# aerius-labs/zksnap-circuits-halo2

Measured on AMD Instinct MI355X. Metric: BN254 G1 MSM Mpoints/sec, higher is better.
Workload: dtype u32x9 (254-bit modular integer, radix 2^29); 1 GPU; BN254 G1 MSM, 2^20 random points/scalars per GPU (BASELINE configs[1]), point-range sharded x1, inputs resident in HBM, bases registered once (prepared fixed-base table, as under ParamsKZG::commit); points_per_gpu=1048576, parallelism=point-range shard x1 + all_gather(96 B) + fold

## Files before the change

include/zkhip.h:

```cpp
#ifndef ZKHIP_H
#define ZKHIP_H
#include <stddef.h>
#include <stdint.h>
#ifdef __cplusplus
extern "C" {
#endif

#define ZKHIP_OK 0
#define ZKHIP_EINVAL (-1)
#define ZKHIP_ENODEV (-2)
#define ZKHIP_EHIP (-3)
#define ZKHIP_ENOMEM (-4)
#define ZKHIP_EBUSY (-5)

int zkhip_init(const int *devices, int ndev);
void zkhip_shutdown(void);
const char *zkhip_last_error(void);
int zkhip_device_name(char *buf, size_t len);
int zkhip_device_count(void);
int zkhip_set_msm_shards(int shards);
int zkhip_msm_shards(void);


int zkhip_msm_g1(const uint64_t *scalars, const uint64_t *bases, size_t n, uint64_t out_xyz[12]);
// ... 103 lines not shown
                                      const uint64_t omega[4], void *d_z, void *stream);

int zkhip_lookup_permute(const uint64_t *input, const uint64_t *table, size_t usable_rows, uint64_t *permuted_input, uint64_t *permuted_table);
int zkhip_lookup_permute_device(const void *d_input, const void *d_table, size_t usable_rows, void *d_permuted_input, void *d_permuted_table,
                                void *stream);
int zkhip_lookup_permute_many_device(const void *const *d_inputs, const void *const *d_tables, uint32_t n_lookups, uint32_t log_n, size_t usable_rows,
                                     void *d_permuted_inputs, void *d_permuted_tables, void *stream);
int zkhip_lookup_products_device(const void *const *d_inputs, const void *const *d_tables, const void *d_permuted_inputs, const void *d_permuted_tables,
                                 uint32_t n_lookups, uint32_t log_n, size_t usable_rows, const uint64_t beta[4], const uint64_t gamma[4], void *d_z,
                                 void *stream);

typedef struct zkhip_check_report { uint64_t failures; uint64_t first; } zkhip_check_report;
int zkhip_check_rows_device(const zkhip_vm_program *progs, uint32_t n_progs, const void *const *d_columns, uint32_t n_columns,
                            uint32_t log_rows, uint64_t row0, uint64_t count, void *d_reports, void *stream);
int zkhip_check_copies_device(const void *const *d_columns, uint32_t n_columns, uint32_t log_n, const void *d_map_col, const void *d_map_row,
                              void *d_report, void *stream);
int zkhip_check_lookups_device(const void *const *d_inputs, const void *const *d_tables, uint32_t n_lookups, uint32_t log_n,
                               size_t usable_rows, void *d_reports, void *stream);

int zkhip_fr_random_device(const uint8_t seed[32], uint64_t stream_id, uint64_t first, size_t n, void *d_out, void *stream);
int zkhip_fr_random(const uint8_t seed[32], uint64_t stream_id, uint64_t first, size_t n, uint64_t *out);
int zkhip_fr_random_rows_device(const uint8_t seed[32], uint64_t stream_id, uint64_t first, const void *const *d_cols,
                                uint32_t n_cols, size_t row0, size_t count, void *stream);

int zkhip_alloc(size_t bytes, void **d_ptr);
int zkhip_free(void *d_ptr);
int zkhip_upload(void *d_dst, const void *src, size_t bytes);
int zkhip_download(void *dst, const void *d_src, size_t bytes);
int zkhip_sync(void);
int zkhip_stream_sync(void *stream);

int zkhip_msm_g1_device(const void *d_scalars, const void *d_bases, size_t n, void *d_out_xyz, void *stream);
int zkhip_msm_g2_device(const void *d_scalars, const void *d_bases, size_t n, void *d_out_xyz, void *stream);
int zkhip_prepare_bases_device(const void *d_bases, size_t n, uint64_t *handle);
int zkhip_prepare_bases_device_c(const void *d_bases, size_t n, int window_bits, uint64_t *handle);
int zkhip_release_bases(uint64_t handle);
int zkhip_prepared_window_bits(uint64_t handle);
int zkhip_msm_g1_prepared_device(uint64_t handle, size_t offset, const void *d_scalars, size_t n, void *d_out_xyz, void *stream);
int zkhip_msm_g1_registered_device(const uint64_t *bases, const void *d_scalars, size_t n, void *d_out_xyz, void *stream);
int zkhip_msm_g1_registered_batch_device(const uint64_t *bases, const void *d_scalars, size_t n, size_t batch, size_t scalar_stride, void *d_out_xyz,
                                         void *stream);
int zkhip_msm_g1_prepared_batch_device(uint64_t handle, size_t offset, const void *d_scalars, size_t n, size_t batch, size_t scalar_stride,
                                       void *d_out_xyz, void *stream);
int zkhip_msm_g1_device_c(const void *d_scalars, const void *d_bases, size_t n, void *d_out_xyz, int window_bits, void *stream);
int zkhip_ntt_fr_device(void *d_a, const uint64_t omega[4], uint32_t log_n, void *stream);
int zkhip_ifft_scaled_device(void *d_a, const uint64_t omega_inv[4], uint32_t log_n, const uint64_t divisor[4], void *stream);
int zkhip_mul_periodic_device(void *d_a, size_t n, const void *d_table, uint32_t period, void *stream);
int zkhip_coeff_to_extended_device(const void *d_a, size_t a_stride, uint32_t k, void *d_out, size_t out_stride, uint32_t ext_k, uint32_t batch,
                                   const uint64_t ext_omega[4], const uint64_t zeta[4], void *stream);
int zkhip_extended_to_coeff_device(const void *d_a, size_t a_stride, uint32_t ext_k, const uint64_t ext_omega_inv[4], const uint64_t ext_divisor[4],
                                   const uint64_t zeta[4], void *d_out, size_t out_stride, size_t out_len, uint32_t batch, void *stream);
int zkhip_ntt_fr_batch_device(void *d_a, const uint64_t omega[4], uint32_t log_n, uint32_t batch, size_t stride, void *stream);
int zkhip_ifft_scaled_batch_device(void *d_a, const uint64_t omega_inv[4], uint32_t log_n, const uint64_t divisor[4], uint32_t batch,
                                   size_t stride, void *stream);
int zkhip_g1_sum_device(const void *d_points_xyz, int m, void *d_out_xyz, void *stream);
int zkhip_g1_sum(const uint64_t *points_xyz, int m, uint64_t out_xyz[12]);
int zkhip_msm_window_bits(size_t n);

int zkhip_g1_gen_walk_device(const uint64_t t0[4], const uint64_t d[4], size_t n, void *d_out, void *stream);
int zkhip_g1_fixed_base_mul_device(const void *d_scalars, size_t n, void *d_out, void *stream);
int zkhip_g1_fft_device(void *d_points_xyz, const uint64_t omega[4], uint32_t log_n, void *stream);
int zkhip_g_to_lagrange_device(const void *d_g, uint32_t k, void *d_g_lagrange, void *stream);
int zkhip_g_to_lagrange(const uint64_t *g_xyz, uint32_t k, uint64_t *g_lagrange);
int zkhip_g1_batch_normalize(const uint64_t *points_xyz, size_t n, uint64_t *out_affine);
int zkhip_g1_batch_normalize_device(const void *d_points_xyz, size_t n, void *d_out_affine, void *stream);
int zkhip_g1_check_points(const uint64_t *points, size_t n, uint64_t *first_bad);
int zkhip_g1_check_points_device(const void *d_points, size_t n, uint64_t *first_bad, void *stream);
int zkhip_g1_compress(const uint64_t *points, size_t n, uint8_t *out32, int flag_layout);
int zkhip_g1_compress_device(const void *d_points, size_t n, void *d_out32, int flag_layout, void *stream);
int zkhip_g1_decompress(const uint8_t *in32, size_t n, uint64_t *points, int flag_layout, uint64_t *first_bad);
int zkhip_g1_decompress_device(const void *d_in32, size_t n, void *d_points, int flag_layout, uint64_t *first_bad, void *stream);
typedef struct zkhip_transcript zkhip_transcript;
zkhip_transcript *zkhip_transcript_new(int flag_layout);
zkhip_transcript *zkhip_transcript_new_reader(const uint8_t *proof, size_t len, int flag_layout);
void zkhip_transcript_free(zkhip_transcript *t);
int zkhip_transcript_common_scalars(zkhip_transcript *t, const uint64_t *fr_mont, size_t n);
int zkhip_transcript_common_points(zkhip_transcript *t, const uint64_t *affine_mont, size_t n);
int zkhip_transcript_squeeze(zkhip_transcript *t, uint64_t out_fr_mont[4]);
int zkhip_transcript_write_scalars(zkhip_transcript *t, const uint64_t *fr_mont, size_t n);
int zkhip_transcript_write_points_device(zkhip_transcript *t, const void *d_points_xyz, size_t n, void *stream);
int zkhip_transcript_write_scalars_device(zkhip_transcript *t, const void *d_fr, size_t n, void *stream);
int zkhip_transcript_write_points(zkhip_transcript *t, const uint64_t *points_xyz, size_t n);
int zkhip_transcript_read_scalars(zkhip_transcript *t, size_t n, uint64_t *fr_mont);
int zkhip_transcript_read_points_device(zkhip_transcript *t, size_t n, void *d_affine, void *stream);
int zkhip_transcript_read_points(zkhip_transcript *t, size_t n, uint64_t *affine_mont);
int zkhip_transcript_proof(const zkhip_transcript *t, uint8_t *buf, size_t cap, size_t *len);
zkhip_transcript *zkhip_transcript_new_poseidon(int flag_layout);
zkhip_transcript *zkhip_transcript_new_poseidon_reader(const uint8_t *proof, size_t len, int flag_layout);
int zkhip_profile_enable(int on);
int zkhip_profile_read(double *ms, char (*names)[64], int max);
int zkhip_profile_read_calls(double *ms, char (*names)[64], int *call_of, int max);

#define ZKHIP_POSEIDON_MAX_WIDTH 16
#define ZKHIP_POSEIDON_SUBTREE 256
int zkhip_poseidon_permute(uint64_t *states, size_t n);
int zkhip_poseidon_hash(const uint64_t *fr, size_t n, uint64_t out[4]);
int zkhip_poseidon_constants(uint64_t out[204 * 4]);
int zkhip_poseidon_hash_many_device(const void *d_in, size_t n, uint32_t width, void *d_out, void *stream);
int zkhip_poseidon_hash_points_device(const void *d_points, size_t n, uint32_t layout, void *d_out, void *stream);
int zkhip_poseidon_merkle_device(const void *d_leaves, size_t n_leaves, void *d_nodes, void *stream);

#define ZKHIP_IMT_MAX_DEPTH 24
typedef struct zkhip_imt zkhip_imt;
typedef struct zkhip_imt_witness {
  void *d_roots;
  void *d_low_leaves;
  void *d_new_leaves;
  void *d_low_indices;
  void *d_low_proofs;
  void *d_new_proofs;
} zkhip_imt_witness;
int zkhip_imt_create(uint32_t depth, zkhip_imt **t);
int zkhip_imt_destroy(zkhip_imt *t);
int zkhip_imt_insert(zkhip_imt *t, const uint64_t *values, size_t n_new, const zkhip_imt_witness *out, size_t *first_bad, void *stream);
int zkhip_imt_root(zkhip_imt *t, uint64_t out[4]);
int zkhip_imt_leaf(zkhip_imt *t, uint32_t index, uint64_t out[12]);
int zkhip_imt_proof(zkhip_imt *t, uint32_t index, uint64_t *out );
int zkhip_imt_size(const zkhip_imt *t, uint32_t *depth, uint32_t *used);
int zkhip_imt_export_device(zkhip_imt *t, void *d_leaves, void *d_nodes, void *d_preimages, void *stream);
int zkhip_imt_link(const uint64_t *used_vals, size_t n_used, const uint64_t *new_vals, size_t n_new, uint32_t *low_index_out, size_t *first_bad);

#define ZKHIP_PAILLIER_WORDS 6
#define ZKHIP_PAILLIER_MAX_N_BITS 192
int zkhip_paillier_mul_device(const uint64_t n[3], const void *d_a, const void *d_b, size_t count, void *d_out, void *stream);
int zkhip_paillier_tally_device(const uint64_t n[3], const void *d_ballots, size_t n_ballots, uint32_t n_cols, const void *d_init, void *d_running, void *stream);
int zkhip_paillier_encrypt_device(const uint64_t n[3], const uint64_t g[6], const void *d_m, const void *d_r, size_t count, void *d_out, void *stream);

#define ZKHIP_PLUME_MAX_MSG 64
int zkhip_secp256k1_lincomb_device(const void *d_a, const void *d_p, const void *d_b, const void *d_q, size_t count, void *d_out, void *d_status, void *stream);
int zkhip_secp256k1_hash_to_curve_device(const uint8_t *msg, size_t msg_len, const void *d_pk, size_t count, void *d_out, void *d_status, void *stream);
int zkhip_plume_verify_device(const uint8_t *msg, size_t msg_len, const void *d_pk, const void *d_nullifier, const void *d_s, const void *d_c, size_t count, void *d_status, void *d_report, void *d_h_out, void *stream);
int zkhip_plume_sign_device(const uint8_t *msg, size_t msg_len, const void *d_sk, const void *d_r, size_t count, void *d_pk, void *d_nullifier, void *d_s, void *d_c, void *d_status, void *d_h_out, void *stream);
int zkhip_secp256k1_hash_to_curve(const uint8_t *msg, size_t msg_len, const uint64_t pk[8], uint64_t out[8], uint32_t *status);
int zkhip_plume_verify(const uint8_t *msg, size_t msg_len, const uint64_t pk[8], const uint64_t nullifier[8], const uint64_t s[4], const uint64_t c[4], uint32_t *verdict, uint64_t h_out[8]);
int zkhip_plume_sign(const uint8_t *msg, size_t msg_len, const uint64_t sk[4], const uint64_t r[4], uint64_t pk[8], uint64_t nullifier[8], uint64_t s[4], uint64_t c[4], uint32_t *status, uint64_t h_out[8]);

int zkhip_fr_domain_points_device(uint32_t k, uint32_t usable_rows, const uint64_t omega[4], const void *d_x, size_t n_points, void *d_out, void *stream);
int zkhip_verify_identity_device(const zkhip_vm_program *prog, const void *d_evals, uint32_t n_evals, const void *d_challenges, uint32_t k,
                                 uint32_t usable_rows, const uint64_t omega[4], size_t n_proofs, void *d_status, void *d_report, void *stream);
int zkhip_fr_instance_evals_device(uint32_t k, const uint64_t omega[4], const void *d_x, const void *d_instances, const uint32_t *column_lens, uint32_t n_columns,
                                   const uint32_t *query_columns, const uint32_t *query_rotations, uint32_t n_queries, size_t n_proofs, void *d_out, void *stream);
int zkhip_verify_identity_instances_device(const zkhip_vm_program *prog, const void *d_evals, uint32_t n_evals, const void *d_challenges, uint32_t k,
                                           uint32_t usable_rows, const uint64_t omega[4], const void *d_instances, const uint32_t *column_lens, uint32_t n_columns,
                                           const uint32_t *query_columns, const uint32_t *query_rotations, uint32_t n_queries, size_t n_proofs,
                                           void *d_status, void *d_report, void *stream);

int zkhip_test_field_op(int field, int op, const uint64_t *a, const uint64_t *b, uint64_t *out, size_t n);
int zkhip_test_g1_op(int op, const uint64_t *a, const uint64_t *b, uint64_t *out_xyz, size_t n);

int zkhip_test_g2_op(int op, const uint64_t *a, const uint64_t *b, uint64_t *out_xyz, size_t n);

int zkhip_test_reduce512(const uint8_t in64[64], uint64_t out_fr_mont[4]);
uint32_t zkhip_test_transcript_chunk(size_t n);

#define ZKHIP_MAX_PAIRS 64
int zkhip_pairing_check(const uint64_t *g1, const uint64_t *g2, size_t n, int *ok);
int zkhip_pairing_check_device(const void *d_g1, const void *d_g2, size_t n, void *d_ok , void *stream);
int zkhip_test_fq12_op(int op, const uint64_t *a, const uint64_t *b, uint64_t *out);

struct zkhip_gwc_plan {
  uint32_t n_evals, n_sets, n_slots, reserved;
  const uint32_t *set_rotation;
  const uint32_t *query_set;
  const uint32_t *query_pos;
  const uint32_t *query_slot;
};
typedef struct zkhip_gwc_plan zkhip_gwc_plan;
int zkhip_gwc_scalars_device(const zkhip_gwc_plan *plan, const void *d_evals, const void *d_points, uint32_t k, const uint64_t omega[4], size_t n_proofs,
                             void *d_rows_a, void *d_rows_c, void *stream);
int zkhip_fr_fold_rows_device(const void *d_rows, uint32_t n_cols, uint32_t n_own, const void *d_r, int negate, size_t n_rows, void *d_out_own,
                              void *d_out_shared, void *stream);
struct zkhip_shplonk_plan {
  uint32_t n_evals, n_sets, n_slots, n_points;
  const uint32_t *point_rotation;
  const uint32_t *set_start;
  const uint32_t *set_point;
  const uint32_t *slot_set;
  const uint32_t *slot_pos;
  const uint32_t *query_slot;
  const uint32_t *query_point;
};
typedef struct zkhip_shplonk_plan zkhip_shplonk_plan;
int zkhip_shplonk_scalars_device(const zkhip_shplonk_plan *plan, const void *d_evals, const void *d_points, uint32_t k, const uint64_t omega[4], size_t n_proofs,
                                 void *d_rows_a, void *d_rows_c, void *d_status, void *stream);

#ifdef __cplusplus
}
#endif
#endif
```

zksnap_circuits_halo2_amd/_lib.py:

```python
from __future__ import annotations

import ctypes as C
import os

_HERE = os.path.dirname(os.path.abspath(__file__))
LIB_PATH = os.path.join(_HERE, "libzkhip.so")
ZKHIP_MAX_ROOTS = 8
ZKHIP_MAX_PAIRS = 64
ZKHIP_POSEIDON_MAX_WIDTH = 16
ZKHIP_POSEIDON_SUBTREE = 256
ZKHIP_IMT_MAX_DEPTH = 24
ZKHIP_PAILLIER_WORDS = 6
ZKHIP_PAILLIER_MAX_N_BITS = 192
ZKHIP_PLUME_MAX_MSG = 64

_SIGS = {
    "zkhip_init": (C.c_int, [C.POINTER(C.c_int), C.c_int]),
    "zkhip_shutdown": (None, []),
    "zkhip_last_error": (C.c_char_p, []),
    "zkhip_device_name": (C.c_int, [C.c_char_p, C.c_size_t]),
    "zkhip_device_count": (C.c_int, []),
    "zkhip_set_msm_shards": (C.c_int, [C.c_int]),
    "zkhip_msm_shards": (C.c_int, []),
    "zkhip_msm_g1": (C.c_int, [C.c_void_p, C.c_void_p, C.c_size_t, C.c_void_p]),
# ... 10 lines not shown
    "zkhip_set_ntt_fanout": (C.c_int, [C.c_int]),
    "zkhip_ntt_fanout": (C.c_int, []),
    "zkhip_register_bases": (C.c_int, [C.c_void_p, C.c_size_t]),
    "zkhip_unregister_bases": (C.c_int, [C.c_void_p]),
    "zkhip_ntt_fr": (C.c_int, [C.c_void_p, C.c_void_p, C.c_uint32]),
    "zkhip_ifft_scaled": (C.c_int, [C.c_void_p, C.c_void_p, C.c_uint32, C.c_void_p]),
    "zkhip_coeff_to_extended": (C.c_int, [C.c_void_p, C.c_uint32, C.c_void_p, C.c_uint32, C.c_void_p, C.c_void_p]),
    "zkhip_extended_to_coeff": (C.c_int, [C.c_void_p, C.c_uint32, C.c_void_p, C.c_void_p, C.c_void_p, C.c_void_p, C.c_size_t]),
    "zkhip_mul_periodic": (C.c_int, [C.c_void_p, C.c_size_t, C.c_void_p, C.c_uint32]),
    "zkhip_fr_eval_polynomial": (C.c_int, [C.c_void_p, C.c_size_t, C.c_void_p, C.c_void_p]),
    "zkhip_fr_kate_division": (C.c_int, [C.c_void_p, C.c_size_t, C.c_void_p, C.c_void_p]),
    "zkhip_fr_batch_invert": (C.c_int, [C.c_void_p, C.c_size_t]),
    "zkhip_fr_prefix_product": (C.c_int, [C.c_void_p, C.c_size_t, C.c_void_p]),
    "zkhip_fr_eval_polynomial_device": (C.c_int, [C.c_void_p, C.c_size_t, C.c_void_p, C.c_void_p, C.c_void_p]),
    "zkhip_fr_eval_polynomial_batch_device": (C.c_int, [C.c_void_p, C.c_size_t, C.c_size_t, C.c_void_p, C.c_void_p, C.c_void_p]),
    "zkhip_fr_kate_division_device": (C.c_int, [C.c_void_p, C.c_size_t, C.c_void_p, C.c_void_p, C.c_void_p]),
    "zkhip_fr_divide_by_roots": (C.c_int, [C.c_void_p, C.c_size_t, C.c_void_p, C.c_uint32, C.c_void_p, C.c_void_p]),
    "zkhip_fr_divide_by_roots_device": (C.c_int, [C.c_void_p, C.c_size_t, C.c_void_p, C.c_uint32, C.c_void_p, C.c_void_p, C.c_void_p]),
    "zkhip_fr_batch_invert_device": (C.c_int, [C.c_void_p, C.c_size_t, C.c_void_p]),
    "zkhip_fr_prefix_product_device": (C.c_int, [C.c_void_p, C.c_size_t, C.c_void_p, C.c_void_p]),
    "zkhip_fr_eval_rows": (C.c_int, [C.c_void_p, C.c_void_p, C.c_uint32, C.c_uint32, C.c_int, C.c_void_p]),
    "zkhip_fr_eval_rows_device": (C.c_int, [C.c_void_p, C.c_void_p, C.c_uint32, C.c_uint32, C.c_int, C.c_void_p, C.c_void_p]),
    "zkhip_fr_grand_product": (C.c_int, [C.c_void_p, C.c_void_p, C.c_size_t, C.c_void_p]),
    "zkhip_fr_grand_product_device": (C.c_int, [C.c_void_p, C.c_void_p, C.c_size_t, C.c_void_p, C.c_void_p]),
    "zkhip_lookup_permute": (C.c_int, [C.c_void_p, C.c_void_p, C.c_size_t, C.c_void_p, C.c_void_p]),
    "zkhip_lookup_permute_device": (C.c_int, [C.c_void_p, C.c_void_p, C.c_size_t, C.c_void_p, C.c_void_p, C.c_void_p]),
    "zkhip_lookup_permute_many_device": (C.c_int, [C.c_void_p, C.c_void_p, C.c_uint32, C.c_uint32, C.c_size_t, C.c_void_p, C.c_void_p, C.c_void_p]),
    "zkhip_lookup_products_device": (C.c_int, [C.c_void_p, C.c_void_p, C.c_void_p, C.c_void_p, C.c_uint32, C.c_uint32, C.c_size_t, C.c_void_p, C.c_void_p, C.c_void_p,
                                               C.c_void_p]),
    "zkhip_check_rows_device": (C.c_int, [C.c_void_p, C.c_uint32, C.c_void_p, C.c_uint32, C.c_uint32, C.c_uint64, C.c_uint64, C.c_void_p, C.c_void_p]),
    "zkhip_check_copies_device": (C.c_int, [C.c_void_p, C.c_uint32, C.c_uint32, C.c_void_p, C.c_void_p, C.c_void_p, C.c_void_p]),
    "zkhip_check_lookups_device": (C.c_int, [C.c_void_p, C.c_void_p, C.c_uint32, C.c_uint32, C.c_size_t, C.c_void_p, C.c_void_p]),
    "zkhip_fr_random_device": (C.c_int, [C.c_void_p, C.c_uint64, C.c_uint64, C.c_size_t, C.c_void_p, C.c_void_p]),
    "zkhip_fr_random": (C.c_int, [C.c_void_p, C.c_uint64, C.c_uint64, C.c_size_t, C.c_void_p]),
    "zkhip_fr_random_rows_device": (C.c_int, [C.c_void_p, C.c_uint64, C.c_uint64, C.c_void_p, C.c_uint32, C.c_size_t, C.c_size_t, C.c_void_p]),
    "zkhip_alloc": (C.c_int, [C.c_size_t, C.POINTER(C.c_void_p)]),
    "zkhip_free": (C.c_int, [C.c_void_p]),
    "zkhip_upload": (C.c_int, [C.c_void_p, C.c_void_p, C.c_size_t]),
    "zkhip_download": (C.c_int, [C.c_void_p, C.c_void_p, C.c_size_t]),
    "zkhip_sync": (C.c_int, []),
    "zkhip_stream_sync": (C.c_int, [C.c_void_p]),
    "zkhip_msm_g1_device": (C.c_int, [C.c_void_p, C.c_void_p, C.c_size_t, C.c_void_p, C.c_void_p]),
    "zkhip_prepare_bases_device": (C.c_int, [C.c_void_p, C.c_size_t, C.POINTER(C.c_uint64)]),
    "zkhip_g1_fft_device": (C.c_int, [C.c_void_p, C.c_void_p, C.c_uint32, C.c_void_p]),
    "zkhip_g_to_lagrange_device": (C.c_int, [C.c_void_p, C.c_uint32, C.c_void_p, C.c_void_p]),
    "zkhip_g_to_lagrange": (C.c_int, [C.c_void_p, C.c_uint32, C.c_void_p]),
    "zkhip_prepare_bases_device_c": (C.c_int, [C.c_void_p, C.c_size_t, C.c_int, C.POINTER(C.c_uint64)]),
    "zkhip_release_bases": (C.c_int, [C.c_uint64]),
    "zkhip_prepared_window_bits": (C.c_int, [C.c_uint64]),
    "zkhip_msm_g1_prepared_device": (C.c_int, [C.c_uint64, C.c_size_t, C.c_void_p, C.c_size_t, C.c_void_p, C.c_void_p]),
    "zkhip_msm_g1_prepared_batch_device": (C.c_int, [C.c_uint64, C.c_size_t, C.c_void_p, C.c_size_t, C.c_size_t, C.c_size_t, C.c_void_p, C.c_void_p]),
    "zkhip_msm_g1_device_c": (C.c_int, [C.c_void_p, C.c_void_p, C.c_size_t, C.c_void_p, C.c_int, C.c_void_p]),
    "zkhip_ntt_fr_device": (C.c_int, [C.c_void_p, C.c_void_p, C.c_uint32, C.c_void_p]),
    "zkhip_ntt_fr_batch_device": (C.c_int, [C.c_void_p, C.c_void_p, C.c_uint32, C.c_uint32, C.c_size_t, C.c_void_p]),
    "zkhip_ifft_scaled_batch_device": (C.c_int, [C.c_void_p, C.c_void_p, C.c_uint32, C.c_void_p, C.c_uint32, C.c_size_t, C.c_void_p]),
    "zkhip_ifft_scaled_device": (C.c_int, [C.c_void_p, C.c_void_p, C.c_uint32, C.c_void_p, C.c_void_p]),
    "zkhip_mul_periodic_device": (C.c_int, [C.c_void_p, C.c_size_t, C.c_void_p, C.c_uint32, C.c_void_p]),
    "zkhip_coeff_to_extended_device": (C.c_int, [C.c_void_p, C.c_size_t, C.c_uint32, C.c_void_p, C.c_size_t, C.c_uint32, C.c_uint32, C.c_void_p, C.c_void_p, C.c_void_p]),
    "zkhip_extended_to_coeff_device": (C.c_int, [C.c_void_p, C.c_size_t, C.c_uint32, C.c_void_p, C.c_void_p, C.c_void_p, C.c_void_p, C.c_size_t, C.c_size_t, C.c_uint32, C.c_void_p]),
    "zkhip_g1_sum_device": (C.c_int, [C.c_void_p, C.c_int, C.c_void_p, C.c_void_p]),
    "zkhip_g1_sum": (C.c_int, [C.c_void_p, C.c_int, C.c_void_p]),
    "zkhip_msm_window_bits": (C.c_int, [C.c_size_t]),
    "zkhip_g1_fixed_base_mul_device": (C.c_int, [C.c_void_p, C.c_size_t, C.c_void_p, C.c_void_p]),
    "zkhip_g1_gen_walk_device": (C.c_int, [C.c_void_p, C.c_void_p, C.c_size_t, C.c_void_p, C.c_void_p]),
    "zkhip_g1_batch_normalize": (C.c_int, [C.c_void_p, C.c_size_t, C.c_void_p]),
    "zkhip_g1_batch_normalize_device": (C.c_int, [C.c_void_p, C.c_size_t, C.c_void_p, C.c_void_p]),
    "zkhip_g1_check_points": (C.c_int, [C.c_void_p, C.c_size_t, C.POINTER(C.c_uint64)]),
    "zkhip_g1_check_points_device": (C.c_int, [C.c_void_p, C.c_size_t, C.POINTER(C.c_uint64), C.c_void_p]),
    "zkhip_msm_g1_registered_device": (C.c_int, [C.c_void_p, C.c_void_p, C.c_size_t, C.c_void_p, C.c_void_p]),
    "zkhip_msm_g1_registered_batch_device": (C.c_int, [C.c_void_p, C.c_void_p, C.c_size_t, C.c_size_t, C.c_size_t, C.c_void_p, C.c_void_p]),
    "zkhip_fr_gather_mul_device": (C.c_int, [C.c_void_p, C.c_size_t, C.c_void_p, C.c_void_p, C.c_size_t, C.c_void_p, C.c_size_t, C.c_void_p, C.c_void_p]),
    "zkhip_g1_compress": (C.c_int, [C.c_void_p, C.c_size_t, C.c_void_p, C.c_int]),
    "zkhip_g1_compress_device": (C.c_int, [C.c_void_p, C.c_size_t, C.c_void_p, C.c_int, C.c_void_p]),
    "zkhip_g1_decompress": (C.c_int, [C.c_void_p, C.c_size_t, C.c_void_p, C.c_int, C.POINTER(C.c_uint64)]),
    "zkhip_g1_decompress_device": (C.c_int, [C.c_void_p, C.c_size_t, C.c_void_p, C.c_int, C.POINTER(C.c_uint64), C.c_void_p]),
    "zkhip_permutation_products": (C.c_int, [C.c_void_p, C.c_void_p, C.c_uint32, C.c_uint32, C.c_uint32, C.c_size_t, C.c_void_p, C.c_void_p, C.c_void_p, C.c_void_p, C.c_void_p]),
    "zkhip_permutation_products_device": (C.c_int, [C.c_void_p, C.c_void_p, C.c_uint32, C.c_uint32, C.c_uint32, C.c_size_t, C.c_void_p, C.c_void_p, C.c_void_p, C.c_void_p,
                                                    C.c_void_p, C.c_void_p]),
    "zkhip_fr_eval_rows_sum_device": (C.c_int, [C.c_void_p, C.c_void_p, C.c_uint32, C.c_void_p, C.c_uint32, C.c_uint32, C.c_void_p, C.c_void_p]),
    "zkhip_fr_eval_rows_window_device": (C.c_int, [C.c_void_p, C.c_void_p, C.c_uint32, C.c_uint32, C.c_uint64, C.c_uint64, C.c_int, C.c_void_p, C.c_void_p]),
    "zkhip_fr_eval_rows_sharded_device": (C.c_int, [C.c_void_p, C.c_void_p, C.c_void_p, C.c_uint32, C.c_uint32, C.c_uint32, C.c_void_p, C.c_void_p, C.c_void_p,
                                                    C.c_void_p]),
    "zkhip_row_shards_create": (C.c_int, [C.c_uint32, C.c_uint32, C.c_uint32, C.c_uint32, C.POINTER(C.c_void_p)]),
    "zkhip_row_shards_destroy": (C.c_int, [C.c_void_p]),
    "zkhip_row_shards_window": (C.c_int, [C.c_void_p, C.c_uint32, C.c_uint32, C.POINTER(C.c_void_p), C.POINTER(C.c_int), C.POINTER(C.c_uint64),
                                          C.POINTER(C.c_uint64)]),
    "zkhip_row_shards_scatter_device": (C.c_int, [C.c_void_p, C.c_uint32, C.c_void_p, C.c_void_p]),
    "zkhip_row_shards_gather_device": (C.c_int, [C.c_void_p, C.c_uint32, C.c_void_p, C.c_void_p]),
    "zkhip_row_shards_upload": (C.c_int, [C.c_void_p, C.c_uint32, C.c_void_p]),
    "zkhip_coeff_to_extended_row_shards_device": (C.c_int, [C.c_void_p, C.c_uint32, C.c_uint32, C.c_size_t, C.c_void_p, C.c_void_p, C.c_void_p, C.c_uint32,
                                                            C.c_void_p]),
    "zkhip_lagrange_cosets_row_shards_device": (C.c_int, [C.c_uint32, C.c_uint64, C.c_void_p, C.c_void_p, C.c_void_p, C.c_void_p, C.c_uint32, C.c_void_p]),
    "zkhip_fr_linear_combination_device": (C.c_int, [C.c_void_p, C.c_void_p, C.c_size_t, C.c_size_t, C.c_void_p, C.c_void_p]),
    "zkhip_multiopen_gwc_device": (C.c_int, [C.c_void_p, C.c_uint32, C.c_void_p, C.c_size_t, C.c_void_p, C.c_void_p, C.c_size_t, C.POINTER(C.c_size_t)]),
    "zkhip_multiopen_shplonk_begin_device": (C.c_int, [C.c_void_p, C.c_uint32, C.c_void_p, C.c_size_t, C.c_void_p, C.c_void_p, C.c_void_p, C.POINTER(C.c_void_p)]),
    "zkhip_multiopen_shplonk_finish_device": (C.c_int, [C.c_void_p, C.c_void_p, C.c_void_p]),
    "zkhip_multiopen_shplonk_abort": (C.c_int, [C.c_void_p]),
    "zkhip_transcript_new": (C.c_void_p, [C.c_int]),
    "zkhip_transcript_new_reader": (C.c_void_p, [C.c_char_p, C.c_size_t, C.c_int]),
    "zkhip_transcript_free": (None, [C.c_void_p]),
    "zkhip_transcript_common_scalars": (C.c_int, [C.c_void_p, C.c_void_p, C.c_size_t]),
    "zkhip_transcript_common_points": (C.c_int, [C.c_void_p, C.c_void_p, C.c_size_t]),
    "zkhip_transcript_squeeze": (C.c_int, [C.c_void_p, C.c_void_p]),
    "zkhip_transcript_write_scalars": (C.c_int, [C.c_void_p, C.c_void_p, C.c_size_t]),
    "zkhip_transcript_write_points_device": (C.c_int, [C.c_void_p, C.c_void_p, C.c_size_t, C.c_void_p]),
    "zkhip_transcript_write_scalars_device": (C.c_int, [C.c_void_p, C.c_void_p, C.c_size_t, C.c_void_p]),
    "zkhip_transcript_write_points": (C.c_int, [C.c_void_p, C.c_void_p, C.c_size_t]),
    "zkhip_transcript_read_scalars": (C.c_int, [C.c_void_p, C.c_size_t, C.c_void_p]),
    "zkhip_transcript_read_points_device": (C.c_int, [C.c_void_p, C.c_size_t, C.c_void_p, C.c_void_p]),
    "zkhip_transcript_read_points": (C.c_int, [C.c_void_p, C.c_size_t, C.c_void_p]),
    "zkhip_transcript_proof": (C.c_int, [C.c_void_p, C.c_void_p, C.c_size_t, C.POINTER(C.c_size_t)]),
    "zkhip_transcript_new_poseidon": (C.c_void_p, [C.c_int]),
    "zkhip_transcript_new_poseidon_reader": (C.c_void_p, [C.c_char_p, C.c_size_t, C.c_int]),
    "zkhip_poseidon_permute": (C.c_int, [C.c_void_p, C.c_size_t]),
    "zkhip_poseidon_hash": (C.c_int, [C.c_void_p, C.c_size_t, C.c_void_p]),
    "zkhip_poseidon_constants": (C.c_int, [C.c_void_p]),
    "zkhip_poseidon_hash_many_device": (C.c_int, [C.c_void_p, C.c_size_t, C.c_uint32, C.c_void_p, C.c_void_p]),
    "zkhip_poseidon_hash_points_device": (C.c_int, [C.c_void_p, C.c_size_t, C.c_uint32, C.c_void_p, C.c_void_p]),
    "zkhip_poseidon_merkle_device": (C.c_int, [C.c_void_p, C.c_size_t, C.c_void_p, C.c_void_p]),
    "zkhip_imt_create": (C.c_int, [C.c_uint32, C.POINTER(C.c_void_p)]),
    "zkhip_imt_destroy": (C.c_int, [C.c_void_p]),
    "zkhip_imt_insert": (C.c_int, [C.c_void_p, C.c_void_p, C.c_size_t, C.c_void_p, C.POINTER(C.c_size_t), C.c_void_p]),
    "zkhip_imt_root": (C.c_int, [C.c_void_p, C.c_void_p]),
    "zkhip_imt_leaf": (C.c_int, [C.c_void_p, C.c_uint32, C.c_void_p]),
    "zkhip_imt_proof": (C.c_int, [C.c_void_p, C.c_uint32, C.c_void_p]),
    "zkhip_imt_size": (C.c_int, [C.c_void_p, C.POINTER(C.c_uint32), C.POINTER(C.c_uint32)]),
    "zkhip_imt_export_device": (C.c_int, [C.c_void_p, C.c_void_p, C.c_void_p, C.c_void_p, C.c_void_p]),
    "zkhip_imt_link": (C.c_int, [C.c_void_p, C.c_size_t, C.c_void_p, C.c_size_t, C.c_void_p, C.POINTER(C.c_size_t)]),
    "zkhip_paillier_mul_device": (C.c_int, [C.c_void_p, C.c_void_p, C.c_void_p, C.c_size_t, C.c_void_p, C.c_void_p]),
    "zkhip_paillier_tally_device": (C.c_int, [C.c_void_p, C.c_void_p, C.c_size_t, C.c_uint32, C.c_void_p, C.c_void_p, C.c_void_p]),
    "zkhip_paillier_encrypt_device": (C.c_int, [C.c_void_p, C.c_void_p, C.c_void_p, C.c_void_p, C.c_size_t, C.c_void_p, C.c_void_p]),
    "zkhip_secp256k1_lincomb_device": (C.c_int, [C.c_void_p, C.c_void_p, C.c_void_p, C.c_void_p, C.c_size_t, C.c_void_p, C.c_void_p, C.c_void_p]),
    "zkhip_secp256k1_hash_to_curve_device": (C.c_int, [C.c_char_p, C.c_size_t, C.c_void_p, C.c_size_t, C.c_void_p, C.c_void_p, C.c_void_p]),
    "zkhip_plume_verify_device": (C.c_int, [C.c_char_p, C.c_size_t, C.c_void_p, C.c_void_p, C.c_void_p, C.c_void_p, C.c_size_t, C.c_void_p, C.c_void_p, C.c_void_p,
                                            C.c_void_p]),
    "zkhip_secp256k1_hash_to_curve": (C.c_int, [C.c_char_p, C.c_size_t, C.c_void_p, C.c_void_p, C.c_void_p]),
    "zkhip_plume_verify": (C.c_int, [C.c_char_p, C.c_size_t, C.c_void_p, C.c_void_p, C.c_void_p, C.c_void_p, C.c_void_p, C.c_void_p]),
    "zkhip_plume_sign_device": (C.c_int, [C.c_char_p, C.c_size_t, C.c_void_p, C.c_void_p, C.c_size_t, C.c_void_p, C.c_void_p, C.c_void_p, C.c_void_p, C.c_void_p,
                                          C.c_void_p, C.c_void_p]),
    "zkhip_plume_sign": (C.c_int, [C.c_char_p, C.c_size_t, C.c_void_p, C.c_void_p, C.c_void_p, C.c_void_p, C.c_void_p, C.c_void_p, C.c_void_p, C.c_void_p]),
    "zkhip_fr_domain_points_device": (C.c_int, [C.c_uint32, C.c_uint32, C.c_void_p, C.c_void_p, C.c_size_t, C.c_void_p, C.c_void_p]),
    "zkhip_verify_identity_device": (C.c_int, [C.c_void_p, C.c_void_p, C.c_uint32, C.c_void_p, C.c_uint32, C.c_uint32, C.c_void_p, C.c_size_t, C.c_void_p, C.c_void_p,
                                               C.c_void_p]),
    "zkhip_fr_instance_evals_device": (C.c_int, [C.c_uint32, C.c_void_p, C.c_void_p, C.c_void_p, C.POINTER(C.c_uint32), C.c_uint32, C.POINTER(C.c_uint32),
                                                 C.POINTER(C.c_uint32), C.c_uint32, C.c_size_t, C.c_void_p, C.c_void_p]),
    "zkhip_verify_identity_instances_device": (C.c_int, [C.c_void_p, C.c_void_p, C.c_uint32, C.c_void_p, C.c_uint32, C.c_uint32, C.c_void_p, C.c_void_p,
                                                         C.POINTER(C.c_uint32), C.c_uint32, C.POINTER(C.c_uint32), C.POINTER(C.c_uint32), C.c_uint32, C.c_size_t,
                                                         C.c_void_p, C.c_void_p, C.c_void_p]),
    "zkhip_gwc_scalars_device": (C.c_int, [C.c_void_p, C.c_void_p, C.c_void_p, C.c_uint32, C.c_void_p, C.c_size_t, C.c_void_p, C.c_void_p, C.c_void_p]),
    "zkhip_fr_fold_rows_device": (C.c_int, [C.c_void_p, C.c_uint32, C.c_uint32, C.c_void_p, C.c_int, C.c_size_t, C.c_void_p, C.c_void_p, C.c_void_p]),
    "zkhip_shplonk_scalars_device": (C.c_int, [C.c_void_p, C.c_void_p, C.c_void_p, C.c_uint32, C.c_void_p, C.c_size_t, C.c_void_p, C.c_void_p, C.c_void_p, C.c_void_p]),
    "zkhip_test_reduce512": (C.c_int, [C.c_void_p, C.c_void_p]),
    "zkhip_test_transcript_chunk": (C.c_uint32, [C.c_size_t]),
    "zkhip_profile_enable": (C.c_int, [C.c_int]),
    "zkhip_profile_read": (C.c_int, [C.c_void_p, C.c_void_p, C.c_int]),
    "zkhip_profile_read_calls": (C.c_int, [C.c_void_p, C.c_void_p, C.c_void_p, C.c_int]),
    "zkhip_test_field_op": (C.c_int, [C.c_int, C.c_int, C.c_void_p, C.c_void_p, C.c_void_p, C.c_size_t]),
    "zkhip_test_g1_op": (C.c_int, [C.c_int, C.c_void_p, C.c_void_p, C.c_void_p, C.c_size_t]),
    "zkhip_pairing_check": (C.c_int, [C.c_void_p, C.c_void_p, C.c_size_t, C.POINTER(C.c_int)]),
    "zkhip_pairing_check_device": (C.c_int, [C.c_void_p, C.c_void_p, C.c_size_t, C.c_void_p, C.c_void_p]),
    "zkhip_test_fq12_op": (C.c_int, [C.c_int, C.c_void_p, C.c_void_p, C.c_void_p]),
}



class ProverQueryC(C.Structure):
    _fields_ = [("point", C.c_uint64 * 4), ("d_poly", C.c_void_p), ("eval", C.c_uint64 * 4), ("has_eval", C.c_uint32), ("reserved", C.c_uint32)]


class ImtWitness(C.Structure):
    _fields_ = [("d_roots", C.c_void_p), ("d_low_leaves", C.c_void_p), ("d_new_leaves", C.c_void_p), ("d_low_indices", C.c_void_p),
                ("d_low_proofs", C.c_void_p), ("d_new_proofs", C.c_void_p)]


class GwcPlan(C.Structure):
    _fields_ = [("n_evals", C.c_uint32), ("n_sets", C.c_uint32), ("n_slots", C.c_uint32), ("reserved", C.c_uint32),
                ("set_rotation", C.POINTER(C.c_uint32)), ("query_set", C.POINTER(C.c_uint32)), ("query_pos", C.POINTER(C.c_uint32)),
                ("query_slot", C.POINTER(C.c_uint32))]


class ShplonkPlan(C.Structure):
    _fields_ = [("n_evals", C.c_uint32), ("n_sets", C.c_uint32), ("n_slots", C.c_uint32), ("n_points", C.c_uint32),
                ("point_rotation", C.POINTER(C.c_uint32)), ("set_start", C.POINTER(C.c_uint32)), ("set_point", C.POINTER(C.c_uint32)),
                ("slot_set", C.POINTER(C.c_uint32)), ("slot_pos", C.POINTER(C.c_uint32)), ("query_slot", C.POINTER(C.c_uint32)),
                ("query_point", C.POINTER(C.c_uint32))]


class CheckReport(C.Structure):
    _fields_ = [("failures", C.c_uint64), ("first", C.c_uint64)]


class VmOperand(C.Structure):
    _fields_ = [("kind", C.c_uint8), ("rot", C.c_uint8), ("index", C.c_uint16)]


class VmInsn(C.Structure):
    _fields_ = [("op", C.c_uint8), ("dst", C.c_uint8), ("reserved", C.c_uint16), ("a", VmOperand), ("b", VmOperand), ("c", VmOperand)]


class VmProgram(C.Structure):
    _fields_ = [("insns", C.POINTER(VmInsn)), ("n_insns", C.c_uint32),
                ("constants", C.c_void_p), ("n_constants", C.c_uint32),
                ("rotations", C.POINTER(C.c_int32)), ("n_rotations", C.c_uint32),
                ("rot_scale", C.c_int32), ("result_reg", C.c_uint32), ("omega", C.c_void_p)]


VM_REGS = 16
_lib = None


class ZkhipError(RuntimeError):
    index = None

    def __init__(self, code: int, msg: str):
        super().__init__(f"libzkhip error {code}: {msg}")
        self.code = code


def load() -> C.CDLL:
    global _lib
    if _lib is not None:
        return _lib
    path = os.environ.get("ZKHIP_LIB_PATH", LIB_PATH)
    if not os.path.exists(path):
        raise ImportError(f"{path} not found: build it with `python -c 'import __graft_entry__ as g; g.build()'` "
                          "(hipcc, gfx950).  There is no CPU fallback.")
    try:
        import torch
    except ImportError:
        pass
    lib = C.CDLL(path)
    for name, (res, args) in _SIGS.items():
        fn = getattr(lib, name)
        fn.restype = res
        fn.argtypes = args
    _lib = lib
    return lib


def exported_symbols():
    return sorted(_SIGS)


def check(rc: int) -> None:
    if rc != 0:
        raise ZkhipError(rc, load().zkhip_last_error().decode(errors="replace"))
```

zksnap_circuits_halo2_amd/csrc/capi.hip:

```cpp
#include <hip/hip_runtime.h>
#include <algorithm>
#include <atomic>
#include <condition_variable>
#include <cstdarg>
#include <cstdio>
#include <cstdlib>
#include <cstring>
#include <dlfcn.h>
#include <functional>
#include <map>
#include <memory>
#include <mutex>
#include <thread>
#include <vector>
#include "zkhip_internal.hpp"
#include "blake2b.hpp"
#include "poseidon.hpp"
#include "imt.hpp"
#include "modn.hpp"
#include "secp256k1_h2c.hpp"
#include "../../include/zkhip.hpp"

namespace zkhip {

// ... 3824 lines not shown
  if (!t) return;
  delete t->sponge;
  if (t->pinned) { (void)hipHostFree(t->pinned); (void)hipGetLastError(); }
  delete t;
}

int zkhip_transcript_common_scalars(zkhip_transcript* t, const uint64_t* fr_mont, size_t n) {
  if (!t || (n && !fr_mont)) { set_error("transcript_common_scalars: null pointer"); return ZKHIP_EINVAL; }
  for (size_t i = 0; i < n; i++) {
    uint8_t repr[32];
    fr_mont_to_repr(fr_mont + i * 4, repr);
    tr_absorb_scalar(t, repr);
  }
  return ZKHIP_OK;
}

int zkhip_transcript_common_points(zkhip_transcript* t, const uint64_t* affine_mont, size_t n) {
  if (!t || (n && !affine_mont)) { set_error("transcript_common_points: null pointer"); return ZKHIP_EINVAL; }
  for (size_t i = 0; i < n; i++)
    if (bytes_zero((const uint8_t*)(affine_mont + i * 8), 64)) { set_error("transcript: cannot write points at infinity to the transcript (point %zu of %zu)", i, n); return ZKHIP_EINVAL; }
  for (size_t i = 0; i < n; i++) {
    uint8_t xy[64];
    fq_mont_to_repr(affine_mont + i * 8, xy);
    fq_mont_to_repr(affine_mont + i * 8 + 4, xy + 32);
    tr_absorb_point(t, xy);
  }
  return ZKHIP_OK;
}

int zkhip_transcript_squeeze(zkhip_transcript* t, uint64_t out_fr_mont[4]) {
  if (!t || !out_fr_mont) { set_error("transcript_squeeze: null pointer"); return ZKHIP_EINVAL; }
  if (t->poseidon) {
    const halo2::Fr c = t->sponge->squeeze();
    memcpy(out_fr_mont, c.l, 32);
    return ZKHIP_OK;
  }
  const uint8_t prefix = 0x00;
  t->st.update(&prefix, 1);
  uint8_t digest[64];
  t->st.digest(digest, 64);
  fr_reduce512(digest, out_fr_mont);
  return ZKHIP_OK;
}

int zkhip_transcript_write_scalars(zkhip_transcript* t, const uint64_t* fr_mont, size_t n) {
  int rc = tr_check_write(t, fr_mont, n, "transcript_write_scalars");
  if (rc != ZKHIP_OK) return rc;
  for (size_t i = 0; i < n; i++) {
    uint8_t repr[32];
    fr_mont_to_repr(fr_mont + i * 4, repr);
    tr_absorb_scalar(t, repr);
    t->proof.insert(t->proof.end(), repr, repr + 32);
  }
  return ZKHIP_OK;
}

int zkhip_transcript_write_points_device(zkhip_transcript* t, const void* d_points_xyz, size_t n, void* stream) {
  ZK_API_RANGE();
  int rc = tr_check_write(t, d_points_xyz, n, "transcript_write_points_device");
  if (rc != ZKHIP_OK) return rc;
  if ((uintptr_t)d_points_xyz & 15) { set_error("transcript_write_points_device: d_points_xyz must be 16-byte aligned"); return ZKHIP_EINVAL; }
  if (n == 0) return ZKHIP_OK;
  hipStream_t s = caller_stream(stream);
  scratch_pin P(s);
  if (P.rc != ZKHIP_OK) return P.rc;
  stream_drain drain(s);
  if ((rc = tr_write_points_core(t, P.sc, s, d_points_xyz, n)) != ZKHIP_OK) return rc;
  drain.done();
  return ZKHIP_OK;
}

int zkhip_transcript_write_scalars_device(zkhip_transcript* t, const void* d_fr, size_t n, void* stream) {
  ZK_API_RANGE();
  int rc = tr_check_write(t, d_fr, n, "transcript_write_scalars_device");
  if (rc != ZKHIP_OK) return rc;
  if ((uintptr_t)d_fr & 15) { set_error("transcript_write_scalars_device: d_fr must be 16-byte aligned"); return ZKHIP_EINVAL; }
  if (n == 0) return ZKHIP_OK;
  hipStream_t s = caller_stream(stream);
  scratch_pin P(s);
  if (P.rc != ZKHIP_OK) return P.rc;
  stream_drain drain(s);
  if ((rc = tr_write_scalars_core(t, P.sc, s, d_fr, n)) != ZKHIP_OK) return rc;
  drain.done();
  return ZKHIP_OK;
}

int zkhip_transcript_write_points(zkhip_transcript* t, const uint64_t* points_xyz, size_t n) {
  ZK_API_RANGE();
  int rc = tr_check_write(t, points_xyz, n, "transcript_write_points");
  if (rc != ZKHIP_OK) return rc;
  if (n == 0) return ZKHIP_OK;
  lane_hold H;
  if (H.rc != ZKHIP_OK) return H.rc;
  if ((rc = H.sc->poly.reserve(n * 96)) != ZKHIP_OK) return rc;
  HIPCHK(hipMemcpyAsync(H.sc->poly.p, points_xyz, n * 96, hipMemcpyHostToDevice, H.s));
  if ((rc = tr_write_points_core(t, H.sc, H.s, H.sc->poly.p, n)) != ZKHIP_OK) return rc;
  return H.finish();
}

int zkhip_transcript_read_scalars(zkhip_transcript* t, size_t n, uint64_t* fr_mont) {
  int rc = tr_check_read(t, fr_mont, n, "transcript_read_scalars");
  if (rc != ZKHIP_OK) return rc;
  const uint8_t* src = t->proof.data() + t->cursor;
  for (size_t i = 0; i < n; i++)
    if (!fr_repr_to_mont(src + i * 32, fr_mont + i * 4)) { set_error("transcript: read_scalars: scalar %zu of %zu (proof byte %zu) is not below r", i, n, t->cursor + i * 32); return ZKHIP_EINVAL; }
  for (size_t i = 0; i < n; i++) tr_absorb_scalar(t, src + i * 32);
  t->cursor += n * 32;
  return ZKHIP_OK;
}

int zkhip_transcript_read_points_device(zkhip_transcript* t, size_t n, void* d_affine, void* stream) {
  ZK_API_RANGE();
  int rc = tr_check_read(t, d_affine, n, "transcript_read_points_device");
  if (rc != ZKHIP_OK) return rc;
  if ((uintptr_t)d_affine & 15) { set_error("transcript_read_points_device: d_affine must be 16-byte aligned"); return ZKHIP_EINVAL; }
  if (n == 0) return ZKHIP_OK;
  hipStream_t s = caller_stream(stream);
  scratch_pin P(s);
  if (P.rc != ZKHIP_OK) return P.rc;
  stream_drain drain(s);
  if ((rc = tr_read_points_core(t, P.sc, s, n, d_affine, nullptr)) != ZKHIP_OK) return rc;
  drain.done();
  return ZKHIP_OK;
}

int zkhip_transcript_read_points(zkhip_transcript* t, size_t n, uint64_t* affine_mont) {
  ZK_API_RANGE();
  int rc = tr_check_read(t, affine_mont, n, "transcript_read_points");
  if (rc != ZKHIP_OK) return rc;
  if (n == 0) return ZKHIP_OK;
  lane_hold H;
  if (H.rc != ZKHIP_OK) return H.rc;
  if ((rc = H.sc->bases.reserve(n * 64)) != ZKHIP_OK) return rc;
  if ((rc = tr_read_points_core(t, H.sc, H.s, n, H.sc->bases.p, affine_mont)) != ZKHIP_OK) return rc;
  return H.finish();
}

int zkhip_transcript_proof(const zkhip_transcript* t, uint8_t* buf, size_t cap, size_t* len) {
  if (!t || !len) { set_error("transcript_proof: null pointer"); return ZKHIP_EINVAL; }
  *len = t->proof.size();
  if (!buf) return ZKHIP_OK;
  if (cap < t->proof.size()) { set_error("transcript_proof: %zu bytes of room, %zu needed", cap, t->proof.size()); return ZKHIP_EINVAL; }
  if (!t->proof.empty()) memcpy(buf, t->proof.data(), t->proof.size());
  return ZKHIP_OK;
}

int zkhip_test_reduce512(const uint8_t in64[64], uint64_t out_fr_mont[4]) {
  if (!in64 || !out_fr_mont) { set_error("test_reduce512: null pointer"); return ZKHIP_EINVAL; }
  fr_reduce512(in64, out_fr_mont);
  return ZKHIP_OK;
}

uint32_t zkhip_test_transcript_chunk(size_t n) { return transcript_chunk(n); }

}
```

zksnap_circuits_halo2_amd/csrc/msm.hip:

```cpp
#include <hip/hip_runtime.h>
#include <atomic>
#include <cstdint>
#include <cstdio>
#include <cstring>
#include <cstdlib>
#include <mutex>
#include "ec_quad.hpp"
#include "fe_inverse.hpp"
#include "reduce_plan.hpp"
#include "zkhip_internal.hpp"

namespace zkhip {

static inline size_t align_up(size_t v, size_t a) { return (v + a - 1) / a * a; }

constexpr int FINE_BITS = 12;
constexpr int MAX_GROUPS = 128;
constexpr int MAX_WIDE_W = 16;
struct win_layout { int c, W, narrow; };
__host__ __device__ __forceinline__ int win_bits(const win_layout& L, int w) { return w < L.W - L.narrow ? L.c : L.c - 1; }
__host__ __device__ __forceinline__ int win_off(const win_layout& L, int w) { const int full = L.W - L.narrow; return w <= full ? w * L.c : full * L.c + (w - full) * (L.c - 1); }
static int msm_narrow_windows(int c, int W) {
  if (c <= 16) return 0;
  const int narrow = W * c - 256;
  return narrow > 0 && narrow <= W ? narrow : 0;
}
constexpr int MAX_TASK_LEN = 128;
constexpr int TASK_SHIFT = 6;

__device__ __forceinline__ xyzz load_xyzz(const uint32_t* base, size_t idx) {
  const uint4* q = reinterpret_cast<const uint4*>(base + idx * 36);
  uint32_t w[36];
#pragma unroll
  for (int i = 0; i < 9; i++) {
    uint4 v = q[i];
    w[4 * i] = v.x; w[4 * i + 1] = v.y; w[4 * i + 2] = v.z; w[4 * i + 3] = v.w;
  }
  xyzz r;
#pragma unroll
  for (int i = 0; i < 9; i++) { r.X.l[i] = w[i]; r.Y.l[i] = w[9 + i]; r.ZZ.l[i] = w[18 + i]; r.ZZZ.l[i] = w[27 + i]; }
  return r;
}

__device__ __forceinline__ void store_xyzz(uint32_t* base, size_t idx, const xyzz& a) {
  uint32_t w[36];
#pragma unroll
  for (int i = 0; i < 9; i++) { w[i] = a.X.l[i]; w[9 + i] = a.Y.l[i]; w[18 + i] = a.ZZ.l[i]; w[27 + i] = a.ZZZ.l[i]; }
  uint4* q = reinterpret_cast<uint4*>(base + idx * 36);
#pragma unroll
  for (int i = 0; i < 9; i++) q[i] = make_uint4(w[4 * i], w[4 * i + 1], w[4 * i + 2], w[4 * i + 3]);
}

__device__ __forceinline__ xyzz xyzz_shfl_xor(const xyzz& a, int mask) {
  xyzz r;
#pragma unroll
  for (int i = 0; i < NL; i++) {
    r.X.l[i] = (uint32_t)__shfl_xor((int)a.X.l[i], mask, 64);
    r.Y.l[i] = (uint32_t)__shfl_xor((int)a.Y.l[i], mask, 64);
    r.ZZ.l[i] = (uint32_t)__shfl_xor((int)a.ZZ.l[i], mask, 64);
    r.ZZZ.l[i] = (uint32_t)__shfl_xor((int)a.ZZZ.l[i], mask, 64);
  }
  return r;
}

__device__ __forceinline__ fe load_fe9_generic(const uint32_t* p, size_t idx) {
  fe r;
#pragma unroll
  for (int i = 0; i < 9; i++) r.l[i] = p[idx * 9 + i];
  return r;
}
__device__ __forceinline__ void store_fe9_generic(uint32_t* p, size_t idx, const fe& a) {
#pragma unroll
  for (int i = 0; i < 9; i++) p[idx * 9 + i] = a.l[i];
}

__global__ void __launch_bounds__(256) k_digits(const uint32_t* __restrict__ scalars, int16_t* __restrict__ digits,
                                                uint32_t n, uint32_t n_pad, int c, int W, uint32_t K, size_t scalar_stride, int narrow) {
  const size_t idx = (size_t)blockIdx.x * blockDim.x + threadIdx.x;
  if (idx >= (size_t)K * n_pad) return;
  const uint32_t kb = (uint32_t)(idx / n_pad), i = (uint32_t)(idx % n_pad);
  digits += (size_t)kb * n_pad;
  const size_t row = (size_t)K * n_pad;
  if (i >= n) {
    for (int win = 0; win < W; win++) digits[(size_t)win * row + i] = 0;
    return;
  }
  uint32_t w[8];
  load_words(scalars + ((size_t)kb * scalar_stride + i) * 8, w);
  fe c32;
#pragma unroll
  for (int k = 0; k < NL; k++) c32.l[k] = FrParams::FROM_EXT_CANON[k];
  fe s = fe_canon_lt2p<FrParams>(fe_mul<FrParams>(c32, fe_unpack<0>(w)));
  fe_pack(s, w);
  const win_layout lay{c, W, narrow};
  uint32_t carry = 0;
  for (int win = 0; win < W; win++) {
    const int bit = win_off(lay, win), cw = win_bits(lay, win);
    const uint32_t half = 1u << (cw - 1), mask = (1u << cw) - 1;
    uint32_t v = 0;
    if (bit < 256) {
      int wi = bit >> 5, sh = bit & 31;
      uint64_t two = w[wi];
      if (wi + 1 < 8) two |= (uint64_t)w[wi + 1] << 32;
      v = (uint32_t)(two >> sh) & mask;
    }
    v += carry;
    int32_t d;
    if (v >= half) { d = (int32_t)v - (int32_t)(1u << cw); carry = 1; } else { d = (int32_t)v; carry = 0; }
    digits[(size_t)win * row + i] = (int16_t)d;
  }
}

__global__ void __launch_bounds__(1024) k_digits_wide(const uint32_t* __restrict__ scalars, int32_t* __restrict__ digits, uint32_t n, uint32_t n_pad,
                                                       int c, int W, uint32_t* __restrict__ gcount, int narrow) {
  __shared__ uint32_t cnt[MAX_WIDE_W * MAX_GROUPS];
  for (uint32_t t = threadIdx.x; t < (uint32_t)W * MAX_GROUPS; t += blockDim.x) cnt[t] = 0;
  __syncthreads();
  const win_layout lay{c, W, narrow};
  for (uint32_t i = blockIdx.x * blockDim.x + threadIdx.x; i < n_pad; i += gridDim.x * blockDim.x) {
    if (i >= n) {
      for (int win = 0; win < W; win++) digits[(size_t)win * n_pad + i] = 0;
      continue;
    }
    uint32_t w[8];
    load_words(scalars + (size_t)i * 8, w);
    fe c32;
#pragma unroll
    for (int k = 0; k < NL; k++) c32.l[k] = FrParams::FROM_EXT_CANON[k];
    fe sv = fe_canon_lt2p<FrParams>(fe_mul<FrParams>(c32, fe_unpack<0>(w)));
    fe_pack(sv, w);
    uint32_t carry = 0;
    for (int win = 0; win < W; win++) {
      const int bit = win_off(lay, win), cw = win_bits(lay, win);
      const uint32_t half = 1u << (cw - 1), mask = (1u << cw) - 1;
      uint32_t v = 0;
      if (bit < 256) {
        const int wi = bit >> 5, sh = bit & 31;
        uint64_t two = w[wi];
        if (wi + 1 < 8) two |= (uint64_t)w[wi + 1] << 32;
        v = (uint32_t)(two >> sh) & mask;
      }
      v += carry;
      int32_t d;
      if (v >= half) { d = (int32_t)v - (int32_t)(1u << cw); carry = 1; } else { d = (int32_t)v; carry = 0; }
      digits[(size_t)win * n_pad + i] = d;
      if (d != 0) atomicAdd(&cnt[win * MAX_GROUPS + (((uint32_t)(d < 0 ? -d : d) - 1) >> FINE_BITS)], 1u);
    }
  }
  __syncthreads();
  for (uint32_t t = threadIdx.x; t < (uint32_t)W * MAX_GROUPS; t += blockDim.x)
    if (cnt[t]) atomicAdd(&gcount[t], cnt[t]);
}

namespace glv {
__device__ constexpr uint32_t G1[3] = {0xc7e0b3d7u, 0xd91d232eu, 0x2u};
__device__ constexpr uint32_t G2[5] = {0x391eb18eu, 0x7a7bd9d4u, 0xa773d2cfu, 0x4ccef014u, 0x2u};
__device__ constexpr uint32_t A1[2] = {0x94d213e3u, 0x89d32568u};
__device__ constexpr uint32_t A2[4] = {0x1221250bu, 0x0be4e154u, 0xeeb859fdu, 0x6f4d8248u};
__device__ constexpr uint32_t NB1[4] = {0x7d4f1128u, 0x8211bbebu, 0xeeb859fcu, 0x6f4d8248u};
__device__ constexpr uint32_t BETA_EXT[8] = {0xd782e155u, 0x71930c11u, 0xffbe3323u, 0xa6bb947cu, 0xd4741444u, 0xaa303344u, 0x26594943u, 0x2c3b3f0du};

template <int NA, int NB, int NO>
__device__ __forceinline__ void mul_low(const uint32_t (&a)[NA], const uint32_t* __restrict__ b, uint32_t (&out)[NO]) {
#pragma unroll
  for (int i = 0; i < NO; i++) out[i] = 0;
#pragma unroll
  for (int i = 0; i < NA; i++) {
    uint32_t carry = 0;
#pragma unroll
    for (int j = 0; j < NB; j++) {
      if (i + j < NO) {
        const uint64_t t = (uint64_t)a[i] * b[j] + out[i + j] + carry;
        out[i + j] = (uint32_t)t;
        carry = (uint32_t)(t >> 32);
      }
    }
    if (i + NB < NO) out[i + NB] = carry;
  }
}

__device__ __forceinline__ bool abs160(uint32_t (&v)[5], uint32_t (&mag)[4]) {
// ... 270 lines not shown

constexpr uint32_t SORT_CHUNK = 28672;

__global__ void __launch_bounds__(64) k_group_offsets(const uint32_t* __restrict__ wcount, int W, int G, uint32_t* __restrict__ goff, uint32_t* __restrict__ wcursor,
                                                       uint32_t* __restrict__ cstart, uint32_t chunk) {
  if (blockIdx.x != 0 || threadIdx.x >= 64) return;
  const int lane = threadIdx.x;
  uint32_t c0 = 0, c1 = 0;
  for (int w = 0; w < W; w++) {
    if (2 * lane < G) c0 += wcount[w * MAX_GROUPS + 2 * lane];
    if (2 * lane + 1 < G) c1 += wcount[w * MAX_GROUPS + 2 * lane + 1];
  }
  const uint32_t k0 = (c0 + chunk - 1) / chunk, k1 = (c1 + chunk - 1) / chunk;
  uint32_t x = c0 + c1, y = k0 + k1;
#pragma unroll
  for (int off = 1; off < 64; off <<= 1) {
    const uint32_t xs = __shfl_up(x, off, 64), ys = __shfl_up(y, off, 64);
    if (lane >= off) { x += xs; y += ys; }
  }
  const uint32_t ex = x - (c0 + c1), ey = y - (k0 + k1);
  if (2 * lane < G) { goff[2 * lane] = ex; cstart[2 * lane] = ey; }
  if (2 * lane + 1 < G) { goff[2 * lane + 1] = ex + c0; cstart[2 * lane + 1] = ey + k0; }
  uint32_t r0 = ex, r1 = ex + c0;
  for (int w = 0; w < W; w++) {
    if (2 * lane < G) { wcursor[w * MAX_GROUPS + 2 * lane] = r0; r0 += wcount[w * MAX_GROUPS + 2 * lane]; }
    if (2 * lane + 1 < G) { wcursor[w * MAX_GROUPS + 2 * lane + 1] = r1; r1 += wcount[w * MAX_GROUPS + 2 * lane + 1]; }
  }
  if (lane == 63) { goff[G] = x; cstart[G] = y; }
}

constexpr int FINE_BATCH = 7;
__device__ __forceinline__ void fine_histogram(const uint16_t* __restrict__ stage_fine, uint32_t start, uint32_t end, uint32_t* __restrict__ cur) {
  for (uint32_t p = start + threadIdx.x; p < end; p += FINE_BATCH * blockDim.x) {
    uint32_t f[FINE_BATCH];
#pragma unroll
    for (int k = 0; k < FINE_BATCH; k++) { const uint32_t q = p + k * blockDim.x; f[k] = q < end ? stage_fine[q] : 0xffffffffu; }
#pragma unroll
    for (int k = 0; k < FINE_BATCH; k++) if (f[k] != 0xffffffffu) atomicAdd(&cur[f[k]], 1u);
  }
}

__global__ void __launch_bounds__(1024) k_fine_sorted(const uint16_t* __restrict__ stage_fine, const uint32_t* __restrict__ stage_ref,
                                                      const uint32_t* __restrict__ goff, const uint32_t* __restrict__ cstart, int G,
                                                      uint32_t* __restrict__ cursor, uint32_t* __restrict__ sorted) {
  extern __shared__ uint32_t hist[];
  constexpr uint32_t FB = 1u << FINE_BITS;
  constexpr uint32_t CHUNK = SORT_CHUNK;
  constexpr int PER_LANE = CHUNK / 1024;
  static_assert(FB == 4096, "one thread owns four buckets in the scan");
  static_assert(CHUNK % 1024 == 0 && CHUNK / 32 <= 1024, "a lane owns CHUNK / 1024 entries; one mask word per thread");
  __shared__ uint32_t wsum[3][16];
  uint32_t* cur = hist;
  uint32_t* delta = hist + FB;
  uint32_t* refs = hist + 2 * FB;
  uint32_t* mask = refs + CHUNK;
  uint32_t* wpre = mask + CHUNK / 32;
  const uint32_t w = blockIdx.x;
  if (w >= cstart[G]) return;
  uint32_t glo = 0, ghi = (uint32_t)G;
  while (ghi - glo > 1) { const uint32_t mid = (glo + ghi) >> 1; if (cstart[mid] <= w) glo = mid; else ghi = mid; }
  const uint32_t g = glo;
  const uint32_t start = goff[g] + (w - cstart[g]) * CHUNK, end = min(goff[g + 1], start + CHUNK), cnt_n = end - start;
  uint32_t f[PER_LANE], r[PER_LANE];
#pragma unroll
  for (int k = 0; k < PER_LANE; k++) { const uint32_t q = start + threadIdx.x + k * 1024u; f[k] = q < end ? stage_fine[q] : 0xffffffffu; }
#pragma unroll
  for (int k = 0; k < PER_LANE; k++) { const uint32_t q = start + threadIdx.x + k * 1024u; r[k] = q < end ? stage_ref[q] : 0u; }
  for (uint32_t b = threadIdx.x; b < FB; b += blockDim.x) cur[b] = 0;
  if (threadIdx.x < CHUNK / 32) mask[threadIdx.x] = 0;
  __syncthreads();
  static_assert(CHUNK <= (1u << 15) && FINE_BITS + 15 < 32, "fine id and rank share a register, and 0xffffffff stays the mark of no entry");
#pragma unroll
  for (int k = 0; k < PER_LANE; k++) if (f[k] != 0xffffffffu) f[k] |= atomicAdd(&cur[f[k]], 1u) << FINE_BITS;
  __syncthreads();
  uint32_t c[4], l[4], s = 0;
#pragma unroll
  for (int k = 0; k < 4; k++) { c[k] = cur[4 * threadIdx.x + k]; s += c[k]; }
  uint32_t* gl = cursor + (size_t)g * FB;
  uint32_t gb[4];
#pragma unroll
  for (int k = 0; k < 4; k++) gb[k] = c[k] ? atomicAdd(&gl[4 * threadIdx.x + k], c[k]) : 0u;
  const int lane = threadIdx.x & 63, wave = threadIdx.x >> 6;
  const uint32_t nz = (c[0] != 0) + (c[1] != 0) + (c[2] != 0) + (c[3] != 0);
  uint32_t x = s, y = nz;
#pragma unroll
  for (int off = 1; off < 64; off <<= 1) {
    const uint32_t xs = __shfl_up(x, off, 64), ys = __shfl_up(y, off, 64);
    if (lane >= off) { x += xs; y += ys; }
  }
  if (lane == 63) { wsum[0][wave] = x; wsum[1][wave] = y; }
  __syncthreads();
  uint32_t run = x - s, rank = y - nz;
#pragma unroll
  for (int i = 0; i < 16; i++) if (i < wave) { run += wsum[0][i]; rank += wsum[1][i]; }
#pragma unroll
  for (int k = 0; k < 4; k++) { l[k] = run; run += c[k]; }
#pragma unroll
  for (int k = 0; k < 4; k++) {
    cur[4 * threadIdx.x + k] = l[k];
    if (c[k]) {
      delta[rank++] = gb[k] - l[k];
      atomicOr(&mask[l[k] >> 5], 1u << (l[k] & 31));
    }
  }
  __syncthreads();
#pragma unroll
  for (int k = 0; k < PER_LANE; k++) if (f[k] != 0xffffffffu) refs[cur[f[k] & (FB - 1)] + (f[k] >> FINE_BITS)] = r[k];
  const uint32_t pc = threadIdx.x < CHUNK / 32 ? (uint32_t)__popc(mask[threadIdx.x]) : 0u;
  uint32_t z = pc;
#pragma unroll
  for (int off = 1; off < 64; off <<= 1) {
    const uint32_t t = __shfl_up(z, off, 64);
    if (lane >= off) z += t;
  }
  if (lane == 63) wsum[2][wave] = z;
  __syncthreads();
  uint32_t zb = z - pc;
#pragma unroll
  for (int i = 0; i < 16; i++) if (i < wave) zb += wsum[2][i];
  if (threadIdx.x < CHUNK / 32) wpre[threadIdx.x] = zb;
  __syncthreads();
  for (uint32_t i = threadIdx.x; i < cnt_n; i += blockDim.x) {
    const uint32_t rk = wpre[i >> 5] + (uint32_t)__popc(mask[i >> 5] & ((2u << (i & 31)) - 1u)) - 1u;
    sorted[delta[rk] + i] = refs[i];
  }
}

__global__ void __launch_bounds__(1024) k_fine_count(const uint16_t* __restrict__ stage_fine, const uint32_t* __restrict__ goff,
                                                     const uint32_t* __restrict__ cstart, int G, uint32_t* __restrict__ count, uint32_t chunk) {
  constexpr uint32_t FB = 1u << FINE_BITS;
  __shared__ uint32_t cur[FB];
  const uint32_t w = blockIdx.x;
  if (w >= cstart[G]) return;
  uint32_t glo = 0, ghi = (uint32_t)G;
  while (ghi - glo > 1) { const uint32_t mid = (glo + ghi) >> 1; if (cstart[mid] <= w) glo = mid; else ghi = mid; }
  const uint32_t g = glo;
  const uint32_t start = goff[g] + (w - cstart[g]) * chunk, end = min(goff[g + 1], start + chunk);
  for (uint32_t b = threadIdx.x; b < FB; b += blockDim.x) cur[b] = 0;
  __syncthreads();
  fine_histogram(stage_fine, start, end, cur);
  __syncthreads();
  uint32_t* gl = count + (size_t)g * FB;
  for (uint32_t b = threadIdx.x; b < FB; b += blockDim.x) {
    const uint32_t v = cur[b];
    if (v) atomicAdd(&gl[b], v);
  }
}

constexpr int SCAN_BLOCK = 256, SCAN_PER_THREAD = 4,
          SCAN_TILE = SCAN_BLOCK * SCAN_PER_THREAD;
constexpr uint32_t SCAN_APPLY_WGS = 256;

template <int MODE>
__device__ __forceinline__ uint32_t scan_xform(uint32_t v, uint32_t task_shift) {
  return MODE == 0 ? v : (v + (1u << task_shift) - 1) >> task_shift;
}

__device__ __forceinline__ uint32_t block_exclusive_scan(uint32_t v, uint32_t* lds, uint32_t& total) {
  const int lane = threadIdx.x & 63, wave = threadIdx.x >> 6;
  uint32_t x = v;
#pragma unroll
  for (int off = 1; off < 64; off <<= 1) {
    uint32_t y = __shfl_up(x, off, 64);
    if (lane >= off) x += y;
  }
  if (lane == 63) lds[wave] = x;
  __syncthreads();
  uint32_t base = 0, tot = 0;
#pragma unroll
  for (int i = 0; i < SCAN_BLOCK / 64; i++) {
    uint32_t t = lds[i];
    if (i < wave) base += t;
    tot += t;
  }
  __syncthreads();
  total = tot;
  return base + x - v;
}

__global__ void __launch_bounds__(SCAN_BLOCK) k_scan_sums2(const uint32_t* __restrict__ in, uint32_t n, uint32_t* __restrict__ sums0,
                                                           uint32_t* __restrict__ sums1, uint32_t task_shift) {
  __shared__ uint32_t lds[4];
  const uint32_t base = blockIdx.x * SCAN_TILE + threadIdx.x * SCAN_PER_THREAD;
  uint32_t s0 = 0, s1 = 0;
#pragma unroll
  for (int i = 0; i < SCAN_PER_THREAD; i++) if (base + i < n) { const uint32_t v = in[base + i]; s0 += v; s1 += scan_xform<1>(v, task_shift); }
  uint32_t t0, t1;
  block_exclusive_scan(s0, lds, t0);
  block_exclusive_scan(s1, lds, t1);
  if (threadIdx.x == 0) { sums0[blockIdx.x] = t0; sums1[blockIdx.x] = t1; }
}

__global__ void __launch_bounds__(SCAN_BLOCK) k_scan_top2(uint32_t* __restrict__ sums0, uint32_t* __restrict__ sums1, uint32_t nb,
                                                          uint32_t* __restrict__ total0, uint32_t* __restrict__ total1) {
  __shared__ uint32_t lds[4];
  uint32_t run0 = 0, run1 = 0;
  for (uint32_t base = 0; base < nb; base += SCAN_BLOCK) {
    const uint32_t i = base + threadIdx.x;
    const uint32_t v0 = i < nb ? sums0[i] : 0, v1 = i < nb ? sums1[i] : 0;
    uint32_t t0, t1;
    const uint32_t e0 = block_exclusive_scan(v0, lds, t0), e1 = block_exclusive_scan(v1, lds, t1);
    if (i < nb) { sums0[i] = run0 + e0; sums1[i] = run1 + e1; }
    run0 += t0; run1 += t1;
  }
  if (threadIdx.x == 0) { *total0 = run0; *total1 = run1; }
}

__global__ void __launch_bounds__(SCAN_BLOCK) k_scan_apply2(const uint32_t* __restrict__ in, uint32_t n, const uint32_t* __restrict__ sums0,
                                                            const uint32_t* __restrict__ sums1, const uint32_t* __restrict__ total0,
                                                            const uint32_t* __restrict__ total1, uint32_t* __restrict__ offset,
                                                            uint32_t* __restrict__ cursor, uint32_t* __restrict__ task_off, uint32_t task_shift,
                                                            uint32_t nblk, uint32_t* __restrict__ len_count) {
  __shared__ uint32_t lds[4];
  __shared__ uint32_t lh[MAX_TASK_LEN + 1];
  static_assert(SCAN_BLOCK > MAX_TASK_LEN, "one thread per length");
  if (threadIdx.x <= MAX_TASK_LEN) lh[threadIdx.x] = 0;
  __syncthreads();
  uint32_t n_full = 0;
  auto load_tile = [&](uint32_t blk, uint32_t (&v)[SCAN_PER_THREAD]) {
    const uint32_t base = blk * SCAN_TILE + threadIdx.x * SCAN_PER_THREAD;
#pragma unroll
    for (int i = 0; i < SCAN_PER_THREAD; i++) v[i] = (blk < nblk && base + i < n) ? in[base + i] : 0;
  };
  uint32_t v[SCAN_PER_THREAD], vn[SCAN_PER_THREAD];
  load_tile(blockIdx.x, v);
  for (uint32_t blk = blockIdx.x; blk < nblk; blk += gridDim.x) {
    const uint32_t base = blk * SCAN_TILE + threadIdx.x * SCAN_PER_THREAD;
    load_tile(blk + gridDim.x, vn);
    uint32_t s0 = 0, s1 = 0;
#pragma unroll
    for (int i = 0; i < SCAN_PER_THREAD; i++) { s0 += v[i]; s1 += scan_xform<1>(v[i], task_shift); }
    uint32_t t0, t1;
    uint32_t e0 = block_exclusive_scan(s0, lds, t0) + sums0[blk];
    uint32_t e1 = block_exclusive_scan(s1, lds, t1) + sums1[blk];
#pragma unroll
    for (int i = 0; i < SCAN_PER_THREAD; i++) {
      if (base + i < n) { offset[base + i] = e0; cursor[base + i] = e0; task_off[base + i] = e1; }
      const uint32_t m = scan_xform<1>(v[i], task_shift);
      if (m) {
        n_full += m - 1;
        atomicAdd(&lh[v[i] - ((m - 1) << task_shift)], 1u);
      }
      e0 += v[i];
      e1 += m;
    }
#pragma unroll
    for (int i = 0; i < SCAN_PER_THREAD; i++) v[i] = vn[i];
  }
#pragma unroll
  for (int off = 32; off >= 1; off >>= 1) n_full += (uint32_t)__shfl_xor((int)n_full, off, 64);
  if ((threadIdx.x & 63) == 0 && n_full) atomicAdd(&lh[1u << task_shift], n_full);
  __syncthreads();
  if (threadIdx.x <= MAX_TASK_LEN && lh[threadIdx.x]) atomicAdd(&len_count[threadIdx.x], lh[threadIdx.x]);
  if (blockIdx.x == 0 && threadIdx.x == 0) { offset[n] = *total0; task_off[n] = *total1; }
}

constexpr uint32_t SCAN_SINGLE_MAX = 8192;
template <int MODE>
__global__ void __launch_bounds__(1024) k_scan_single(const uint32_t* __restrict__ in, uint32_t n, uint32_t* __restrict__ total_out,
                                                      uint32_t* __restrict__ out, uint32_t* __restrict__ out2, uint32_t task_shift,
                                                      uint32_t* __restrict__ len_cursor) {
  __shared__ uint32_t wsum[16];
  __shared__ uint32_t lh[MAX_TASK_LEN + 1];
  if (MODE == 1 && threadIdx.x <= MAX_TASK_LEN) lh[threadIdx.x] = 0;
  __syncthreads();
  const int lane = threadIdx.x & 63, wave = threadIdx.x >> 6;
  const uint32_t full = 1u << task_shift;
  uint32_t running = 0, n_full = 0;
  for (uint32_t tile = 0; tile < n; tile += 8192) {
    const uint32_t base = tile + threadIdx.x * 8;
    uint32_t v[8], s = 0;
#pragma unroll
    for (int i = 0; i < 8; i++) {
      const uint32_t raw = base + i < n ? in[base + i] : 0u;
      v[i] = scan_xform<MODE>(raw, task_shift);
      s += v[i];
      if (MODE == 1 && raw) {
        n_full += v[i] - 1;
        atomicAdd(&lh[raw - ((v[i] - 1) << task_shift)], 1u);
      }
    }
    uint32_t x = s;
#pragma unroll
    for (int off = 1; off < 64; off <<= 1) {
      const uint32_t y = __shfl_up(x, off, 64);
      if (lane >= off) x += y;
    }
    if (lane == 63) wsum[wave] = x;
    __syncthreads();
    uint32_t before = 0, tot = 0;
#pragma unroll
    for (int i = 0; i < 16; i++) {
      const uint32_t t = wsum[i];
      if (i < wave) before += t;
      tot += t;
    }
    __syncthreads();
    uint32_t ex = running + before + x - s;
#pragma unroll
    for (int i = 0; i < 8; i++) {
      if (base + i < n) { out[base + i] = ex; if (out2) out2[base + i] = ex; }
      ex += v[i];
    }
    running += tot;
  }
  if (threadIdx.x == 0) { out[n] = running; *total_out = running; }
  if (MODE == 1) {
    if (n_full) atomicAdd(&lh[full], n_full);
    __syncthreads();
    if (threadIdx.x == 0) {
      uint32_t run = 0;
      for (int L = MAX_TASK_LEN; L >= 1; L--) { len_cursor[L] = run; run += lh[L]; }
    }
  }
}

constexpr uint32_t HEAVY_SLICE = 2048;
constexpr uint32_t COOP_TASKS = 32;
__global__ void __launch_bounds__(256) k_make_tasks(const uint32_t* __restrict__ offset, const uint32_t* __restrict__ task_off,
                                                    uint32_t nbuckets, task_t* __restrict__ tasks, uint32_t task_shift,
                                                    uint32_t* __restrict__ max_parts, uint32_t seq_parts,
                                                    uint32_t* __restrict__ heavy_count, uint2* __restrict__ heavy, uint32_t heavy_cap) {
  uint32_t nt = 0;
  const uint32_t lane = threadIdx.x & 63u;
  for (uint32_t base = blockIdx.x * blockDim.x + (threadIdx.x & ~63u); base < nbuckets; base += gridDim.x * blockDim.x) {
    const uint32_t k = base + lane;
    uint32_t s = 0, e = 0, t = 0, m = 0;
    if (k < nbuckets) { s = offset[k]; e = offset[k + 1]; t = task_off[k]; m = task_off[k + 1] - t; }
    const bool coop = m > COOP_TASKS;
    if (!coop) {
      for (uint32_t j = 0; j < m; j++) {
        task_t tk;
        tk.bucket = k;
        tk.start = s + (j << task_shift);
        tk.len = min(1u << task_shift, e - tk.start);
        tasks[t + j] = tk;
      }
    }
    if (m > seq_parts) {
      const uint32_t P = (m + HEAVY_SLICE - 1) / HEAVY_SLICE;
      const uint32_t idx = atomicAdd(heavy_count, P);
      for (uint32_t i = 0; i < P; i++)
        if (idx + i < heavy_cap) heavy[idx + i] = make_uint2(k, i);
    }
    nt = max(nt, m);
    unsigned long long big = __ballot(coop);
    while (big) {
      const int src = __ffsll((long long)big) - 1;
      big &= big - 1;
      const uint32_t bk = (uint32_t)__shfl((int)k, src, 64), bs = (uint32_t)__shfl((int)s, src, 64), be = (uint32_t)__shfl((int)e, src, 64),
                     bt = (uint32_t)__shfl((int)t, src, 64), bm = (uint32_t)__shfl((int)m, src, 64);
      for (uint32_t j = lane; j < bm; j += 64) {
        task_t tk;
        tk.bucket = bk;
        tk.start = bs + (j << task_shift);
        tk.len = min(1u << task_shift, be - tk.start);
        tasks[bt + j] = tk;
      }
    }
  }
#pragma unroll
  for (int off = 32; off >= 1; off >>= 1) nt = max(nt, (uint32_t)__shfl_xor((int)nt, off, 64));
  if ((threadIdx.x & 63) == 0 && nt > 1) atomicMax(max_parts, nt);
}

constexpr int ORDER_JMAX = 64;
__global__ void __launch_bounds__(256) k_make_order(const uint32_t* __restrict__ offset, const uint32_t* __restrict__ task_off,
                                                    uint32_t nbuckets, uint32_t task_shift, uint32_t* __restrict__ len_cursor,
                                                    const uint32_t* __restrict__ sorted, uint4* __restrict__ order,
                                                    const uint32_t* __restrict__ len_count, task_t* __restrict__ tasks,
                                                    uint32_t* __restrict__ max_parts, uint32_t seq_parts, uint32_t* __restrict__ heavy_count,
                                                    uint2* __restrict__ heavy, uint32_t heavy_cap) {
  __shared__ uint32_t lh[MAX_TASK_LEN + 1], lbase[MAX_TASK_LEN + 1];
  __shared__ uint32_t jcnt[ORDER_JMAX + 1], joff[ORDER_JMAX + 1];
  static_assert(MAX_TASK_LEN == 128, "two lengths per lane of one wavefront");
  if (threadIdx.x <= MAX_TASK_LEN) lh[threadIdx.x] = 0;
  if (threadIdx.x <= ORDER_JMAX) jcnt[threadIdx.x] = 0;
  if (threadIdx.x >= 192) {
    const int lane = threadIdx.x - 192, L0 = MAX_TASK_LEN - 2 * lane, L1 = L0 - 1;
    const uint32_t c0 = len_count ? len_count[L0] : 0u, c1 = len_count ? len_count[L1] : 0u;
    uint32_t x = c0 + c1;
#pragma unroll
    for (int off = 1; off < 64; off <<= 1) {
      const uint32_t y = __shfl_up(x, off, 64);
      if (lane >= off) x += y;
    }
    const uint32_t ex = x - (c0 + c1);
    lbase[L0] = ex;
    lbase[L1] = ex + c0;
    if (lane == 0) lbase[0] = 0;
  }
  __syncthreads();
  const uint32_t full = 1u << task_shift, step = gridDim.x * blockDim.x;
  for (uint32_t k = blockIdx.x * blockDim.x + threadIdx.x; k < nbuckets; k += step) {
    const uint32_t nt = task_off[k + 1] - task_off[k];
    if (nt) {
      const uint32_t rem = (offset[k + 1] - offset[k]) - ((nt - 1) << task_shift);
      atomicAdd(&lh[rem], 1u);
      const uint32_t nfull = nt - 1, head = min(nfull, (uint32_t)ORDER_JMAX);
      for (uint32_t j = 0; j < head; j++) atomicAdd(&jcnt[j], 1u);
      if (nfull > head) atomicAdd(&jcnt[ORDER_JMAX], nfull - head);
    }
  }
  __syncthreads();
  if (threadIdx.x == 0) {
    uint32_t run = 0;
    for (int j = 0; j <= ORDER_JMAX; j++) { joff[j] = run; run += jcnt[j]; }
    const uint32_t base = run ? lbase[full] + atomicAdd(&len_cursor[full], run) : 0u;
    for (int j = 0; j <= ORDER_JMAX; j++) joff[j] += base;
  }
  if (threadIdx.x <= MAX_TASK_LEN && threadIdx.x != full) { const uint32_t v = lh[threadIdx.x]; lh[threadIdx.x] = v ? lbase[threadIdx.x] + atomicAdd(&len_cursor[threadIdx.x], v) : 0u; }
  __syncthreads();
  if (threadIdx.x == 0 && lh[full]) lh[full] = lbase[full] + atomicAdd(&len_cursor[full], lh[full]);
  __syncthreads();
  const uint32_t lane = threadIdx.x & 63u;
  uint32_t mx = 0;
  for (uint32_t base = blockIdx.x * blockDim.x + (threadIdx.x & ~63u); base < nbuckets; base += step) {
    const uint32_t k = base + lane;
    uint32_t t = 0, nt = 0, s0 = 0, pos = 0, nfull = 0, head = 0;
    if (k < nbuckets) { t = task_off[k]; nt = task_off[k + 1] - t; }
    if (nt) {
      s0 = offset[k];
      const uint32_t rem = (offset[k + 1] - s0) - ((nt - 1) << task_shift);
      nfull = nt - 1;
      head = min(nfull, (uint32_t)ORDER_JMAX);
      for (uint32_t j = 0; j < head; j++) {
        const uint32_t st = s0 + (j << task_shift);
        order[atomicAdd(&joff[j], 1u)] = make_uint4(t + j, st, full, sorted[st]);
        if (tasks) tasks[t + j] = task_t{k, st, full};
      }
      if (nfull > head) pos = atomicAdd(&joff[ORDER_JMAX], nfull - head);
      const uint32_t st = s0 + ((nt - 1) << task_shift);
      order[atomicAdd(&lh[rem], 1u)] = make_uint4(nt == 1 ? (0x80000000u | k) : t + nt - 1, st, rem, sorted[st]);
      if (tasks) tasks[t + nt - 1] = task_t{k, st, rem};
      if (tasks && nt > seq_parts) {
        const uint32_t P = (nt + HEAVY_SLICE - 1) / HEAVY_SLICE;
        const uint32_t idx = atomicAdd(heavy_count, P);
        for (uint32_t i = 0; i < P; i++)
          if (idx + i < heavy_cap) heavy[idx + i] = make_uint2(k, i);
      }
      mx = max(mx, nt);
    }
    const bool coop = nfull - head > COOP_TASKS;
    if (!coop) {
      for (uint32_t j = head; j < nfull; j++) {
        const uint32_t st = s0 + (j << task_shift);
        order[pos + j - head] = make_uint4(t + j, st, full, sorted[st]);
        if (tasks) tasks[t + j] = task_t{k, st, full};
      }
    }
    unsigned long long big = __ballot(coop);
    while (big) {
      const int src = __ffsll((long long)big) - 1;
      big &= big - 1;
      const uint32_t bt = (uint32_t)__shfl((int)t, src, 64), bs0 = (uint32_t)__shfl((int)s0, src, 64), bpos = (uint32_t)__shfl((int)pos, src, 64),
                     bnfull = (uint32_t)__shfl((int)nfull, src, 64), bhead = (uint32_t)__shfl((int)head, src, 64);
      for (uint32_t j = bhead + lane; j < bnfull; j += 64) {
        const uint32_t st = bs0 + (j << task_shift);
        order[bpos + j - bhead] = make_uint4(bt + j, st, full, sorted[st]);
        if (tasks) tasks[bt + j] = task_t{base + (uint32_t)src, st, full};
      }
    }
  }
  if (tasks) {
#pragma unroll
    for (int off = 32; off >= 1; off >>= 1) mx = max(mx, (uint32_t)__shfl_xor((int)mx, off, 64));
    if (lane == 0 && mx > 1) atomicMax(max_parts, mx);
  }
}

template <bool TABLE>
__global__ void __launch_bounds__(128) __attribute__((amdgpu_waves_per_eu(4, 4))) k_accumulate(const task_t* __restrict__ tasks, const uint32_t* __restrict__ ntasks_p,
                                                    const uint4* __restrict__ order, const uint32_t* __restrict__ sorted,
                                                    const uint32_t* __restrict__ bases, uint32_t* __restrict__ partials,
                                                    uint32_t* __restrict__ buckets, const uint32_t* __restrict__ bases2, uint32_t split) {
  auto point = [&](uint32_t idx) -> affine_words {
    if constexpr (!TABLE) { if (idx >= split) return load_affine(bases2, idx - split); }
    return load_affine(bases, idx);
  };
  const uint32_t ntasks = *ntasks_p;
  for (uint32_t i = blockIdx.x * blockDim.x + threadIdx.x; i < ntasks; i += gridDim.x * blockDim.x) {
    const uint4 rec = order[i];
    const uint32_t t = rec.x;
    struct { uint32_t start, len; } tk = {rec.y, rec.z};
    xyzz acc = xyzz_identity();
    const uint32_t* refs = sorted + tk.start;
    uint32_t ref = rec.w;
    affine_words pt = point(ref & 0x7fffffffu);
    uint32_t j = 0;
    if constexpr (TABLE) {
      if (!affine_is_identity(pt)) {
        acc.X = fe_unpack<0>(pt.x);
        acc.Y = fe_unpack<0>(pt.y);
        if (ref >> 31) acc.Y = fe_norm(fe_neg_red(acc.Y, Fq::P2_S1));
        acc.ZZ = acc.ZZZ = fe_one<Fq>();
      }
      if (tk.len > 1) {
        ref = refs[1];
        pt = point(ref & 0x7fffffffu);
      }
      j = 1;
    }
    uint32_t nref = j + 1 < tk.len ? refs[j + 1] : 0u;
    for (; j < tk.len; j++) {
      affine_words cur = pt;
      uint32_t cref = ref;
      if (j + 1 < tk.len) {
        ref = nref;
        pt = point(ref & 0x7fffffffu);
      }
      if (j + 2 < tk.len) nref = refs[j + 2];
      if (affine_is_identity(cur)) continue;
      fe x2, y2;
      if constexpr (TABLE) {
        x2 = fe_unpack<0>(cur.x);
        y2 = fe_unpack<0>(cur.y);
        if (cref >> 31) y2 = fe_neg_red(y2, Fq::P2_S1);
      } else {
        x2 = fe_from_ext_lazy(cur.x);
        y2 = fe_from_ext_lazy(cur.y);
        if (cref >> 31) y2 = fe_neg_red(y2, Fq::P64_S1);
      }
      xyzz_madd<true>(acc, x2, y2);
    }
    if (t >> 31) store_xyzz(buckets, t & 0x7fffffffu, acc);
    else store_xyzz(partials, t, acc);
  }
}

constexpr uint32_t HEAVY_WGS = 256;
constexpr uint32_t HEAVY_QUAD_MAX = 256;

__device__ __forceinline__ xyzz workgroup_sum_128(xyzz acc, uint32_t* __restrict__ xch) {
#pragma unroll 1
  for (uint32_t half = 64; half >= 1; half >>= 1) {
    __syncthreads();
    if (threadIdx.x >= half && threadIdx.x < 2 * half) store_xyzz(xch, threadIdx.x - half, acc);
    __syncthreads();
    if (threadIdx.x < half) acc = xyzz_add(acc, load_xyzz(xch, threadIdx.x));
  }
  return acc;
}

__device__ __forceinline__ void combine_heavy_buckets(uint32_t wg, const uint32_t* __restrict__ task_off, uint32_t* __restrict__ partials,
                                                      uint32_t* __restrict__ buckets, const uint32_t* __restrict__ heavy_count,
                                                      const uint2* __restrict__ heavy, uint32_t heavy_cap, uint32_t* __restrict__ heavy_done,
                                                      uint32_t* __restrict__ xch , uint32_t quad_max) {
  __shared__ uint32_t is_last;
  const uint32_t nh = min(*heavy_count, heavy_cap);
  for (uint32_t i = wg; i < nh; i += HEAVY_WGS) {
    const uint2 e = heavy[i];
    const uint32_t k = e.x, sl = e.y, t = task_off[k], m = task_off[k + 1] - t;
    const uint32_t P = (m + HEAVY_SLICE - 1) / HEAVY_SLICE, lo = sl * HEAVY_SLICE, hi = min(m, lo + HEAVY_SLICE);
    if (m <= quad_max) {
      const uint32_t q = threadIdx.x & 3, quad = threadIdx.x >> 2;
      xyzz acc = xyzz_identity();
#pragma unroll 1
      for (uint32_t j = quad; j < m; j += 32) acc = xyzz_add_quad(acc, load_xyzz(partials, t + j), q);
#pragma unroll 1
      for (int mask = 4; mask < 64; mask <<= 1) acc = xyzz_add_quad(acc, xyzz_shfl_xor(acc, mask), q);
      __syncthreads();
      if (threadIdx.x == 64) store_xyzz(xch, 0, acc);
      __syncthreads();
      if (threadIdx.x < 4) {
        acc = xyzz_add_quad(acc, load_xyzz(xch, 0), q);
        if (q == 0) store_xyzz(buckets, k, acc);
      }
      continue;
    }
    xyzz acc = xyzz_identity();
#pragma unroll 1
    for (uint32_t j = lo + threadIdx.x; j < hi; j += 128) acc = xyzz_add(acc, load_xyzz(partials, t + j));
    acc = workgroup_sum_128(acc, xch);
    if (P == 1) {
      if (threadIdx.x == 0) store_xyzz(buckets, k, acc);
      continue;
    }
    if (threadIdx.x == 0) {
      store_xyzz(partials, t + lo, acc);
      __threadfence();
      is_last = atomicAdd(&heavy_done[i - sl], 1u) == P - 1;
    }
    __syncthreads();
    if (!is_last) continue;
    __threadfence();
    acc = xyzz_identity();
#pragma unroll 1
    for (uint32_t j = threadIdx.x; j < P; j += 128) acc = xyzz_add(acc, load_xyzz(partials, t + j * HEAVY_SLICE));
    acc = workgroup_sum_128(acc, xch);
    if (threadIdx.x == 0) store_xyzz(buckets, k, acc);
  }
}

template <int COMBINE_LANES>
__global__ void __launch_bounds__(128) k_combine_seq(const uint32_t* __restrict__ task_off, uint32_t nbuckets,
                                                     uint32_t* __restrict__ partials, uint32_t* __restrict__ buckets,
                                                     uint32_t seq_parts, uint32_t blocks, const uint32_t* __restrict__ heavy_count,
                                                     const uint2* __restrict__ heavy, uint32_t heavy_cap, uint32_t* __restrict__ heavy_done, uint32_t quad_max) {
  __shared__ __attribute__((aligned(16))) uint32_t xch[64 * 36];
  if (blockIdx.x >= blocks) { combine_heavy_buckets(blockIdx.x - blocks, task_off, partials, buckets, heavy_count, heavy, heavy_cap, heavy_done, xch, quad_max); return; }
  const uint32_t gid = blockIdx.x * blockDim.x + threadIdx.x;
  const uint32_t k = gid / COMBINE_LANES, q = gid % COMBINE_LANES;
  const bool live = k < nbuckets;
  xyzz acc = xyzz_identity();
  uint32_t m = 0;
  if (live) {
    const uint32_t t = task_off[k];
    m = task_off[k + 1] - t;
    const uint32_t left = (m == 1 || m > seq_parts) ? 0u : m;
#pragma unroll 1
    for (uint32_t j = q; j < left; j += COMBINE_LANES) acc = xyzz_add(acc, load_xyzz(partials, t + j));
// ... 134 lines not shown
    if (q == 0) {
      if (jac_out) store_jacobian(acc, jac_out + (size_t)win * 24);
      else store_xyzz(winsum, win, acc);
    }
  }
}

constexpr int FINISH_CHAIN0 = 11, FINISH_CHAIN1 = 15, FINISH_CHAIN2 = 17;

__global__ void __launch_bounds__(FINISH_THREADS) k_reduce_finish(const uint32_t* __restrict__ in, uint32_t in_stride, uint32_t N, int s,
                                                                  uint32_t* __restrict__ winsum, uint32_t* __restrict__ jac_out) {
  __shared__ __attribute__((aligned(16))) uint32_t lds[(REDUCE_FINISH_ADDS + REDUCE_FINISH_ADDS2) * 36];
  __shared__ __attribute__((aligned(16))) uint32_t xch[3 * 36];
  constexpr uint32_t BUF1 = REDUCE_FINISH_ADDS * 36;
  const int win = blockIdx.x;
  const uint32_t q = threadIdx.x & 3, quad = threadIdx.x >> 2;
  const uint32_t* wi = in + (size_t)win * in_stride * 36;
  const bool levels = N > 2;
  uint32_t cur = 0;
  bool first = true;
#pragma unroll 1
  while (N > 2) {
    const uint32_t per_win = N / 2 + (uint32_t)s * (N / 4);
    const uint32_t nxt = first ? 0u : (cur == 0 ? BUF1 : 0u);
    static_assert(FINISH_THREADS / 4 >= (int)REDUCE_FINISH_ADDS, "one quad per addition of the widest level");
    if (quad < per_win) {
      uint32_t ia, ib;
      reduce_step_operands(N, s, quad, ia, ib);
      xyzz a, b;
      if (first) { a = load_xyzz(wi, ia); b = load_xyzz(wi, ib); }
      else { a = load_xyzz(lds + cur, ia); b = load_xyzz(lds + cur, ib); }
      const xyzz r = xyzz_add_quad(a, b, q);
      if (q == 0) store_xyzz(lds + nxt, quad, r);
    }
    __syncthreads();
    cur = nxt; first = false;
    N >>= 1;
    s++;
  }
  const int nz = s - 1;
  const int wave = threadIdx.x >> 6, j = (threadIdx.x & 63) >> 2;
  const int n0 = min(nz, FINISH_CHAIN0) + 1;
  int dbl = 0;
  int idx = -1;
  int count = 0;
  auto chains = [&](int lo, int hi) {
    count = max(0, min(nz, hi) - lo + 1);
    if (j < count) { dbl = lo + j; idx = dbl < nz ? 2 + dbl : 1; }
  };
  if (wave == 0) { chains(0, FINISH_CHAIN0); count = n0 + 2; if (j == n0) idx = 0; else if (j == n0 + 1) idx = 1; }
  else if (wave == 1) chains(FINISH_CHAIN0 + 1, FINISH_CHAIN1);
  else if (wave == 2) chains(FINISH_CHAIN1 + 1, FINISH_CHAIN2);
  else if (wave == 3) chains(FINISH_CHAIN2 + 1, 63);
  xyzz acc = xyzz_identity();
  if (idx >= 0) { if (levels) acc = load_xyzz(lds + cur, idx); else acc = load_xyzz(wi, idx); }
#pragma unroll 1
  for (int i = 0; i < dbl; i++) acc = xyzz_dbl_quad(acc, q);
#pragma unroll 1
  for (int phase = 0; phase < 2; phase++) {
    if (phase == 1) {
      __syncthreads();
      count = wave == 0 ? 4 : 0;
      if (wave == 0 && j >= 1) acc = j < 4 ? load_xyzz(xch, j - 1) : xyzz_identity();
    }
#pragma unroll 1
    for (int mask = 4; (mask >> 2) < count; mask <<= 1) acc = xyzz_add_quad(acc, xyzz_shfl_xor(acc, mask), q);
    if (phase == 0 && wave >= 1 && wave <= 3 && (threadIdx.x & 63) == 0) store_xyzz(xch, wave - 1, acc);
  }
  if (threadIdx.x == 0) {
    if (jac_out) store_jacobian(acc, jac_out + (size_t)win * 24);
    else store_xyzz(winsum, win, acc);
  }
}

__global__ void __launch_bounds__(64) k_fold(const uint32_t* __restrict__ winsum, int W, int c, uint32_t* __restrict__ out) {
  if (threadIdx.x >= 4 || blockIdx.x != 0) return;
  const uint32_t q = threadIdx.x;
  xyzz acc = load_xyzz(winsum, W - 1);
  for (int w = W - 2; w >= 0; w--) {
#pragma unroll 1
    for (int i = 0; i < c; i++) acc = xyzz_dbl_quad(acc, q);
    acc = xyzz_add_quad(acc, load_xyzz(winsum, w), q);
  }
  if (q == 0) store_jacobian(acc, out);
}

__global__ void __launch_bounds__(STORE_THREADS) k_store_results(const uint32_t* __restrict__ winsum, uint32_t K, uint32_t* __restrict__ out) {
  const uint32_t k = blockIdx.x * blockDim.x + threadIdx.x;
  if (k < K) store_jacobian(load_xyzz(winsum, k), out + (size_t)k * 24);
}

__global__ void __launch_bounds__(64) k_sum_jacobian(const uint32_t* __restrict__ in, int m, uint32_t* __restrict__ out, uint32_t stride) {
  const uint32_t q = threadIdx.x & 3;
  const int grp = threadIdx.x >> 2;
  in += (size_t)blockIdx.x * 24;
  out += (size_t)blockIdx.x * 24;
  xyzz acc = xyzz_identity();
  for (int i = grp; i < m; i += 16) acc = xyzz_add_quad(acc, load_jacobian(in + (size_t)i * stride * 24), q);
#pragma unroll 1
  for (int mask = 4; mask < 64; mask <<= 1) {
    if ((mask >> 2) >= m && mask > 4) break;
    acc = xyzz_add_quad(acc, xyzz_shfl_xor(acc, mask), q);
  }
  if (threadIdx.x == 0) store_jacobian(acc, out);
}

static bool msm_top_window_is_degenerate(int c) {
  const int W = (256 + c - 1) / c, top_bits = 254 - (W - 1) * c;
  return top_bits > 0 && top_bits < 6;
}

static inline int msm_windows(int c, bool glv) {
  if (!glv) return (256 + c - 1) / c;
  return (128 + c - 1) / c + ((c == 2 || c == 4) ? 1 : 0);
}

int msm_pick_window(size_t n) {
  int best = 16;
  double best_cost = 1e300;
  for (int c = 2; c <= 16; c++) {
    const int Wi = msm_windows(c, true), top_bits = 127 - (Wi - 1) * c;
    if (top_bits > 0 && top_bits < 6) continue;
    const double cost = (double)Wi * (10.0 * (double)(2 * n) + 28.0 * (double)(1u << (c - 1)));
    if (cost < best_cost) { best_cost = cost; best = c; }
  }
  return best;
}


constexpr int MAX_WINDOW_PREPARED = 20;

int msm_pick_window_prepared(size_t n) {
  const bool large = n >= ((size_t)1 << 20);
  int best = 2;
  double best_cost = 1e300;
  for (int c = 2; c <= MAX_WINDOW_PREPARED; c++) {
    const double W = (256 + c - 1) / c, buckets = (double)(1u << (c - 1));
    if (msm_top_window_is_degenerate(c) && c <= 16) continue;
    if (c > 16 && !large) continue;
    if (c == 17) continue;
    double cost;
    if (!large) cost = W * 10.0 * (double)n + 28.0 * buckets;
    else {
      const double eff = c == 20 ? 1.0 : (c == 19 ? 1.13 : (c == 18 ? 1.06 : 1.07));
      cost = W * (10.0 * eff + 1.0) * (double)n + 39.0 * buckets + 1.1e6 * (double)(c - 2) + 13.0e6;
    }
    if (cost < best_cost) { best_cost = cost; best = c; }
  }
  if (n >= ((size_t)1 << 14) && n < ((size_t)3 << 14)) best = 15;
  return best;
}

struct msm_layout {
  uint32_t task_shift;
  size_t max_tasks;
  void* digits;
  uint32_t* stage_ref; uint16_t* stage_fine;
  char* zero_lo; size_t zero_bytes;
  uint32_t *gcounters, *counters, *count, *sorted, *offset, *cursor, *task_off, *bsum1, *bsum2;
  task_t* tasks; uint4* order;
  uint32_t *partials, *pyrA, *pyrB, *winsum;
  uint32_t* endo;
  int combine_lanes;
  uint32_t seq_parts;
  uint2* heavy; uint32_t heavy_cap;
  uint32_t* heavy_done;
  size_t total;
};

static uint32_t msm_task_shift(size_t entries , size_t NB, size_t xyzz_bytes = 144) {
  uint32_t task_shift = TASK_SHIFT;
  if ((entries >> 7) >= ((size_t)3 << 16)) task_shift = 7;
  const bool g2 = xyzz_bytes == 288;
  if ((entries >> TASK_SHIFT) < ((size_t)1 << (g2 ? 14 : 17))) {
    const double occ = (double)entries / (double)NB;
    double best = 1e300;
    for (uint32_t sh = 2; sh <= (uint32_t)TASK_SHIFT; sh++) {
      const double L = (double)(1u << sh), parts = occ / L;
      const double est = 5.0 * L + (g2 ? 15.0 : 10.0) * (parts > 1.0 ? parts - 1.0 : 0.0);
      if (est < best) { best = est; task_shift = sh; }
    }
  }
  return task_shift;
}

constexpr size_t GLV_TWO_LEVEL_MIN = (size_t)1 << 18;
constexpr size_t PREP_TWO_LEVEL_MIN = (size_t)1 << 16;
static bool msm_two_level(int c, bool glv, size_t n_in, bool shared_buckets, size_t K) {
  if (c > 16) return true;
  if (c != 16 || K != 1) return false;
  if (glv) return n_in >= GLV_TWO_LEVEL_MIN;
  return shared_buckets && n_in >= PREP_TWO_LEVEL_MIN;
}

static msm_layout msm_lay_out(char* base, size_t n_in, size_t K, int c, bool prepared, size_t xyzz_bytes = 144, bool glv = false) {
  msm_layout L;
  const size_t n = glv ? 2 * n_in : n_in;
  const size_t W = (size_t)msm_windows(c, glv), B = (size_t)1 << (c - 1), WB = prepared ? K : W, NB = WB * B;
  const bool wide = msm_two_level(c, glv, n_in, prepared, K);
  const size_t nk = n * K, entries = W * nk;
  const size_t n_pad = (n + 7) & ~(size_t)7;
  L.task_shift = msm_task_shift(entries, NB, xyzz_bytes);
  L.max_tasks = (entries >> L.task_shift) + NB + 1;
  const double parts_avg = (double)entries / (double)NB / (double)(1u << L.task_shift);
  L.combine_lanes = parts_avg <= 2.0 ? 1 : (parts_avg <= 4.0 ? 2 : (parts_avg <= 12.0 ? 4 : 8));
  L.seq_parts = 16u * (uint32_t)L.combine_lanes;
  L.heavy_cap = (uint32_t)(std::min<size_t>(L.max_tasks / (L.seq_parts + 1) + 1, NB) + L.max_tasks / HEAVY_SLICE + 1);
  char* p = base;
  auto carve = [&](size_t bytes) { void* r = p; p += align_up(bytes, 256); return r; };
  L.digits = carve(W * K * n_pad * (wide ? sizeof(int32_t) : sizeof(int16_t)));
  L.stage_ref = wide ? (uint32_t*)carve(entries * sizeof(uint32_t)) : nullptr;
  L.stage_fine = wide ? (uint16_t*)carve(entries * sizeof(uint16_t)) : nullptr;
  L.zero_lo = p;
  L.gcounters = wide ? (uint32_t*)carve(32768) : nullptr;
  L.counters = (uint32_t*)carve(2048);
  L.count = (uint32_t*)carve((NB + 1) * sizeof(uint32_t));
  L.heavy_done = (uint32_t*)carve((size_t)L.heavy_cap * sizeof(uint32_t));
  L.zero_bytes = (size_t)(p - L.zero_lo);
  L.sorted = (uint32_t*)carve(entries * sizeof(uint32_t));
  L.offset = (uint32_t*)carve((NB + 1) * sizeof(uint32_t));
  L.cursor = (uint32_t*)carve((NB + 1) * sizeof(uint32_t));
  L.task_off = (uint32_t*)carve((NB + 1) * sizeof(uint32_t));
  L.heavy = (uint2*)carve((size_t)L.heavy_cap * sizeof(uint2));
  L.bsum1 = (uint32_t*)carve((NB / SCAN_TILE + 2) * sizeof(uint32_t));
  L.bsum2 = (uint32_t*)carve((NB / SCAN_TILE + 2) * sizeof(uint32_t));
  L.tasks = (task_t*)carve(L.max_tasks * sizeof(task_t));
  L.order = (uint4*)carve(L.max_tasks * sizeof(uint4));
  L.partials = (uint32_t*)carve(L.max_tasks * xyzz_bytes);
  L.pyrA = (uint32_t*)carve(WB * B * xyzz_bytes);
  L.pyrB = (uint32_t*)carve(WB * B * xyzz_bytes);
  L.winsum = (uint32_t*)carve((W + K) * xyzz_bytes);
  L.endo = glv ? (uint32_t*)carve(n_in * (xyzz_bytes == 288 ? 128 : 64)) : nullptr;
  L.total = (size_t)(p - base);
  return L;
}

static bool msm_uses_glv(bool prepared, size_t batch) { return !prepared && batch == 1; }
int msm_glv_windows(int c) { return msm_windows(c, true); }

int msm_direct_max_log() {
  static const int v = [] { const char* e = getenv("ZKHIP_DIRECT_MAX_LOG"); const int x = e ? atoi(e) : 15; return (x >= 0 && x <= 18) ? x : 15; }();
  return v;
}
static inline bool msm_direct_wanted(size_t n) { const int L = msm_direct_max_log(); return L > 0 && n >= 2 && n <= ((size_t)1 << L); }

size_t msm_workspace_bytes(size_t n_one, int c, bool prepared, size_t batch, size_t xyzz_bytes) {
  if (n_one == 0 || batch == 0) return 0;
  size_t b = msm_lay_out(nullptr, n_one, batch, c, prepared, xyzz_bytes, msm_uses_glv(prepared, batch)).total;
  if (prepared && batch == 1 && xyzz_bytes == 144 && msm_direct_wanted(n_one)) b = std::max(b, msm_direct_workspace_bytes(n_one));
  return b;
}

int msm_build_tasks(const uint32_t* d_scalars, size_t n_in, size_t batch, size_t scalar_stride, int c, bool shared_buckets, uint32_t ref_base, uint32_t ref_stride,
                    size_t xyzz_bytes, void* ws, size_t ws_bytes, hipStream_t stream, msm_tasks_view* out, bool glv) {
  const uint32_t K = (uint32_t)batch;
  const bool wide = msm_two_level(c, glv, n_in, shared_buckets, batch);
  const int W = msm_windows(c, glv);
  if (glv && (K != 1 || c > 16 || shared_buckets)) { set_error("msm: GLV digits are for one vector of the general path"); return ZKHIP_EINVAL; }
  const size_t n = glv ? 2 * n_in : n_in;
  const uint32_t B = 1u << (c - 1);
  const int WB = shared_buckets ? (int)K : W;
  const uint32_t NB = (uint32_t)WB * B;
  if ((size_t)W * n * K >= (1ull << 32) || (size_t)WB * B >= (1ull << 31)) { set_error("msm: W*n*batch overflows 32-bit slot index"); return ZKHIP_EINVAL; }
  if (c > 16 && (!shared_buckets || K != 1)) { set_error("msm: windows above 16 bits need one shared bucket set"); return ZKHIP_EINVAL; }
  if (wide && !shared_buckets && (size_t)W * (B >> FINE_BITS) > (size_t)MAX_GROUPS) { set_error("msm: two-level sort: %d windows x %u groups exceed %d", W, B >> FINE_BITS, MAX_GROUPS); return ZKHIP_EINVAL; }
  if (wide && W > MAX_WIDE_W) { set_error("msm: %d windows of %d bits exceed the wide path's %d", W, c, MAX_WIDE_W); return ZKHIP_EINVAL; }
  const msm_layout lay = msm_lay_out((char*)ws, n_in, K, c, shared_buckets, xyzz_bytes, glv);
  if (ws_bytes < lay.total) { set_error("msm: workspace too small (%zu < %zu bytes)", ws_bytes, lay.total); return ZKHIP_EINVAL; }
  const uint32_t task_shift = lay.task_shift;
  const uint32_t n_pad = (uint32_t)((n + 7) & ~(size_t)7);
  void* const digits = lay.digits;
  uint32_t* const stage_ref = lay.stage_ref;
  uint16_t* const stage_fine = lay.stage_fine;
  uint32_t *const gcounters = lay.gcounters, *const counters = lay.counters, *const count = lay.count, *const sorted = lay.sorted,
           *const offset = lay.offset, *const cursor = lay.cursor, *const task_off = lay.task_off, *const bsum1 = lay.bsum1, *const bsum2 = lay.bsum2;
  task_t* const tasks = lay.tasks;
  uint4* const order = lay.order;

  prof_begin(stream);
  HIPCHK(hipMemsetAsync(lay.zero_lo, 0, lay.zero_bytes, stream));
  const size_t sstride = K > 1 ? scalar_stride : n;
  const unsigned dblocks = (unsigned)(((size_t)K * n_pad + 255) / 256);
  const int narrow = (shared_buckets && !glv) ? msm_narrow_windows(c, W) : 0;
  if (glv && wide) hipLaunchKernelGGL(k_digits_glv<int32_t>, dim3((unsigned)((std::max<size_t>(n_in, 8) + 255) / 256)), dim3(256), 0, stream, d_scalars, (int32_t*)digits, (uint32_t)n_in, n_pad, c, W);
  else if (glv) hipLaunchKernelGGL(k_digits_glv<int16_t>, dim3((unsigned)((std::max<size_t>(n_in, 8) + 255) / 256)), dim3(256), 0, stream, d_scalars, (int16_t*)digits, (uint32_t)n_in, n_pad, c, W);
  else if (wide) {
    const unsigned wg_cap = n_pad > (1u << 21) ? 1024u : 512u;
    const unsigned wblocks = (unsigned)std::min<size_t>(((size_t)n_pad + 1023) / 1024, wg_cap);
    hipLaunchKernelGGL(k_digits_wide, dim3(wblocks), dim3(1024), 0, stream, d_scalars, (int32_t*)digits, (uint32_t)n, n_pad, c, W, gcounters + 1024, narrow);
  }
  else hipLaunchKernelGGL(k_digits, dim3(dblocks), dim3(256), 0, stream, d_scalars, (int16_t*)digits, (uint32_t)n, n_pad, c, W, K, sstride, 0);
  prof_mark(stream, "digits");
  uint32_t chunks = (uint32_t)((n + 65535) / 65536);
  while (chunks * (uint32_t)W * K < 256 && chunks < (n + 4095) / 4096) chunks *= 2;
  if (chunks == 0) chunks = 1;
  const uint32_t chunk = (uint32_t)((((n + chunks - 1) / chunks) + 7) & ~(size_t)7);
  const size_t lds = wide ? ((size_t)4 << FINE_BITS) : (size_t)B * sizeof(uint32_t);
  static std::once_flag attr_once[64];
  static hipError_t attr_err[64];
  int cur_dev = 0;
  HIPCHK(hipGetDevice(&cur_dev));
  std::call_once(attr_once[cur_dev & 63], [&] {
    hipError_t e = hipFuncSetAttribute((const void*)k_sort_pass<false>, hipFuncAttributeMaxDynamicSharedMemorySize, 128 * 1024);
    if (e == hipSuccess) e = hipFuncSetAttribute((const void*)k_sort_pass<true>, hipFuncAttributeMaxDynamicSharedMemorySize, 128 * 1024);
    if (e == hipSuccess) e = hipFuncSetAttribute((const void*)k_fine_sorted, hipFuncAttributeMaxDynamicSharedMemorySize, (2 * (1 << FINE_BITS) + SORT_CHUNK + SORT_CHUNK / 16) * 4);
    attr_err[cur_dev & 63] = e;
  });
  HIPCHK(attr_err[cur_dev & 63]);
  const uint32_t gstride = (wide && !shared_buckets) ? (B >> FINE_BITS) : 0u;
  const int G = wide ? (int)(gstride ? (uint32_t)W * gstride : (B >> FINE_BITS)) : 1;
  const uint32_t sort_chunk = SORT_CHUNK;
  const uint32_t sort_chunks = (uint32_t)(((size_t)W * n + sort_chunk - 1) / sort_chunk) + (uint32_t)G;
  const uint32_t wb_stride = shared_buckets ? 0u : B;
  if (wide) {
    if (glv)
      hipLaunchKernelGGL(k_coarse_count, dim3(chunks, W), dim3(1024), 0, stream, (const int32_t*)digits, n_pad, chunk, gcounters + 1024, gstride);
    hipLaunchKernelGGL(k_group_offsets, dim3(1), dim3(64), 0, stream, gcounters + 1024, W, G, gcounters + 128, gcounters + 3072, gcounters + 512, sort_chunk);
    static_assert(MAX_GROUPS == 128, "k_coarse_sorted scans two groups per lane of one wavefront");
    hipLaunchKernelGGL(k_coarse_sorted, dim3((n_pad + COARSE_CHUNK - 1) / COARSE_CHUNK, W), dim3(1024), 0, stream, (const int32_t*)digits, n_pad, gcounters + 3072,
                       stage_ref, stage_fine, ref_base, ref_stride, gstride);
    prof_mark(stream, "coarse");
    hipLaunchKernelGGL(k_fine_count, dim3(sort_chunks), dim3(1024), 0, stream, stage_fine, gcounters + 128, gcounters + 512, G, count, sort_chunk);
  } else {
    hipLaunchKernelGGL(k_sort_pass<false>, dim3(chunks, W, K), dim3(1024), lds, stream, (const int16_t*)digits, n_pad, chunk, c, count, (uint32_t*)nullptr, wb_stride, ref_base, ref_stride);
  }
  prof_mark(stream, "count");
  const uint32_t nblk = (NB + SCAN_TILE - 1) / SCAN_TILE;
  const bool scan_single = NB <= SCAN_SINGLE_MAX;
  if (scan_single) {
    hipLaunchKernelGGL(k_scan_single<0>, dim3(1), dim3(1024), 0, stream, count, (uint32_t)NB, counters + 0, offset, cursor, 0u, (uint32_t*)nullptr);
  } else {
    hipLaunchKernelGGL(k_scan_sums2, dim3(nblk), dim3(SCAN_BLOCK), 0, stream, count, NB, bsum1, bsum2, task_shift);
    hipLaunchKernelGGL(k_scan_top2, dim3(1), dim3(SCAN_BLOCK), 0, stream, bsum1, bsum2, nblk, counters + 0, counters + 1);
    hipLaunchKernelGGL(k_scan_apply2, dim3(std::min(nblk, SCAN_APPLY_WGS)), dim3(SCAN_BLOCK), 0, stream, count, NB, bsum1, bsum2, counters + 0, counters + 1, offset, cursor, task_off,
                       task_shift, nblk, counters + 32);
  }
  prof_mark(stream, "scan");
  if (wide) {
    hipLaunchKernelGGL(k_fine_sorted, dim3(sort_chunks), dim3(1024), (size_t)(2u * (1u << FINE_BITS) + SORT_CHUNK + SORT_CHUNK / 16) * 4, stream, stage_fine, stage_ref,
                       gcounters + 128, gcounters + 512, G, cursor, sorted);
  }
  else hipLaunchKernelGGL(k_sort_pass<true>, dim3(chunks, W, K), dim3(1024), lds, stream, (const int16_t*)digits, n_pad, chunk, c, cursor, sorted, wb_stride, ref_base, ref_stride);
  prof_mark(stream, "scatter");
  const unsigned task_blocks = (unsigned)std::min<size_t>((NB + 255) / 256, 256);
  if (scan_single) {
    hipLaunchKernelGGL(k_scan_single<1>, dim3(1), dim3(1024), 0, stream, count, (uint32_t)NB, counters + 1, task_off, (uint32_t*)nullptr, task_shift, counters + 192);
    hipLaunchKernelGGL(k_make_tasks, dim3(task_blocks), dim3(256), 0, stream, offset, task_off, NB, tasks, task_shift, counters + 2, lay.seq_parts,
                       counters + 3, lay.heavy, lay.heavy_cap);
    hipLaunchKernelGGL(k_make_order, dim3(task_blocks), dim3(256), 0, stream, offset, task_off, NB, task_shift, counters + 192, sorted, order,
                       (const uint32_t*)nullptr, (task_t*)nullptr, counters + 2, lay.seq_parts, counters + 3, lay.heavy, lay.heavy_cap);
  } else {
    hipLaunchKernelGGL(k_make_order, dim3(task_blocks), dim3(256), 0, stream, offset, task_off, NB, task_shift, counters + 192, sorted, order,
                       (const uint32_t*)(counters + 32), tasks, counters + 2, lay.seq_parts, counters + 3, lay.heavy, lay.heavy_cap);
  }
  prof_mark(stream, "tasks");
  out->c = c; out->W = W; out->WB = WB; out->B = B; out->NB = NB; out->task_shift = task_shift; out->max_tasks = lay.max_tasks; out->nk = n * K;
  out->tasks = tasks; out->ntasks = counters + 1; out->max_parts = counters + 2; out->order = order; out->sorted = sorted; out->task_off = task_off;
  out->partials = lay.partials; out->pyrA = lay.pyrA; out->pyrB = lay.pyrB; out->winsum = lay.winsum;
  out->combine_lanes = lay.combine_lanes; out->seq_parts = lay.seq_parts; out->heavy_count = counters + 3; out->heavy = lay.heavy; out->heavy_cap = lay.heavy_cap; out->heavy_done = lay.heavy_done;
  out->endo = lay.endo;
  HIPCHK(hipGetLastError());
  return ZKHIP_OK;
}

static int msm_accumulate_combine(const msm_tasks_view& tv, const uint32_t* d_bases, bool prepared, bool glv, size_t n, uint32_t* buckets, hipStream_t stream) {
  const uint32_t NB = tv.NB;
  const size_t max_tasks = tv.max_tasks;
  const task_t* const tasks = tv.tasks;
  uint32_t* const counters = tv.ntasks - 1;
  const uint4* const order = tv.order;
  const uint32_t *const sorted = tv.sorted, *const task_off = tv.task_off;
  uint32_t* const partials = tv.partials;
  {
    uint32_t blocks = (uint32_t)((max_tasks + 127) / 128);
    if (blocks > 256 * 64) blocks = 256 * 64;
    if (prepared) hipLaunchKernelGGL(k_accumulate<true>, dim3(blocks), dim3(128), 0, stream, tasks, counters + 1, order, sorted, d_bases, partials, buckets, (const uint32_t*)nullptr, 0xffffffffu);
    else hipLaunchKernelGGL(k_accumulate<false>, dim3(blocks), dim3(128), 0, stream, tasks, counters + 1, order, sorted, d_bases, partials, buckets, (const uint32_t*)tv.endo,
                            glv ? (uint32_t)n : 0xffffffffu);
  }
  prof_mark(stream, "accumulate");
  {
    const int combine_lanes = tv.combine_lanes;
    const uint32_t seq_parts = tv.seq_parts;
    const size_t lanes_total = (size_t)NB * combine_lanes;
    const bool quad = lanes_total * 4 <= 131072;
    const unsigned blocks = (unsigned)((lanes_total * (quad ? 4 : 1) + 127) / 128);
#define ZK_LAUNCH_COMBINE(L)                                                                                                                        \
    do {                                                                                                                                              \
      if (quad) hipLaunchKernelGGL(k_combine_seq_quad<L>, dim3(blocks + HEAVY_WGS), dim3(128), 0, stream, task_off, NB, partials, buckets, seq_parts, blocks,   \
                                   tv.heavy_count, (const uint2*)tv.heavy, tv.heavy_cap, tv.heavy_done, HEAVY_QUAD_MAX);                              \
      else hipLaunchKernelGGL(k_combine_seq<L>, dim3(blocks + HEAVY_WGS), dim3(128), 0, stream, task_off, NB, partials, buckets, seq_parts, blocks,             \
                              tv.heavy_count, (const uint2*)tv.heavy, tv.heavy_cap, tv.heavy_done, HEAVY_QUAD_MAX);                                   \
    } while (0)
    if (combine_lanes == 1) ZK_LAUNCH_COMBINE(1);
    else if (combine_lanes == 2) ZK_LAUNCH_COMBINE(2);
    else if (combine_lanes == 4) ZK_LAUNCH_COMBINE(4);
    else ZK_LAUNCH_COMBINE(8);
#undef ZK_LAUNCH_COMBINE
  }
  prof_mark(stream, "combine");
  return ZKHIP_OK;
}

static int msm_reduce_buckets(int WB, uint32_t B, int c, uint32_t K, bool prepared, uint32_t* cur, uint32_t* nxt, uint32_t* winsum, uint32_t* d_out, hipStream_t stream) {
  if (B == 1) { set_error("msm: internal: B == 1"); return ZKHIP_EINVAL; }
  reduce_plan plan;
  if (!reduce_make_plan(B, WB, prepared, &plan)) { set_error("msm: internal: no reduction plan for %u buckets x %d sets", B, WB); return ZKHIP_EINVAL; }
  uint32_t* const jac_out = plan.direct ? d_out : nullptr;
  for (int i = 0; i < plan.n; i++) {
    const reduce_launch& L = plan.l[i];
    const dim3 rows(L.grid, WB), threads(PYRAMID_THREADS);
    const bool sum = L.kind == REDUCE_FINISH || L.kind == REDUCE_HORNER_QUAD || L.kind == REDUCE_HORNER;
    if (sum) prof_mark(stream, "pyramid");
    switch (L.kind) {
      case REDUCE_STEP: hipLaunchKernelGGL(k_pyramid_step, rows, threads, 0, stream, cur, nxt, L.N, L.s, L.in_stride, L.out_stride); break;
      case REDUCE_STEP_QUAD: hipLaunchKernelGGL(k_pyramid_step_quad, rows, threads, 0, stream, cur, nxt, L.N, L.s, L.in_stride, L.out_stride); break;
      case REDUCE_PAIR_QUAD: hipLaunchKernelGGL(k_pyramid_pair_quad, rows, threads, 0, stream, cur, nxt, L.N, L.s, L.in_stride, L.out_stride); break;
      case REDUCE_PAIR: hipLaunchKernelGGL(k_pyramid_pair, rows, threads, 0, stream, cur, nxt, L.N, L.in_stride, L.out_stride); break;
      case REDUCE_FINISH: hipLaunchKernelGGL(k_reduce_finish, dim3(L.grid), dim3(FINISH_THREADS), 0, stream, cur, L.in_stride, L.N, L.s, winsum, jac_out); break;
      case REDUCE_HORNER_QUAD: hipLaunchKernelGGL(k_window_horner_quad, dim3(L.grid), dim3(128), 0, stream, cur, L.in_stride, plan.nz, winsum, jac_out); break;
      case REDUCE_HORNER: hipLaunchKernelGGL(k_window_horner, dim3(L.grid), dim3(HORNER_THREADS), 0, stream, cur, L.in_stride, plan.nz, winsum, WB); break;
      case REDUCE_STORE: hipLaunchKernelGGL(k_store_results, dim3(L.grid), dim3(STORE_THREADS), 0, stream, winsum, K, d_out); break;
      case REDUCE_FOLD: hipLaunchKernelGGL(k_fold, dim3(L.grid), dim3(64), 0, stream, winsum, WB, c, d_out); break;
    }
    if (sum) prof_mark(stream, "horner");
    if (L.out_stride) { uint32_t* t = cur; cur = nxt; nxt = t; }
  }
  prof_mark(stream, "fold");
  HIPCHK(hipGetLastError());
  return ZKHIP_OK;
}

int msm_g1_device(const uint32_t* d_scalars, const uint32_t* d_bases, size_t n, uint32_t* d_out, void* ws, size_t ws_bytes,
                  int c_override, hipStream_t stream, const prepared_bases* prepared, size_t prepared_off, size_t batch,
                  size_t scalar_stride) {
  if (batch == 0) return ZKHIP_OK;
  if (n == 0) {
    for (size_t k = 0; k < batch; k++) hipLaunchKernelGGL(k_sum_jacobian, dim3(1), dim3(64), 0, stream, (const uint32_t*)nullptr, 0, d_out + k * 24, 1u);
    HIPCHK(hipGetLastError());
    return ZKHIP_OK;
  }
  if (batch > 1 && (!prepared || prepared->c > 16 || batch > 65535)) { set_error("msm: batch needs prepared bases with a window <= 16 bits"); return ZKHIP_EINVAL; }
  const uint32_t K = (uint32_t)batch;
  if (n >= (1ull << 31)) { set_error("msm: n = %zu too large", n); return ZKHIP_EINVAL; }
  const int c = prepared ? prepared->c : (c_override > 0 ? c_override : msm_pick_window(n));
  if (c < 2 || c > (prepared ? MAX_WINDOW_PREPARED : 16)) { set_error("msm: window bits %d out of range", c); return ZKHIP_EINVAL; }
  if (prepared) {
    if (prepared_off + n > prepared->n) { set_error("msm: range exceeds the prepared bases"); return ZKHIP_EINVAL; }
    if ((size_t)((256 + c - 1) / c) * prepared->n >= (1ull << 31)) { set_error("msm: prepared table too large for 31-bit point references"); return ZKHIP_EINVAL; }
    d_bases = prepared->table;
    if (prepared->direct && batch == 1) return msm_g1_direct(d_scalars, n, prepared, prepared_off, d_out, ws, ws_bytes, stream);
  }
  msm_tasks_view tv;
  const bool glv = msm_uses_glv(prepared != nullptr, batch);
  int rc = msm_build_tasks(d_scalars, n, batch, scalar_stride, c, prepared != nullptr, prepared ? (uint32_t)prepared_off : 0u, prepared ? (uint32_t)prepared->n : 0u,
                           144, ws, ws_bytes, stream, &tv, glv);
  if (rc != ZKHIP_OK) return rc;
  if (glv) hipLaunchKernelGGL(k_endo_bases, dim3((unsigned)((n + 255) / 256)), dim3(256), 0, stream, d_bases, (uint32_t)n, tv.endo);
  if ((rc = msm_accumulate_combine(tv, d_bases, prepared != nullptr, glv, n, tv.pyrA, stream)) != ZKHIP_OK) return rc;
  return msm_reduce_buckets(tv.WB, tv.B, c, K, prepared != nullptr, tv.pyrA, tv.pyrB, tv.winsum, d_out, stream);
}

__global__ void __launch_bounds__(128) k_bucket_sets_add(uint32_t* __restrict__ acc, const uint32_t* __restrict__ add, uint32_t nb) {
  const uint32_t k = blockIdx.x * blockDim.x + threadIdx.x;
  if (k >= nb) return;
  store_xyzz(acc, k, xyzz_add(load_xyzz(acc, k), load_xyzz(add, k)));
}

static size_t msm_chunk_lay_bytes(size_t chunk_cap, int c) {
  size_t b = msm_lay_out(nullptr, chunk_cap, 1, c, true).total;
  if (chunk_cap > 1) b = std::max(b, msm_lay_out(nullptr, chunk_cap - 1, 1, c, true).total);
  return align_up(b, 256);
}

size_t msm_chunk_workspace_bytes(size_t chunk_cap, int c) {
  if (chunk_cap == 0) return 0;
  return msm_chunk_lay_bytes(chunk_cap, c) + align_up(((size_t)1 << (c - 1)) * 144, 256);
}

int msm_chunk_add(const uint32_t* d_scalars, size_t n, const prepared_bases* pb, size_t pb_off, size_t chunk_cap, bool first, void* ws, size_t ws_bytes, hipStream_t stream) {
  if (!pb || n == 0 || n > chunk_cap || pb_off + n > pb->n) { set_error("msm_chunk_add: bad piece (n = %zu, capacity %zu)", n, chunk_cap); return ZKHIP_EINVAL; }
  const size_t lay_bytes = msm_chunk_lay_bytes(chunk_cap, pb->c);
  if (ws_bytes < msm_chunk_workspace_bytes(chunk_cap, pb->c)) { set_error("msm_chunk_add: workspace too small"); return ZKHIP_EINVAL; }
  uint32_t* const acc = (uint32_t*)((char*)ws + lay_bytes);
  msm_tasks_view tv;
  int rc = msm_build_tasks(d_scalars, n, 1, 0, pb->c, true, (uint32_t)pb_off, (uint32_t)pb->n, 144, ws, lay_bytes, stream, &tv, false);
  if (rc != ZKHIP_OK) return rc;
  if ((rc = msm_accumulate_combine(tv, pb->table, true, false, n, first ? acc : tv.pyrA, stream)) != ZKHIP_OK) return rc;
  if (!first) hipLaunchKernelGGL(k_bucket_sets_add, dim3((tv.NB + 127) / 128), dim3(128), 0, stream, acc, (const uint32_t*)tv.pyrA, tv.NB);
  HIPCHK(hipGetLastError());
  return ZKHIP_OK;
}

int msm_chunk_finish(const prepared_bases* pb, size_t chunk_cap, uint32_t* d_out, void* ws, size_t ws_bytes, hipStream_t stream) {
  if (!pb || ws_bytes < msm_chunk_workspace_bytes(chunk_cap, pb->c)) { set_error("msm_chunk_finish: workspace too small"); return ZKHIP_EINVAL; }
  const msm_layout lay = msm_lay_out((char*)ws, chunk_cap, 1, pb->c, true);
  uint32_t* const acc = (uint32_t*)((char*)ws + msm_chunk_lay_bytes(chunk_cap, pb->c));
  return msm_reduce_buckets(1, 1u << (pb->c - 1), pb->c, 1, true, acc, lay.pyrA, lay.winsum, d_out, stream);
}


constexpr int GEN_CHUNK = 32;

__device__ __forceinline__ xyzz scalar_mul_affine(const uint32_t (&kw)[8], const fe& gx, const fe& gy) {
  xyzz acc = xyzz_identity();
  for (int bit = 255; bit >= 0; bit--) {
    acc = xyzz_dbl(acc);
    if ((kw[bit >> 5] >> (bit & 31)) & 1) xyzz_madd(acc, gx, gy);
  }
// ... 661 lines not shown
```

zksnap_circuits_halo2_amd/csrc/msm_g2.hip:

```cpp
#include <hip/hip_runtime.h>
#include <cstdint>
#include "ec2.hpp"
#include "ec2_quad.hpp"
#include "reduce_plan.hpp"
#include "zkhip_internal.hpp"

namespace zkhip {

__device__ constexpr uint32_t BETA2_EXT[8] = {0x13e80b9cu, 0x3350c88eu, 0xdb5e56b9u, 0x7dce557cu, 0xb615564au, 0x6001b4b8u, 0x020217e0u, 0x2682e617u};

__global__ void __launch_bounds__(256) k2_endo_bases(const uint32_t* __restrict__ bases, uint32_t n, uint32_t* __restrict__ endo) {
  const uint32_t i = blockIdx.x * blockDim.x + threadIdx.x;
  if (i >= n) return;
  const affine2_words pt = load_affine2(bases, i);
  const fe beta = fq_from_ext(BETA2_EXT);
  uint32_t out[32];
  fq_to_ext(fe_mul<Fq>(beta, fq_from_ext(pt.w)), out);
  fq_to_ext(fe_mul<Fq>(beta, fq_from_ext(pt.w + 8)), out + 8);
#pragma unroll
  for (int k = 16; k < 32; k++) out[k] = pt.w[k];
  uint4* o = reinterpret_cast<uint4*>(endo + (size_t)i * 32);
#pragma unroll
  for (int k = 0; k < 8; k++) o[k] = make_uint4(out[4 * k], out[4 * k + 1], out[4 * k + 2], out[4 * k + 3]);
}
// ... 59 lines not shown
  const bool live = k < nbuckets;
  xyzz2 acc = xyzz2_identity();
  uint32_t m = 0;
  if (live) {
    const uint32_t t = task_off[k];
    m = task_off[k + 1] - t;
    if (m > seq_parts) m = 1;
    if (m != 1) {
#pragma unroll 1
      for (uint32_t j = q; j < m; j += LANES) acc = xyzz2_add_lazy_regmem<true>(acc, partials, t + j);
    }
  }
#pragma unroll 1
  for (int mask = 1; mask < LANES; mask <<= 1) acc = xyzz2_add_lazy<true>(acc, xyzz2_shfl_xor(acc, mask));
  if (live && q == 0 && m != 1) store_xyzz2(buckets, k, acc);
}

__global__ void __launch_bounds__(64) k2_combine_heavy(const uint32_t* __restrict__ task_off, const uint32_t* __restrict__ partials, uint32_t* __restrict__ buckets,
                                                       const uint32_t* __restrict__ heavy_count, const uint2* __restrict__ heavy, uint32_t heavy_cap) {
  __shared__ __attribute__((aligned(16))) uint32_t xch[32 * 72];
  const uint32_t nh = min(*heavy_count, heavy_cap);
  for (uint32_t i = blockIdx.x; i < nh; i += gridDim.x) {
    const uint2 e = heavy[i];
    if (e.y != 0) continue;
    const uint32_t k = e.x, t = task_off[k], m = task_off[k + 1] - t;
    xyzz2 acc = xyzz2_identity();
#pragma unroll 1
    for (uint32_t j = threadIdx.x; j < m; j += 64) acc = xyzz2_add_lazy_regmem<true>(acc, partials, t + j);
#pragma unroll 1
    for (uint32_t half = 32; half >= 1; half >>= 1) {
      __syncthreads();
      if (threadIdx.x >= half && threadIdx.x < 2 * half) store_xyzz2(xch, threadIdx.x - half, acc);
      __syncthreads();
      if (threadIdx.x < half) acc = xyzz2_add_lazy_regmem<true>(acc, xch, threadIdx.x);
    }
    if (threadIdx.x == 0) store_xyzz2(buckets, k, acc);
  }
}

__global__ void __launch_bounds__(64) k2_pyramid_step(const uint32_t* __restrict__ in, uint32_t* __restrict__ out, uint32_t N, int s, uint32_t in_stride,
                                                      uint32_t out_stride) {
  const uint32_t per_win = N / 2 + (uint32_t)s * (N / 4);
  const uint32_t tid = blockIdx.x * blockDim.x + threadIdx.x;
  if (tid >= per_win) return;
  const int win = blockIdx.y;
  const uint32_t* wi = in + (size_t)win * in_stride * 72;
  uint32_t* wo = out + (size_t)win * out_stride * 72;
  uint32_t ia, ib;
  reduce_step_operands(N, s, tid, ia, ib);
  store_xyzz2(wo, tid, xyzz2_add_lazy_mem<true>(wi, ia, wi, ib));
}

__global__ void __launch_bounds__(64) k2_pyramid_step_quad(const uint32_t* __restrict__ in, uint32_t* __restrict__ out, uint32_t N, int s, uint32_t in_stride,
                                                           uint32_t out_stride) {
  const uint32_t per_win = N / 2 + (uint32_t)s * (N / 4);
  const uint32_t gid = blockIdx.x * blockDim.x + threadIdx.x;
  const uint32_t tid = gid >> 2, q = gid & 3;
  if (tid >= per_win) return;
  const int win = blockIdx.y;
  const uint32_t* wi = in + (size_t)win * in_stride * 72;
  uint32_t* wo = out + (size_t)win * out_stride * 72;
  uint32_t ia, ib;
  reduce_step_operands(N, s, tid, ia, ib);
  const xyzz2 r = xyzz2_quad_to_std(xyzz2_add_quad_lazy(load_xyzz2(wi, ia), load_xyzz2(wi, ib), q));
  if (q == 0) store_xyzz2(wo, tid, r);
}

__global__ void __launch_bounds__(128) k2_window_sum(const uint32_t* __restrict__ in, uint32_t in_stride, int nz, uint32_t* __restrict__ winsum, int W) {
  __shared__ __attribute__((aligned(16))) uint32_t xch[72];
  const int win = blockIdx.x, term = threadIdx.x >> 2;
  const uint32_t q = threadIdx.x & 3;
  const uint32_t* wi = in + (size_t)win * in_stride * 72;
  xyzz2 acc = xyzz2_identity();
  int dbl = 0;
  if (term < nz) { acc = load_xyzz2(wi, 2 + term); dbl = term; }
  else if (term == nz) { acc = load_xyzz2(wi, 1); dbl = nz; }
  else if (term == nz + 1) acc = xyzz2_add_quad_lazy(load_xyzz2(wi, 0), load_xyzz2(wi, 1), q);
#pragma unroll 1
  for (int i = 0; i < dbl; i++) acc = xyzz2_dbl_quad_lazy(acc, q);
#pragma unroll 1
  for (int mask = 4; mask < 64; mask <<= 1) acc = xyzz2_add_quad_lazy(acc, xyzz2_quad_to_std(xyzz2_shfl_xor(acc, mask)), q);
  acc = xyzz2_quad_to_std(acc);
  if (threadIdx.x == 64) store_xyzz2(xch, 0, acc);
  __syncthreads();
  if (threadIdx.x < 4) {
    acc = xyzz2_quad_to_std(xyzz2_add_quad_lazy(acc, load_xyzz2(xch, 0), q));
    if (q == 0) store_xyzz2(winsum, win, acc);
  }
}

__global__ void __launch_bounds__(64) k2_fold(const uint32_t* __restrict__ winsum, int W, int c, uint32_t* __restrict__ out) {
  if (threadIdx.x >= 4 || blockIdx.x != 0) return;
  const uint32_t q = threadIdx.x;
  xyzz2 acc = load_xyzz2(winsum, W - 1);
  for (int w = W - 2; w >= 0; w--) {
#pragma unroll 1
    for (int i = 0; i < c; i++) acc = xyzz2_dbl_quad_lazy(acc, q);
    acc = xyzz2_add_quad_lazy(acc, load_xyzz2(winsum, w), q);
  }
  if (q == 0) store_jacobian2(xyzz2_quad_to_std(acc), out);
}

__global__ void __launch_bounds__(64) k2_store_identity(uint32_t* __restrict__ out) {
  if (threadIdx.x == 0 && blockIdx.x == 0) store_jacobian2(xyzz2_identity(), out);
}

__global__ void __launch_bounds__(64) k2_test_op_quad(int op, const uint32_t* __restrict__ a, const uint32_t* __restrict__ b, uint32_t* __restrict__ out, size_t n) {
  const size_t gid = (size_t)blockIdx.x * blockDim.x + threadIdx.x;
  const size_t i = gid >> 2;
  const uint32_t q = (uint32_t)(gid & 3);
  if (i >= n) return;
  const affine2_words pa = load_affine2(a, i), pb = load_affine2(b, i);
  xyzz2 A = xyzz2_identity(), B = xyzz2_identity();
  fe2 x, y;
  if (!affine2_is_identity(pa)) { affine2_coords(pa, false, x, y); xyzz2_madd(A, x, y); A = xyzz2_dbl(A); }
  if (!affine2_is_identity(pb)) { affine2_coords(pb, false, x, y); xyzz2_madd(B, x, y); }
  xyzz2 r;
  if (op == 3) r = xyzz2_add_quad(A, B, q);
  else if (op == 4) r = xyzz2_dbl_quad(A, q);
  else if (op == 5) r = xyzz2_quad_to_std(xyzz2_add_quad_lazy(xyzz2_dbl_quad_lazy(A, q), B, q));
  else r = xyzz2_quad_to_std(xyzz2_dbl_quad_lazy(xyzz2_dbl_quad_lazy(xyzz2_dbl_quad_lazy(A, q), q), q));
  if (q == 0) store_jacobian2(r, out + i * 48);
}

__global__ void __launch_bounds__(64) k2_test_op(int op, const uint32_t* __restrict__ a, const uint32_t* __restrict__ b, uint32_t* __restrict__ out, size_t n) {
  const size_t i = (size_t)blockIdx.x * blockDim.x + threadIdx.x;
  if (i >= n) return;
  const affine2_words pa = load_affine2(a, i), pb = load_affine2(b, i);
  xyzz2 acc = xyzz2_identity();
  fe2 x, y;
  if (!affine2_is_identity(pa)) { affine2_coords(pa, false, x, y); xyzz2_madd(acc, x, y); }
  if (op == 1) acc = xyzz2_dbl(acc);
  else if (!affine2_is_identity(pb)) {
    affine2_coords(pb, op == 2, x, y);
    if (i & 1) xyzz2_madd(acc, x, y);
    else { xyzz2 t = xyzz2_identity(); xyzz2_madd(t, x, y); acc = xyzz2_add(acc, t); }
  }
  store_jacobian2(acc, out + i * 48);
}

static int pick_window_g2(size_t n) {
  int best = 2;
  double best_cost = 1e300;
  for (int c = 2; c <= 16; c++) {
    const int W = msm_glv_windows(c), top_bits = 127 - (W - 1) * c;
    if (top_bits > 0 && top_bits < 6) continue;
    const double cost = (double)W * (34.0 * (double)(2 * n) + 96.0 * (double)(1u << (c - 1))) + 1.3e6 * (double)c * (double)(W - 1) / 16.0;
    if (cost < best_cost) { best_cost = cost; best = c; }
  }
  return best;
}

size_t msm_g2_workspace_bytes(size_t n) { return n ? msm_workspace_bytes(n, pick_window_g2(n), false, 1, 288) : 0; }

int msm_g2_device(const uint32_t* d_scalars, const uint32_t* d_bases, size_t n, uint32_t* d_out, void* ws, size_t ws_bytes, hipStream_t stream) {
  if (n == 0) {
    hipLaunchKernelGGL(k2_store_identity, dim3(1), dim3(64), 0, stream, d_out);
    HIPCHK(hipGetLastError());
    return ZKHIP_OK;
  }
  if (n >= (1ull << 31)) { set_error("msm_g2: n = %zu too large", n); return ZKHIP_EINVAL; }
  const int c = pick_window_g2(n);
  msm_tasks_view tv;
  int rc = msm_build_tasks(d_scalars, n, 1, n, c, false, 0u, 0u, 288, ws, ws_bytes, stream, &tv, true);
  if (rc != ZKHIP_OK) return rc;
  hipLaunchKernelGGL(k2_endo_bases, dim3((unsigned)((n + 255) / 256)), dim3(256), 0, stream, d_bases, (uint32_t)n, tv.endo);
  {
    uint32_t blocks = (uint32_t)((tv.max_tasks + 63) / 64);
    if (blocks > 256 * 32) blocks = 256 * 32;
    hipLaunchKernelGGL(k2_accumulate, dim3(blocks), dim3(64), 0, stream, tv.ntasks, tv.order, tv.sorted, d_bases, tv.partials, tv.pyrA, (const uint32_t*)tv.endo, (uint32_t)n);
  }
  prof_mark(stream, "accumulate_g2");
  {
    const unsigned cblocks = (unsigned)(((size_t)tv.NB * (size_t)tv.combine_lanes + 63) / 64);
    if (tv.combine_lanes == 1) hipLaunchKernelGGL(k2_combine<1>, dim3(cblocks), dim3(64), 0, stream, tv.task_off, tv.NB, tv.partials, tv.pyrA, tv.seq_parts);
    else if (tv.combine_lanes == 2) hipLaunchKernelGGL(k2_combine<2>, dim3(cblocks), dim3(64), 0, stream, tv.task_off, tv.NB, tv.partials, tv.pyrA, tv.seq_parts);
    else if (tv.combine_lanes == 4) hipLaunchKernelGGL(k2_combine<4>, dim3(cblocks), dim3(64), 0, stream, tv.task_off, tv.NB, tv.partials, tv.pyrA, tv.seq_parts);
    else hipLaunchKernelGGL(k2_combine<8>, dim3(cblocks), dim3(64), 0, stream, tv.task_off, tv.NB, tv.partials, tv.pyrA, tv.seq_parts);
  }
  hipLaunchKernelGGL(k2_combine_heavy, dim3(256), dim3(64), 0, stream, tv.task_off, tv.partials, tv.pyrA, tv.heavy_count, (const uint2*)tv.heavy, tv.heavy_cap);
  prof_mark(stream, "combine_g2");
  uint32_t* cur = tv.pyrA;
  uint32_t* nxt = tv.pyrB;
  uint32_t in_stride = tv.B, N = tv.B;
  int s = 1;
  while (N > 2) {
    const uint32_t per_win = N / 2 + (uint32_t)s * (N / 4);
    if ((size_t)per_win * tv.WB <= 32768) hipLaunchKernelGGL(k2_pyramid_step_quad, dim3((4 * per_win + 63) / 64, tv.WB), dim3(64), 0, stream, cur, nxt, N, s, in_stride, per_win);
    else hipLaunchKernelGGL(k2_pyramid_step, dim3((per_win + 63) / 64, tv.WB), dim3(64), 0, stream, cur, nxt, N, s, in_stride, per_win);
    uint32_t* t = cur; cur = nxt; nxt = t;
    in_stride = per_win;
    N >>= 1;
    s++;
  }
  const int nz = s - 1;
  prof_mark(stream, "pyramid_g2");
  hipLaunchKernelGGL(k2_window_sum, dim3(tv.WB), dim3(128), 0, stream, cur, in_stride, nz, tv.winsum, tv.WB);
  hipLaunchKernelGGL(k2_fold, dim3(1), dim3(64), 0, stream, tv.winsum, tv.WB, c, d_out);
  prof_mark(stream, "fold_g2");
  HIPCHK(hipGetLastError());
  return ZKHIP_OK;
}

int test_g2_op(int op, const uint32_t* d_a, const uint32_t* d_b, uint32_t* d_out, size_t n, hipStream_t stream) {
  if (n == 0) return ZKHIP_OK;
  if (op >= 3) hipLaunchKernelGGL(k2_test_op_quad, dim3((unsigned)((4 * n + 63) / 64)), dim3(64), 0, stream, op, d_a, d_b, d_out, n);
  else hipLaunchKernelGGL(k2_test_op, dim3((unsigned)((n + 63) / 64)), dim3(64), 0, stream, op, d_a, d_b, d_out, n);
  return hipGetLastError() == hipSuccess ? ZKHIP_OK : ZKHIP_EHIP;
}

}
```

zksnap_circuits_halo2_amd/csrc/zkhip_internal.hpp:

```cpp
#pragma once
#include <string>
#include <hip/hip_runtime.h>
#include <cstddef>
#include <cstdint>
#include <cstring>
#include <vector>
#include "../../include/zkhip.h"
#include "scan_plan.hpp"
#include "rowvm_blob.hpp"

namespace zkhip {

void set_error(const char* fmt, ...) __attribute__((format(printf, 1, 2)));

static inline bool fr_words_canonical(const uint64_t w[4]) {
  constexpr uint64_t R[4] = {0x43e1f593f0000001ull, 0x2833e84879b97091ull, 0xb85045b68181585dull, 0x30644e72e131a029ull};
  for (int i = 3; i >= 0; i--)
    if (w[i] != R[i]) return w[i] < R[i];
  return false;
}

#define HIPCHK(x) do { hipError_t e_ = (x); if (e_ != hipSuccess) { ::zkhip::set_error("%s failed: %s", #x, hipGetErrorString(e_)); return ZKHIP_EHIP; } } while (0)

void prof_begin(hipStream_t stream);
void prof_mark(hipStream_t stream, const char* name);

int g1_gen_walk_device(const uint32_t t0_ext[8], const uint32_t d_ext[8], size_t n, uint32_t* d_out, void* ws, size_t ws_bytes, hipStream_t stream);
size_t g1_gen_walk_workspace(size_t n);
size_t g1_fixed_base_table_bytes();
size_t g1_fixed_base_workspace(size_t n);
int g1_fixed_base_table_build(uint32_t* d_table, void* ws, size_t ws_bytes, hipStream_t stream);
int g1_fixed_base_mul_device(const uint32_t* d_scalars, size_t n, const uint32_t* d_table, uint32_t* d_out, void* ws, size_t ws_bytes, hipStream_t stream);
int msm_pick_window(size_t n);
size_t msm_workspace_bytes(size_t n, int c, bool prepared = false, size_t batch = 1, size_t xyzz_bytes = 144);
struct task_t {
  uint32_t bucket, start, len;
};
struct msm_tasks_view {
  int c, W, WB;
  uint32_t B, NB, task_shift;
  size_t max_tasks, nk;
  const task_t* tasks;
  uint32_t* ntasks;
  uint32_t* max_parts;
  const uint4* order;
  const uint32_t* sorted;
  const uint32_t* task_off;
  uint32_t *partials, *pyrA, *pyrB, *winsum;
  int combine_lanes;
  uint32_t seq_parts;
  const uint32_t* heavy_count;
  const void* heavy;
  uint32_t heavy_cap;
  uint32_t* heavy_done;
  uint32_t* endo;
};
int msm_glv_windows(int c);
int msm_build_tasks(const uint32_t* d_scalars, size_t n, size_t batch, size_t scalar_stride, int c, bool shared_buckets, uint32_t ref_base, uint32_t ref_stride,
                    size_t xyzz_bytes, void* ws, size_t ws_bytes, hipStream_t stream, msm_tasks_view* out, bool glv = false);
size_t msm_g2_workspace_bytes(size_t n);
int msm_g2_device(const uint32_t* d_scalars, const uint32_t* d_bases, size_t n, uint32_t* d_out, void* ws, size_t ws_bytes, hipStream_t stream);
int test_g2_op(int op, const uint32_t* d_a, const uint32_t* d_b, uint32_t* d_out, size_t n, hipStream_t stream);
int test_g2_formula_op(int op, const uint32_t* d_a, const uint32_t* d_b, uint32_t* d_out, uint32_t* d_work, size_t n, hipStream_t stream);
int pairing_check_device(const uint32_t* d_g1, const uint32_t* d_g2, size_t n, uint32_t* d_ok, hipStream_t stream);
int test_fq12_op(int op, int which, const uint32_t* d_a, const uint32_t* d_b, uint32_t* d_out, hipStream_t stream);
struct prepared_bases {
  uint32_t* table;
  size_t n;
  int c, W;
  uint32_t* direct = nullptr;
};
size_t direct_table_bytes(size_t n);
size_t msm_direct_workspace_bytes(size_t n);
int prepare_direct_table(prepared_bases* pb, const uint32_t* d_bases, hipStream_t stream);
int msm_g1_direct(const uint32_t* d_scalars, size_t n, const prepared_bases* pb, size_t off, uint32_t* d_out, void* ws, size_t ws_bytes, hipStream_t stream);
int msm_pick_window_prepared(size_t n);
int msm_g1_device(const uint32_t* d_scalars, const uint32_t* d_bases, size_t n, uint32_t* d_out, void* ws, size_t ws_bytes,
                  int c_override, hipStream_t stream, const prepared_bases* prepared = nullptr, size_t prepared_off = 0, size_t batch = 1,
                  size_t scalar_stride = 0);
size_t msm_chunk_workspace_bytes(size_t chunk_cap, int c);
int msm_chunk_add(const uint32_t* d_scalars, size_t n, const prepared_bases* pb, size_t pb_off, size_t chunk_cap, bool first, void* ws, size_t ws_bytes, hipStream_t stream);
int msm_chunk_finish(const prepared_bases* pb, size_t chunk_cap, uint32_t* d_out, void* ws, size_t ws_bytes, hipStream_t stream);
int prepare_bases_device(const uint32_t* d_bases, size_t n, hipStream_t stream, prepared_bases** out, int c_override = 0, size_t n_whole = 0);
void release_prepared(prepared_bases* pb);
int sum_jacobian_device(const uint32_t* d_in, int m, uint32_t* d_out, hipStream_t stream, size_t count = 1);
size_t g1_batch_normalize_workspace(size_t n);
int g1_batch_normalize_device(const uint32_t* d_in, size_t n, uint32_t* d_out, void* ws, size_t ws_bytes, hipStream_t stream);
size_t g1_fft_workspace(size_t n);
int g1_fft_device(const uint32_t* d_in, int in_format, uint32_t* d_out, int out_format, uint32_t log_n, const uint32_t omega_ext[8],
                  const uint32_t* scale_ext, void* ws, size_t ws_bytes, hipStream_t stream);

int ntt_passes(uint32_t L);
int ntt_transform(const uint32_t* d_in, uint32_t in_len, uint32_t in_stride, uint32_t* d_out, uint32_t out_len, uint32_t out_stride,
                  uint32_t batch, uint32_t L, const uint32_t omega_ext[8], const uint32_t* in_scale, uint32_t in_period,
                  const uint32_t* out_scale, uint32_t out_period, uint32_t* tmp0, uint32_t* tmp1, hipStream_t stream);
int fr_mul_periodic_device(uint32_t* d_a, size_t n, const uint32_t* d_table_ext, uint32_t period, hipStream_t stream);
int fr_scale_device(uint32_t* d_a, size_t n, const uint32_t scale_ext[8], hipStream_t stream);
void ntt_clear_cache();

struct arg_ring {
  static constexpr int SLOTS = 8;
  static constexpr size_t SLOT_BYTES = 32768;
  void* host = nullptr;
  hipEvent_t ev[SLOTS] = {};
  bool used[SLOTS] = {};
  int turn = 0;
  int upload(void* dst, const void* src, size_t bytes, hipStream_t stream) {
    if (bytes == 0) return ZKHIP_OK;
    if (bytes > SLOT_BYTES) return plain(dst, src, bytes, stream);
    if (!host && hipHostMalloc(&host, SLOTS * SLOT_BYTES, hipHostMallocDefault) != hipSuccess) { (void)hipGetLastError(); host = nullptr; return plain(dst, src, bytes, stream); }
    const int s = turn;
    turn = (turn + 1) % SLOTS;
    if (!ev[s] && hipEventCreateWithFlags(&ev[s], hipEventDisableTiming) != hipSuccess) { (void)hipGetLastError(); ev[s] = nullptr; return plain(dst, src, bytes, stream); }
    if (used[s] && hipEventSynchronize(ev[s]) != hipSuccess) { set_error("arg_ring: event wait failed"); return ZKHIP_EHIP; }
    void* slot = (char*)host + (size_t)s * SLOT_BYTES;
    std::memcpy(slot, src, bytes);
    if (hipMemcpyAsync(dst, slot, bytes, hipMemcpyHostToDevice, stream) != hipSuccess || hipEventRecord(ev[s], stream) != hipSuccess) { set_error("arg_ring: copy failed"); return ZKHIP_EHIP; }
    used[s] = true;
    return ZKHIP_OK;
  }
  static int plain(void* dst, const void* src, size_t bytes, hipStream_t stream) {
    if (hipMemcpyAsync(dst, src, bytes, hipMemcpyHostToDevice, stream) != hipSuccess || hipStreamSynchronize(stream) != hipSuccess) { set_error("upload of call arguments failed"); return ZKHIP_EHIP; }
    return ZKHIP_OK;
  }
  void release() {
    for (int i = 0; i < SLOTS; i++) if (ev[i]) { if (used[i]) (void)hipEventSynchronize(ev[i]); (void)hipEventDestroy(ev[i]); ev[i] = nullptr; used[i] = false; }
    if (host) { (void)hipHostFree(host); host = nullptr; }
  }
};
static inline int upload_args(arg_ring* ring, void* dst, const void* src, size_t bytes, hipStream_t stream) {
  return ring ? ring->upload(dst, src, bytes, stream) : arg_ring::plain(dst, src, bytes, stream);
}

size_t poly_workspace_bytes(size_t n);
int fr_eval_polynomial_device(const uint32_t* d_a, size_t n, const uint32_t x_host[8], uint32_t* d_result, void* ws, size_t ws_bytes, hipStream_t stream);
size_t poly_batch_workspace_bytes(size_t n, size_t count);
int fr_eval_polynomial_batch_device(const void* const* d_polys_host, size_t count, size_t n, const uint32_t x_host[8], uint32_t* d_results,
                                    void* ws, size_t ws_bytes, hipStream_t stream, arg_ring* ring = nullptr);
int fr_kate_division_device(const uint32_t* d_a, size_t n, const uint32_t b_host[8], uint32_t* d_q, void* ws, size_t ws_bytes, hipStream_t stream);
size_t poly_roots_workspace_bytes(size_t n, uint32_t m);
int fr_divide_by_roots_device(const uint32_t* d_a, size_t n, const uint32_t (*roots_host)[8], uint32_t m, uint32_t* d_q, uint32_t* d_evals, void* ws,
                              size_t ws_bytes, hipStream_t stream);
int fr_prefix_product_device(const uint32_t* d_v, size_t n, uint32_t* d_out, void* ws, size_t ws_bytes, hipStream_t stream);
int fr_batch_invert_device(uint32_t* d_a, size_t n, void* ws, size_t ws_bytes, hipStream_t stream);
int fr_lagrange_cosets_window_device(uint32_t* out_l0, uint32_t* out_last, uint32_t* out_active, size_t W, uint64_t start, uint32_t k, uint32_t ext_k,
                                     uint32_t n_terms, int active_is_sum, const uint32_t consts[10][8], hipStream_t stream);
size_t lincomb_workspace_bytes(size_t count, size_t n);
int fr_linear_combination_device(const void* const* d_cols_host, const uint32_t* coeffs_host, size_t count, size_t n, uint32_t* d_out, void* ws, size_t ws_bytes,
                                 hipStream_t stream, arg_ring* ring = nullptr);
size_t perm_workspace_bytes(uint32_t nperm, uint32_t chunk, uint32_t log_n);
int fr_permutation_products_device(const void* const* d_values_host, const void* const* d_sigmas_host, uint32_t nperm, uint32_t chunk, uint32_t log_n,
                                   size_t usable, const uint32_t beta[8], const uint32_t gamma[8], const uint32_t delta[8], const uint32_t omega[8],
                                   uint32_t* d_z, void* ws, size_t ws_bytes, hipStream_t stream, arg_ring* ring = nullptr);
size_t lookup_products_workspace_bytes(uint32_t n_lookups, uint32_t log_n);
int fr_lookup_products_device(const void* const* d_inputs_host, const void* const* d_tables_host, const uint32_t* d_permuted_inputs, const uint32_t* d_permuted_tables,
                              uint32_t n_lookups, uint32_t log_n, size_t usable, const uint32_t beta[8], const uint32_t gamma[8], uint32_t* d_z, void* ws,
                              size_t ws_bytes, hipStream_t stream, arg_ring* ring = nullptr);

int row_vm_validate(const zkhip_vm_program* p, uint32_t n_columns, uint32_t log_rows, int accumulate);
struct vm_staging {
  void* host[2] = {nullptr, nullptr};
  size_t cap[2] = {0, 0};
  hipEvent_t copied[2] = {nullptr, nullptr};
  int turn = 0;
  void release();
};
enum vm_form { VM_WHOLE, VM_WINDOW, VM_CHECK };
struct vm_call {
  const zkhip_vm_program* progs = nullptr;
  uint32_t n_progs = 1;
  const void* const* d_columns = nullptr;
  uint32_t n_columns = 0, log_rows = 0;
  vm_form form = VM_WHOLE;
  uint64_t row0 = 0, count = 0;
  int accumulate = 0;
  uint32_t* d_out = nullptr;
  uint32_t* const* d_outs = nullptr;
  void* ws = nullptr;
  size_t ws_bytes = 0;
  hipStream_t stream = nullptr;
  vm_staging* staging = nullptr;
  bool interpreter_only = false;
  int* compiled = nullptr;
};
int row_vm_launch(const vm_call& c);
bool row_vm_jit_wanted(const zkhip_vm_program* p, uint32_t n_columns, uint32_t log_rows);
bool row_vm_jit_wanted_window(const zkhip_vm_program* p, uint32_t n_columns, uint64_t count);
int row_vm_jit_launch(const zkhip_vm_program* p, const void* const* d_columns, uint32_t n_columns, uint32_t log_rows, bool window, uint64_t row0, uint64_t count,
                      int accumulate, const uint32_t* d_consts, const uint32_t* d_pow_lo, const uint32_t* d_pow_hi, uint32_t* d_out, hipStream_t stream);
void row_vm_jit_clear();
uint64_t row_vm_jit_launches();
int row_vm_jit_source(const zkhip_vm_program* p, uint32_t n_columns, uint32_t log_rows, std::string* out);
int row_vm_jit_compile_only(const zkhip_vm_program* p, uint32_t n_columns, uint32_t log_rows, size_t* code_bytes);
int fr_pointwise_mul_device(const uint32_t* d_a, const uint32_t* d_b, size_t n, uint32_t* d_out, hipStream_t stream);
int fr_gather_mul_device(const uint32_t* d_a, uint32_t a_len, const uint32_t* d_ia, const uint32_t* d_b, uint32_t b_len, const uint32_t* d_ib, size_t n,
                         uint32_t* d_out, hipStream_t stream);
int check_reports_init_device(void* d_reports, uint32_t n, hipStream_t stream);
int check_copies_device(const void* d_columns_dev, uint32_t n_columns, uint32_t log_n, const uint32_t* d_map_col, const uint32_t* d_map_row, void* d_report,
                        hipStream_t stream);

size_t lookup_permute_workspace_bytes(size_t usable_rows);
int lookup_permute_device(const uint32_t* d_input, const uint32_t* d_table, size_t usable_rows, uint32_t* d_out_input, uint32_t* d_out_table,
                          void* ws, size_t ws_bytes, hipStream_t stream);
size_t lookup_permute_many_workspace_bytes(uint32_t n_lookups, size_t usable_rows);
int lookup_permute_many_device(const void* const* d_inputs_host, const void* const* d_tables_host, uint32_t n_lookups, size_t n, size_t usable_rows,
                               uint32_t* d_out_input, uint32_t* d_out_table, void* ws, size_t ws_bytes, hipStream_t stream, arg_ring* ring = nullptr);
size_t lookup_check_workspace_bytes(uint32_t n_lookups, size_t usable_rows);
int lookup_check_device(const void* const* d_inputs_host, const void* const* d_tables_host, uint32_t n_lookups, size_t usable_rows, void* d_reports, void* ws,
                        size_t ws_bytes, hipStream_t stream, arg_ring* ring = nullptr);

int fr_random_device(const uint8_t seed[32], uint64_t stream_id, uint64_t first, size_t n, uint32_t* d_out, hipStream_t stream);
size_t fr_random_rows_workspace_bytes(uint32_t n_cols);
int fr_random_rows_device(const uint8_t seed[32], uint64_t stream_id, uint64_t first, const void* const* d_cols_host, uint32_t n_cols, size_t row0, size_t count,
// ... 76 lines not shown
```

Baseline: 765.8 Mpoints/s.

## Generalize MSM bucket task length from power-of-two shift to arbitrary length

Replaces the power-of-two task_shift with a general task_len and moves the choice into a new task_plan header. For large inputs the new heuristic sizes tasks to fit the estimated lane slots across the chip, so lengths that are not powers of two can be chosen to balance load and fill the device. It also folds the full-length cursor reservation in k_make_order into one atomic and drops one block barrier. In exchange, shifts in the scan and task kernels become integer divide and multiply. A test export for the chosen task length is added.

```diff
diff --git a/include/zkhip.h b/include/zkhip.h
--- a/include/zkhip.h
+++ b/include/zkhip.h
@@ -279,6 +279,7 @@
 
 int zkhip_test_reduce512(const uint8_t in64[64], uint64_t out_fr_mont[4]);
 uint32_t zkhip_test_transcript_chunk(size_t n);
+uint32_t zkhip_test_task_length(size_t n, size_t K, int prepared, int g2);
 
 #define ZKHIP_MAX_PAIRS 64
 int zkhip_pairing_check(const uint64_t *g1, const uint64_t *g2, size_t n, int *ok);
diff --git a/zksnap_circuits_halo2_amd/_lib.py b/zksnap_circuits_halo2_amd/_lib.py
--- a/zksnap_circuits_halo2_amd/_lib.py
+++ b/zksnap_circuits_halo2_amd/_lib.py
@@ -186,6 +186,7 @@
     "zkhip_shplonk_scalars_device": (C.c_int, [C.c_void_p, C.c_void_p, C.c_void_p, C.c_uint32, C.c_void_p, C.c_size_t, C.c_void_p, C.c_void_p, C.c_void_p, C.c_void_p]),
     "zkhip_test_reduce512": (C.c_int, [C.c_void_p, C.c_void_p]),
     "zkhip_test_transcript_chunk": (C.c_uint32, [C.c_size_t]),
+    "zkhip_test_task_length": (C.c_uint32, [C.c_size_t, C.c_size_t, C.c_int, C.c_int]),
     "zkhip_profile_enable": (C.c_int, [C.c_int]),
     "zkhip_profile_read": (C.c_int, [C.c_void_p, C.c_void_p, C.c_int]),
     "zkhip_profile_read_calls": (C.c_int, [C.c_void_p, C.c_void_p, C.c_void_p, C.c_int]),
diff --git a/zksnap_circuits_halo2_amd/csrc/capi.hip b/zksnap_circuits_halo2_amd/csrc/capi.hip
--- a/zksnap_circuits_halo2_amd/csrc/capi.hip
+++ b/zksnap_circuits_halo2_amd/csrc/capi.hip
@@ -4000,5 +4000,10 @@
 }
 
 uint32_t zkhip_test_transcript_chunk(size_t n) { return transcript_chunk(n); }
-
-}
+uint32_t zkhip_test_task_length(size_t n, size_t K, int prepared, int g2) {
+  if (g2) return (K == 1 && !prepared) ? msm_g2_task_length(n) : 0u;
+  if (n == 0 || K == 0) return 0u;
+  return msm_task_length(n, prepared ? msm_pick_window_prepared(n) : msm_pick_window(n), prepared != 0, K);
+}
+
+}
diff --git a/zksnap_circuits_halo2_amd/csrc/msm.hip b/zksnap_circuits_halo2_amd/csrc/msm.hip
--- a/zksnap_circuits_halo2_amd/csrc/msm.hip
+++ b/zksnap_circuits_halo2_amd/csrc/msm.hip
@@ -8,6 +8,7 @@
 #include "ec_quad.hpp"
 #include "fe_inverse.hpp"
 #include "reduce_plan.hpp"
+#include "task_plan.hpp"
 #include "zkhip_internal.hpp"
 
 namespace zkhip {
@@ -25,8 +26,6 @@
   const int narrow = W * c - 256;
   return narrow > 0 && narrow <= W ? narrow : 0;
 }
-constexpr int MAX_TASK_LEN = 128;
-constexpr int TASK_SHIFT = 6;
 
 __device__ __forceinline__ xyzz load_xyzz(const uint32_t* base, size_t idx) {
   const uint4* q = reinterpret_cast<const uint4*>(base + idx * 36);
@@ -603,8 +602,8 @@
 constexpr uint32_t SCAN_APPLY_WGS = 256;
 
 template <int MODE>
-__device__ __forceinline__ uint32_t scan_xform(uint32_t v, uint32_t task_shift) {
-  return MODE == 0 ? v : (v + (1u << task_shift) - 1) >> task_shift;
+__device__ __forceinline__ uint32_t scan_xform(uint32_t v, uint32_t task_len) {
+  return MODE == 0 ? v : task_count(v, task_len);
 }
 
 __device__ __forceinline__ uint32_t block_exclusive_scan(uint32_t v, uint32_t* lds, uint32_t& total) {
@@ -630,12 +629,12 @@
 }
 
 __global__ void __launch_bounds__(SCAN_BLOCK) k_scan_sums2(const uint32_t* __restrict__ in, uint32_t n, uint32_t* __restrict__ sums0,
-                                                           uint32_t* __restrict__ sums1, uint32_t task_shift) {
+                                                           uint32_t* __restrict__ sums1, uint32_t task_len) {
   __shared__ uint32_t lds[4];
   const uint32_t base = blockIdx.x * SCAN_TILE + threadIdx.x * SCAN_PER_THREAD;
   uint32_t s0 = 0, s1 = 0;
 #pragma unroll
-  for (int i = 0; i < SCAN_PER_THREAD; i++) if (base + i < n) { const uint32_t v = in[base + i]; s0 += v; s1 += scan_xform<1>(v, task_shift); }
+  for (int i = 0; i < SCAN_PER_THREAD; i++) if (base + i < n) { const uint32_t v = in[base + i]; s0 += v; s1 += scan_xform<1>(v, task_len); }
   uint32_t t0, t1;
   block_exclusive_scan(s0, lds, t0);
   block_exclusive_scan(s1, lds, t1);
@@ -660,7 +659,7 @@
 __global__ void __launch_bounds__(SCAN_BLOCK) k_scan_apply2(const uint32_t* __restrict__ in, uint32_t n, const uint32_t* __restrict__ sums0,
                                                             const uint32_t* __restrict__ sums1, const uint32_t* __restrict__ total0,
                                                             const uint32_t* __restrict__ total1, uint32_t* __restrict__ offset,
-                                                            uint32_t* __restrict__ cursor, uint32_t* __restrict__ task_off, uint32_t task_shift,
+                                                            uint32_t* __restrict__ cursor, uint32_t* __restrict__ task_off, uint32_t task_len,
                                                             uint32_t nblk, uint32_t* __restrict__ len_count) {
   __shared__ uint32_t lds[4];
   __shared__ uint32_t lh[MAX_TASK_LEN + 1];
@@ -680,17 +679,17 @@
     load_tile(blk + gridDim.x, vn);
     uint32_t s0 = 0, s1 = 0;
 #pragma unroll
-    for (int i = 0; i < SCAN_PER_THREAD; i++) { s0 += v[i]; s1 += scan_xform<1>(v[i], task_shift); }
+    for (int i = 0; i < SCAN_PER_THREAD; i++) { s0 += v[i]; s1 += scan_xform<1>(v[i], task_len); }
     uint32_t t0, t1;
     uint32_t e0 = block_exclusive_scan(s0, lds, t0) + sums0[blk];
     uint32_t e1 = block_exclusive_scan(s1, lds, t1) + sums1[blk];
 #pragma unroll
     for (int i = 0; i < SCAN_PER_THREAD; i++) {
       if (base + i < n) { offset[base + i] = e0; cursor[base + i] = e0; task_off[base + i] = e1; }
-      const uint32_t m = scan_xform<1>(v[i], task_shift);
+      const uint32_t m = scan_xform<1>(v[i], task_len);
       if (m) {
         n_full += m - 1;
-        atomicAdd(&lh[v[i] - ((m - 1) << task_shift)], 1u);
+        atomicAdd(&lh[task_last_len(v[i], m, task_len)], 1u);
       }
       e0 += v[i];
       e1 += m;
@@ -700,7 +699,7 @@
   }
 #pragma unroll
   for (int off = 32; off >= 1; off >>= 1) n_full += (uint32_t)__shfl_xor((int)n_full, off, 64);
-  if ((threadIdx.x & 63) == 0 && n_full) atomicAdd(&lh[1u << task_shift], n_full);
+  if ((threadIdx.x & 63) == 0 && n_full) atomicAdd(&lh[task_len], n_full);
   __syncthreads();
   if (threadIdx.x <= MAX_TASK_LEN && lh[threadIdx.x]) atomicAdd(&len_count[threadIdx.x], lh[threadIdx.x]);
   if (blockIdx.x == 0 && threadIdx.x == 0) { offset[n] = *total0; task_off[n] = *total1; }
@@ -709,14 +708,14 @@
 constexpr uint32_t SCAN_SINGLE_MAX = 8192;
 template <int MODE>
 __global__ void __launch_bounds__(1024) k_scan_single(const uint32_t* __restrict__ in, uint32_t n, uint32_t* __restrict__ total_out,
-                                                      uint32_t* __restrict__ out, uint32_t* __restrict__ out2, uint32_t task_shift,
+                                                      uint32_t* __restrict__ out, uint32_t* __restrict__ out2, uint32_t task_len,
                                                       uint32_t* __restrict__ len_cursor) {
   __shared__ uint32_t wsum[16];
   __shared__ uint32_t lh[MAX_TASK_LEN + 1];
   if (MODE == 1 && threadIdx.x <= MAX_TASK_LEN) lh[threadIdx.x] = 0;
   __syncthreads();
   const int lane = threadIdx.x & 63, wave = threadIdx.x >> 6;
-  const uint32_t full = 1u << task_shift;
+  const uint32_t full = task_len;
   uint32_t running = 0, n_full = 0;
   for (uint32_t tile = 0; tile < n; tile += 8192) {
     const uint32_t base = tile + threadIdx.x * 8;
@@ -724,11 +723,11 @@
 #pragma unroll
     for (int i = 0; i < 8; i++) {
       const uint32_t raw = base + i < n ? in[base + i] : 0u;
-      v[i] = scan_xform<MODE>(raw, task_shift);
+      v[i] = scan_xform<MODE>(raw, task_len);
       s += v[i];
       if (MODE == 1 && raw) {
         n_full += v[i] - 1;
-        atomicAdd(&lh[raw - ((v[i] - 1) << task_shift)], 1u);
+        atomicAdd(&lh[task_last_len(raw, v[i], task_len)], 1u);
       }
     }
     uint32_t x = s;
@@ -766,10 +765,9 @@
   }
 }
 
-constexpr uint32_t HEAVY_SLICE = 2048;
 constexpr uint32_t COOP_TASKS = 32;
 __global__ void __launch_bounds__(256) k_make_tasks(const uint32_t* __restrict__ offset, const uint32_t* __restrict__ task_off,
-                                                    uint32_t nbuckets, task_t* __restrict__ tasks, uint32_t task_shift,
+                                                    uint32_t nbuckets, task_t* __restrict__ tasks, uint32_t task_len,
                                                     uint32_t* __restrict__ max_parts, uint32_t seq_parts,
                                                     uint32_t* __restrict__ heavy_count, uint2* __restrict__ heavy, uint32_t heavy_cap) {
   uint32_t nt = 0;
@@ -783,13 +781,13 @@
       for (uint32_t j = 0; j < m; j++) {
         task_t tk;
         tk.bucket = k;
-        tk.start = s + (j << task_shift);
-        tk.len = min(1u << task_shift, e - tk.start);
+        tk.start = task_first(s, j, task_len);
+        tk.len = task_len_of(e - s, j, task_len);
         tasks[t + j] = tk;
       }
     }
     if (m > seq_parts) {
-      const uint32_t P = (m + HEAVY_SLICE - 1) / HEAVY_SLICE;
+      const uint32_t P = heavy_slices(m);
       const uint32_t idx = atomicAdd(heavy_count, P);
       for (uint32_t i = 0; i < P; i++)
         if (idx + i < heavy_cap) heavy[idx + i] = make_uint2(k, i);
@@ -804,8 +802,8 @@
       for (uint32_t j = lane; j < bm; j += 64) {
         task_t tk;
         tk.bucket = bk;
-        tk.start = bs + (j << task_shift);
-        tk.len = min(1u << task_shift, be - tk.start);
+        tk.start = task_first(bs, j, task_len);
+        tk.len = task_len_of(be - bs, j, task_len);
         tasks[bt + j] = tk;
       }
     }
@@ -817,7 +815,7 @@
 
 constexpr int ORDER_JMAX = 64;
 __global__ void __launch_bounds__(256) k_make_order(const uint32_t* __restrict__ offset, const uint32_t* __restrict__ task_off,
-                                                    uint32_t nbuckets, uint32_t task_shift, uint32_t* __restrict__ len_cursor,
+                                                    uint32_t nbuckets, uint32_t task_len, uint32_t* __restrict__ len_cursor,
                                                     const uint32_t* __restrict__ sorted, uint4* __restrict__ order,
                                                     const uint32_t* __restrict__ len_count, task_t* __restrict__ tasks,
                                                     uint32_t* __restrict__ max_parts, uint32_t seq_parts, uint32_t* __restrict__ heavy_count,
@@ -842,11 +840,11 @@
     if (lane == 0) lbase[0] = 0;
   }
   __syncthreads();
-  const uint32_t full = 1u << task_shift, step = gridDim.x * blockDim.x;
+  const uint32_t full = task_len, step = gridDim.x * blockDim.x;
   for (uint32_t k = blockIdx.x * blockDim.x + threadIdx.x; k < nbuckets; k += step) {
     const uint32_t nt = task_off[k + 1] - task_off[k];
     if (nt) {
-      const uint32_t rem = (offset[k + 1] - offset[k]) - ((nt - 1) << task_shift);
+      const uint32_t rem = task_last_len(offset[k + 1] - offset[k], nt, full);
       atomicAdd(&lh[rem], 1u);
       const uint32_t nfull = nt - 1, head = min(nfull, (uint32_t)ORDER_JMAX);
       for (uint32_t j = 0; j < head; j++) atomicAdd(&jcnt[j], 1u);
@@ -857,12 +855,12 @@
   if (threadIdx.x == 0) {
     uint32_t run = 0;
     for (int j = 0; j <= ORDER_JMAX; j++) { joff[j] = run; run += jcnt[j]; }
-    const uint32_t base = run ? lbase[full] + atomicAdd(&len_cursor[full], run) : 0u;
+    const uint32_t rfull = lh[full];
+    const uint32_t base = (run + rfull) ? lbase[full] + atomicAdd(&len_cursor[full], run + rfull) : 0u;
     for (int j = 0; j <= ORDER_JMAX; j++) joff[j] += base;
+    lh[full] = base + run;
   }
   if (threadIdx.x <= MAX_TASK_LEN && threadIdx.x != full) { const uint32_t v = lh[threadIdx.x]; lh[threadIdx.x] = v ? lbase[threadIdx.x] + atomicAdd(&len_cursor[threadIdx.x], v) : 0u; }
-  __syncthreads();
-  if (threadIdx.x == 0 && lh[full]) lh[full] = lbase[full] + atomicAdd(&len_cursor[full], lh[full]);
   __syncthreads();
   const uint32_t lane = threadIdx.x & 63u;
   uint32_t mx = 0;
@@ -872,20 +870,21 @@
     if (k < nbuckets) { t = task_off[k]; nt = task_off[k + 1] - t; }
     if (nt) {
       s0 = offset[k];
-      const uint32_t rem = (offset[k + 1] - s0) - ((nt - 1) << task_shift);
+      const uint32_t rem = task_last_len(offset[k + 1] - s0, nt, full);
       nfull = nt - 1;
       head = min(nfull, (uint32_t)ORDER_JMAX);
+      const uint32_t st = task_first(s0, nt - 1, full);
+      const uint32_t ref_last = sorted[st], ref_first = sorted[s0];
       for (uint32_t j = 0; j < head; j++) {
-        const uint32_t st = s0 + (j << task_shift);
-        order[atomicAdd(&joff[j], 1u)] = make_uint4(t + j, st, full, sorted[st]);
-        if (tasks) tasks[t + j] = task_t{k, st, full};
+        const uint32_t stj = task_first(s0, j, full);
+        order[atomicAdd(&joff[j], 1u)] = make_uint4(t + j, stj, full, j == 0 ? ref_first : sorted[stj]);
+        if (tasks) tasks[t + j] = task_t{k, stj, full};
       }
       if (nfull > head) pos = atomicAdd(&joff[ORDER_JMAX], nfull - head);
-      const uint32_t st = s0 + ((nt - 1) << task_shift);
-      order[atomicAdd(&lh[rem], 1u)] = make_uint4(nt == 1 ? (0x80000000u | k) : t + nt - 1, st, rem, sorted[st]);
+      order[atomicAdd(&lh[rem], 1u)] = make_uint4(nt == 1 ? (0x80000000u | k) : t + nt - 1, st, rem, ref_last);
       if (tasks) tasks[t + nt - 1] = task_t{k, st, rem};
       if (tasks && nt > seq_parts) {
-        const uint32_t P = (nt + HEAVY_SLICE - 1) / HEAVY_SLICE;
+        const uint32_t P = heavy_slices(nt);
         const uint32_t idx = atomicAdd(heavy_count, P);
         for (uint32_t i = 0; i < P; i++)
           if (idx + i < heavy_cap) heavy[idx + i] = make_uint2(k, i);
@@ -895,7 +894,7 @@
     const bool coop = nfull - head > COOP_TASKS;
     if (!coop) {
       for (uint32_t j = head; j < nfull; j++) {
-        const uint32_t st = s0 + (j << task_shift);
+        const uint32_t st = task_first(s0, j, full);
         order[pos + j - head] = make_uint4(t + j, st, full, sorted[st]);
         if (tasks) tasks[t + j] = task_t{k, st, full};
       }
@@ -907,7 +906,7 @@
       const uint32_t bt = (uint32_t)__shfl((int)t, src, 64), bs0 = (uint32_t)__shfl((int)s0, src, 64), bpos = (uint32_t)__shfl((int)pos, src, 64),
                      bnfull = (uint32_t)__shfl((int)nfull, src, 64), bhead = (uint32_t)__shfl((int)head, src, 64);
       for (uint32_t j = bhead + lane; j < bnfull; j += 64) {
-        const uint32_t st = bs0 + (j << task_shift);
+        const uint32_t st = task_first(bs0, j, full);
         order[bpos + j - bhead] = make_uint4(bt + j, st, full, sorted[st]);
         if (tasks) tasks[bt + j] = task_t{base + (uint32_t)src, st, full};
       }
@@ -1348,7 +1347,7 @@
 }
 
 struct msm_layout {
-  uint32_t task_shift;
+  uint32_t task_len;
   size_t max_tasks;
   void* digits;
   uint32_t* stage_ref; uint16_t* stage_fine;
@@ -1364,21 +1363,6 @@
   size_t total;
 };
 
-static uint32_t msm_task_shift(size_t entries , size_t NB, size_t xyzz_bytes = 144) {
-  uint32_t task_shift = TASK_SHIFT;
-  if ((entries >> 7) >= ((size_t)3 << 16)) task_shift = 7;
-  const bool g2 = xyzz_bytes == 288;
-  if ((entries >> TASK_SHIFT) < ((size_t)1 << (g2 ? 14 : 17))) {
-    const double occ = (double)entries / (double)NB;
-    double best = 1e300;
-    for (uint32_t sh = 2; sh <= (uint32_t)TASK_SHIFT; sh++) {
-      const double L = (double)(1u << sh), parts = occ / L;
-      const double est = 5.0 * L + (g2 ? 15.0 : 10.0) * (parts > 1.0 ? parts - 1.0 : 0.0);
-      if (est < best) { best = est; task_shift = sh; }
-    }
-  }
-  return task_shift;
-}
 
 constexpr size_t GLV_TWO_LEVEL_MIN = (size_t)1 << 18;
 constexpr size_t PREP_TWO_LEVEL_MIN = (size_t)1 << 16;
@@ -1396,12 +1380,12 @@
   const bool wide = msm_two_level(c, glv, n_in, prepared, K);
   const size_t nk = n * K, entries = W * nk;
   const size_t n_pad = (n + 7) & ~(size_t)7;
-  L.task_shift = msm_task_shift(entries, NB, xyzz_bytes);
-  L.max_tasks = (entries >> L.task_shift) + NB + 1;
-  const double parts_avg = (double)entries / (double)NB / (double)(1u << L.task_shift);
-  L.combine_lanes = parts_avg <= 2.0 ? 1 : (parts_avg <= 4.0 ? 2 : (parts_avg <= 12.0 ? 4 : 8));
-  L.seq_parts = 16u * (uint32_t)L.combine_lanes;
-  L.heavy_cap = (uint32_t)(std::min<size_t>(L.max_tasks / (L.seq_parts + 1) + 1, NB) + L.max_tasks / HEAVY_SLICE + 1);
+  const task_plan plan = task_make_plan(entries, NB, task_lane_slots(xyzz_bytes), xyzz_bytes);
+  L.task_len = plan.len;
+  L.max_tasks = plan.max_tasks;
+  L.combine_lanes = plan.combine_lanes;
+  L.seq_parts = plan.seq_parts;
+  L.heavy_cap = plan.heavy_cap;
   char* p = base;
   auto carve = [&](size_t bytes) { void* r = p; p += align_up(bytes, 256); return r; };
   L.digits = carve(W * K * n_pad * (wide ? sizeof(int32_t) : sizeof(int16_t)));
@@ -1447,6 +1431,11 @@
   return b;
 }
 
+uint32_t msm_task_length(size_t n_one, int c, bool prepared, size_t batch, size_t xyzz_bytes) {
+  if (n_one == 0 || batch == 0) return 0;
+  return msm_lay_out(nullptr, n_one, batch, c, prepared, xyzz_bytes, msm_uses_glv(prepared, batch)).task_len;
+}
+
 int msm_build_tasks(const uint32_t* d_scalars, size_t n_in, size_t batch, size_t scalar_stride, int c, bool shared_buckets, uint32_t ref_base, uint32_t ref_stride,
                     size_t xyzz_bytes, void* ws, size_t ws_bytes, hipStream_t stream, msm_tasks_view* out, bool glv) {
   const uint32_t K = (uint32_t)batch;
@@ -1463,7 +1452,7 @@
   if (wide && W > MAX_WIDE_W) { set_error("msm: %d windows of %d bits exceed the wide path's %d", W, c, MAX_WIDE_W); return ZKHIP_EINVAL; }
   const msm_layout lay = msm_lay_out((char*)ws, n_in, K, c, shared_buckets, xyzz_bytes, glv);
   if (ws_bytes < lay.total) { set_error("msm: workspace too small (%zu < %zu bytes)", ws_bytes, lay.total); return ZKHIP_EINVAL; }
-  const uint32_t task_shift = lay.task_shift;
+  const uint32_t task_len = lay.task_len;
   const uint32_t n_pad = (uint32_t)((n + 7) & ~(size_t)7);
   void* const digits = lay.digits;
   uint32_t* const stage_ref = lay.stage_ref;
@@ -1526,10 +1515,10 @@
   if (scan_single) {
     hipLaunchKernelGGL(k_scan_single<0>, dim3(1), dim3(1024), 0, stream, count, (uint32_t)NB, counters + 0, offset, cursor, 0u, (uint32_t*)nullptr);
   } else {
-    hipLaunchKernelGGL(k_scan_sums2, dim3(nblk), dim3(SCAN_BLOCK), 0, stream, count, NB, bsum1, bsum2, task_shift);
+    hipLaunchKernelGGL(k_scan_sums2, dim3(nblk), dim3(SCAN_BLOCK), 0, stream, count, NB, bsum1, bsum2, task_len);
     hipLaunchKernelGGL(k_scan_top2, dim3(1), dim3(SCAN_BLOCK), 0, stream, bsum1, bsum2, nblk, counters + 0, counters + 1);
     hipLaunchKernelGGL(k_scan_apply2, dim3(std::min(nblk, SCAN_APPLY_WGS)), dim3(SCAN_BLOCK), 0, stream, count, NB, bsum1, bsum2, counters + 0, counters + 1, offset, cursor, task_off,
-                       task_shift, nblk, counters + 32);
+                       task_len, nblk, counters + 32);
   }
   prof_mark(stream, "scan");
   if (wide) {
@@ -1540,17 +1529,17 @@
   prof_mark(stream, "scatter");
   const unsigned task_blocks = (unsigned)std::min<size_t>((NB + 255) / 256, 256);
   if (scan_single) {
-    hipLaunchKernelGGL(k_scan_single<1>, dim3(1), dim3(1024), 0, stream, count, (uint32_t)NB, counters + 1, task_off, (uint32_t*)nullptr, task_shift, counters + 192);
-    hipLaunchKernelGGL(k_make_tasks, dim3(task_blocks), dim3(256), 0, stream, offset, task_off, NB, tasks, task_shift, counters + 2, lay.seq_parts,
+    hipLaunchKernelGGL(k_scan_single<1>, dim3(1), dim3(1024), 0, stream, count, (uint32_t)NB, counters + 1, task_off, (uint32_t*)nullptr, task_len, counters + 192);
+    hipLaunchKernelGGL(k_make_tasks, dim3(task_blocks), dim3(256), 0, stream, offset, task_off, NB, tasks, task_len, counters + 2, lay.seq_parts,
                        counters + 3, lay.heavy, lay.heavy_cap);
-    hipLaunchKernelGGL(k_make_order, dim3(task_blocks), dim3(256), 0, stream, offset, task_off, NB, task_shift, counters + 192, sorted, order,
+    hipLaunchKernelGGL(k_make_order, dim3(task_blocks), dim3(256), 0, stream, offset, task_off, NB, task_len, counters + 192, sorted, order,
                        (const uint32_t*)nullptr, (task_t*)nullptr, counters + 2, lay.seq_parts, counters + 3, lay.heavy, lay.heavy_cap);
   } else {
-    hipLaunchKernelGGL(k_make_order, dim3(task_blocks), dim3(256), 0, stream, offset, task_off, NB, task_shift, counters + 192, sorted, order,
+    hipLaunchKernelGGL(k_make_order, dim3(task_blocks), dim3(256), 0, stream, offset, task_off, NB, task_len, counters + 192, sorted, order,
                        (const uint32_t*)(counters + 32), tasks, counters + 2, lay.seq_parts, counters + 3, lay.heavy, lay.heavy_cap);
   }
   prof_mark(stream, "tasks");
-  out->c = c; out->W = W; out->WB = WB; out->B = B; out->NB = NB; out->task_shift = task_shift; out->max_tasks = lay.max_tasks; out->nk = n * K;
+  out->c = c; out->W = W; out->WB = WB; out->B = B; out->NB = NB; out->task_len = task_len; out->max_tasks = lay.max_tasks; out->nk = n * K;
   out->tasks = tasks; out->ntasks = counters + 1; out->max_parts = counters + 2; out->order = order; out->sorted = sorted; out->task_off = task_off;
   out->partials = lay.partials; out->pyrA = lay.pyrA; out->pyrB = lay.pyrB; out->winsum = lay.winsum;
   out->combine_lanes = lay.combine_lanes; out->seq_parts = lay.seq_parts; out->heavy_count = counters + 3; out->heavy = lay.heavy; out->heavy_cap = lay.heavy_cap; out->heavy_done = lay.heavy_done;
diff --git a/zksnap_circuits_halo2_amd/csrc/msm_g2.hip b/zksnap_circuits_halo2_amd/csrc/msm_g2.hip
--- a/zksnap_circuits_halo2_amd/csrc/msm_g2.hip
+++ b/zksnap_circuits_halo2_amd/csrc/msm_g2.hip
@@ -235,6 +235,7 @@
 }
 
 size_t msm_g2_workspace_bytes(size_t n) { return n ? msm_workspace_bytes(n, pick_window_g2(n), false, 1, 288) : 0; }
+uint32_t msm_g2_task_length(size_t n) { return n ? msm_task_length(n, pick_window_g2(n), false, 1, 288) : 0; }
 
 int msm_g2_device(const uint32_t* d_scalars, const uint32_t* d_bases, size_t n, uint32_t* d_out, void* ws, size_t ws_bytes, hipStream_t stream) {
   if (n == 0) {
diff --git a/zksnap_circuits_halo2_amd/csrc/task_plan.hpp b/zksnap_circuits_halo2_amd/csrc/task_plan.hpp
--- /dev/null
+++ b/zksnap_circuits_halo2_amd/csrc/task_plan.hpp
@@ -0,0 +1,76 @@
+#pragma once
+#include <algorithm>
+#include <cstddef>
+#include <cstdint>
+
+#if defined(__HIPCC__)
+#define TASK_HD __host__ __device__ __forceinline__
+#else
+#define TASK_HD inline
+#endif
+
+namespace zkhip {
+
+constexpr int MAX_TASK_LEN = 128;
+constexpr int MIN_TASK_LEN = 4;
+constexpr uint32_t TASK_LEN_64 = 64;
+constexpr uint32_t HEAVY_SLICE = 2048;
+constexpr size_t TASK_FULL_MIN_TASKS = (size_t)1 << 17, TASK_FULL_MIN_TASKS_G2 = (size_t)1 << 14;
+constexpr size_t TASK_DEEP_MIN_TASKS = (size_t)3 << 16;
+constexpr double TASK_GAMMA = 1.0;
+constexpr uint32_t TASK_FULL_MIN_LEN = 32;
+constexpr size_t TASK_CHIP_SIMDS = 1024;
+
+inline size_t task_lane_slots(size_t xyzz_bytes) { return TASK_CHIP_SIMDS * (xyzz_bytes == 288 ? 2 : 4) * 64; }
+
+TASK_HD uint32_t task_count(uint32_t cnt, uint32_t L) { return cnt / L + (cnt % L ? 1u : 0u); }
+TASK_HD uint32_t task_first(uint32_t s0, uint32_t j, uint32_t L) { return s0 + j * L; }
+TASK_HD uint32_t task_last_len(uint32_t cnt, uint32_t nt, uint32_t L) { return cnt - (nt - 1) * L; }
+TASK_HD uint32_t task_len_of(uint32_t cnt, uint32_t j, uint32_t L) { const uint32_t r = cnt - j * L; return r < L ? r : L; }
+TASK_HD uint32_t heavy_slices(uint32_t nt) { return (nt + HEAVY_SLICE - 1) / HEAVY_SLICE; }
+
+struct task_plan {
+  uint32_t len;
+  size_t max_tasks;
+  int combine_lanes;
+  uint32_t seq_parts;
+  uint32_t heavy_cap;
+};
+
+inline uint32_t task_pick_len(size_t entries , size_t NB, size_t slots, size_t xyzz_bytes) {
+  const bool g2 = xyzz_bytes == 288;
+  const double occ = (double)entries / (double)NB;
+  if (entries / TASK_LEN_64 < (g2 ? TASK_FULL_MIN_TASKS_G2 : TASK_FULL_MIN_TASKS)) {
+    uint32_t len = TASK_LEN_64;
+    double best = 1e300;
+    for (uint32_t L = MIN_TASK_LEN; L <= TASK_LEN_64; L *= 2) {
+      const double parts = occ / (double)L;
+      const double est = 5.0 * (double)L + (g2 ? 15.0 : 10.0) * (parts > 1.0 ? parts - 1.0 : 0.0);
+      if (est < best) { best = est; len = L; }
+    }
+    return len;
+  }
+  const double fit = TASK_GAMMA * (double)entries / (double)slots;
+  const uint32_t deep = entries / MAX_TASK_LEN >= TASK_DEEP_MIN_TASKS ? (uint32_t)MAX_TASK_LEN : TASK_LEN_64;
+  if (occ > fit) return deep;
+  if (g2 || fit >= (double)TASK_LEN_64) return deep;
+  return std::max((uint32_t)fit, TASK_FULL_MIN_LEN);
+}
+
+inline size_t task_max_tasks(size_t entries, size_t NB, uint32_t L) { return entries / L + NB + 1; }
+inline uint32_t task_heavy_cap(size_t max_tasks, uint32_t seq_parts, size_t NB) {
+  return (uint32_t)(std::min<size_t>(max_tasks / (seq_parts + 1) + 1, NB) + max_tasks / HEAVY_SLICE + 1);
+}
+
+inline task_plan task_make_plan(size_t entries, size_t NB, size_t slots, size_t xyzz_bytes) {
+  task_plan P;
+  P.len = task_pick_len(entries, NB, slots, xyzz_bytes);
+  P.max_tasks = task_max_tasks(entries, NB, P.len);
+  const double parts_avg = (double)entries / (double)NB / (double)P.len;
+  P.combine_lanes = parts_avg <= 2.0 ? 1 : (parts_avg <= 4.0 ? 2 : (parts_avg <= 12.0 ? 4 : 8));
+  P.seq_parts = 16u * (uint32_t)P.combine_lanes;
+  P.heavy_cap = task_heavy_cap(P.max_tasks, P.seq_parts, NB);
+  return P;
+}
+
+}
diff --git a/zksnap_circuits_halo2_amd/csrc/zkhip_internal.hpp b/zksnap_circuits_halo2_amd/csrc/zkhip_internal.hpp
--- a/zksnap_circuits_halo2_amd/csrc/zkhip_internal.hpp
+++ b/zksnap_circuits_halo2_amd/csrc/zkhip_internal.hpp
@@ -33,12 +33,13 @@
 int g1_fixed_base_mul_device(const uint32_t* d_scalars, size_t n, const uint32_t* d_table, uint32_t* d_out, void* ws, size_t ws_bytes, hipStream_t stream);
 int msm_pick_window(size_t n);
 size_t msm_workspace_bytes(size_t n, int c, bool prepared = false, size_t batch = 1, size_t xyzz_bytes = 144);
+uint32_t msm_task_length(size_t n, int c, bool prepared = false, size_t batch = 1, size_t xyzz_bytes = 144);
 struct task_t {
   uint32_t bucket, start, len;
 };
 struct msm_tasks_view {
   int c, W, WB;
-  uint32_t B, NB, task_shift;
+  uint32_t B, NB, task_len;
   size_t max_tasks, nk;
   const task_t* tasks;
   uint32_t* ntasks;
@@ -59,6 +60,7 @@
 int msm_build_tasks(const uint32_t* d_scalars, size_t n, size_t batch, size_t scalar_stride, int c, bool shared_buckets, uint32_t ref_base, uint32_t ref_stride,
                     size_t xyzz_bytes, void* ws, size_t ws_bytes, hipStream_t stream, msm_tasks_view* out, bool glv = false);
 size_t msm_g2_workspace_bytes(size_t n);
+uint32_t msm_g2_task_length(size_t n);
 int msm_g2_device(const uint32_t* d_scalars, const uint32_t* d_bases, size_t n, uint32_t* d_out, void* ws, size_t ws_bytes, hipStream_t stream);
 int test_g2_op(int op, const uint32_t* d_a, const uint32_t* d_b, uint32_t* d_out, size_t n, hipStream_t stream);
 int test_g2_formula_op(int op, const uint32_t* d_a, const uint32_t* d_b, uint32_t* d_out, uint32_t* d_work, size_t n, hipStream_t stream);
```

Measured after the change: 770.1 Mpoints/s (median of 6 runs). No clear change (+0.6%).
